# vibevoice-community/VibeVoice

Hardware: AMD Instinct MI355X
Metric: audio-sec/wall-sec (higher is better)
Workload: dtype bf16

## Files before the change

vibevoice_amd/csrc/engine.hip:

```cpp
#include "engine_ctx.h"

thread_local char g_err[512] = "";
std::shared_mutex g_dev_mu;
std::mutex g_family_mu;

int fail(vv_ctx* ctx, const char* fmt, ...) {
    va_list ap; va_start(ap, fmt);
    char* dst = ctx ? ctx->err : g_err;
    vsnprintf(dst, 512, fmt, ap);
    va_end(ap);
    if (ctx) snprintf(g_err, 512, "%s", ctx->err);
    return -1;
}

int ring_acquire(vv_ctx* ctx) {
    const int slot = ctx->ring_i;
    ctx->ring_i = (ctx->ring_i + 1) % vv_ctx::RING;
    if (ctx->ring_used[slot]) hipEventSynchronize(ctx->ring_ev[slot]);
    ctx->ring_used[slot] = true;
    return slot;
}

void* dalloc(vv_ctx* ctx, size_t bytes, bool zero) {
    void* p = nullptr;
    if (bytes == 0) bytes = 16;
    if (hipMalloc(&p, bytes) != hipSuccess) { fail(ctx, "hipMalloc(%zu) failed", bytes); return nullptr; }
    if (zero) hipMemset(p, 0, bytes);
    else { static const int poison = [] { const char* e = getenv("VVHIP_POISON"); return (e && e[0] == '1') ? 1 : 0; }();
           if (poison) hipMemset(p, 0xFF, bytes); }
    if (ctx) ctx->allocs.insert(p);
    return p;
}
void dfree(vv_ctx* ctx, void* p) {
    if (!p) return;
    if (ctx) ctx->allocs.erase(p);
    hipFree(p);
}

int add_w(vv_ctx* ctx, const std::string& name, int kind, int64_t nelem, bool optional) {
    Weight w; w.name = name; w.kind = kind; w.nelem = nelem; w.optional = optional;
    ctx->widx[name] = (int)ctx->w.size();
    ctx->w.push_back(w);
    return (int)ctx->w.size() - 1;
}
void add_mat(vv_ctx* ctx, const std::string& name, int N, int K, void* base, int ntile_off, int pk, int Cin, int Cout, int ksz,
             int stride, int64_t src_nelem) {
    int i = add_w(ctx, name, W_MAT, src_nelem < 0 ? (int64_t)N * K : src_nelem);
    Weight& w = ctx->w[i];
    w.N = N; w.K = K; w.pk = pk; w.Cin = Cin; w.Cout = Cout; w.ksz = ksz; w.stride = stride;
    const int k_tiles = (K + 31) / 32;
    w.dev = (char*)base + (int64_t)ntile_off * k_tiles * 1024;
}
void* walloc(vv_ctx* ctx, size_t bytes, bool zero) {
    if (!ctx->creating) return dalloc(ctx, bytes, zero);
    if (ctx->parent) {
        vv_ctx* p = ctx->parent;
        if (ctx->wshare_i >= p->wallocs.size() || p->wallocs[ctx->wshare_i].second != bytes) {
            fail(ctx, "vv_create_shared: weight allocation %zu (%zu bytes) does not match the parent's -- different model configuration", ctx->wshare_i, bytes);
            return nullptr;
        }
        void* q = p->wallocs[ctx->wshare_i++].first;
        ctx->wallocs.push_back({q, bytes});
        return q;
    }
    void* q = dalloc(ctx, bytes, zero);
    ctx->wallocs.push_back({q, bytes});
    return q;
}
void* alloc_packed(vv_ctx* ctx, int N, int K) { return walloc(ctx, (size_t)vv_packed_elems(N, K) * 2); }
float* add_vec(vv_ctx* ctx, const std::string& name, int64_t n, float* dst, int kind, int rep) {
    int i = add_w(ctx, name, kind, n);
    if (!dst) dst = (float*)walloc(ctx, (size_t)n * rep * 4);
    ctx->w[i].dev = dst; ctx->w[i].rep = rep;
    return dst;
}

VVGemm mk_gemm(const void* W, const float* X, float* Y, int T, int N, int K, int ldx, int ldy) {
    VVGemm g; memset(&g, 0, sizeof(g));
    g.W = (const u32x4*)W; g.X = X; g.Y = Y; g.T = T; g.N = N; g.K = K; g.ldx = ldx; g.ldy = ldy;
    g.pro = VV_PRO_NONE; g.epi = VV_EPI_STORE; g.ksplit = 0; g.nt = 0; g.eps = 1e-6f;
    return g;
}
int ksplit_parts(const vv_ctx* ctx, VVGemm& g, float* parts, int part_stride) {
    const int n_tiles = (g.N + 15) / 16, k_tiles = (g.K + 31) / 32;
    constexpr int max_tiles = 128;
    if (g.T > 4 || n_tiles > max_tiles || k_tiles < 96) return 0;
    const int ks = 3;
    g.kgrid = ks; g.yparts = parts; g.part_stride = part_stride;
    if (!vv_gemv_ok(&g)) { g.kgrid = 0; g.yparts = nullptr; g.part_stride = 0; return 0; }
    return ks - 1;
}
int graphed_run(vv_ctx* ctx, const std::string& key, hipStream_t st, const std::function<int()>& body) {
    if (!ctx->c.use_graph || ctx->prof_on) { VV_SHARED; return body(); }
    auto it = ctx->graphs.find(key);
    if (it == ctx->graphs.end()) {
        if (ctx->seen.size() > 8192) ctx->seen.clear();
        if (ctx->seen.insert(key).second) { VV_SHARED; return body(); }
        hipGraph_t graph = nullptr;
        GraphEntry ge; ge.last_use = 0;
        bool captured = false;
        {
            std::unique_lock<std::shared_mutex> lk(g_dev_mu);
            HIPCHK(ctx, hipStreamBeginCapture(st, hipStreamCaptureModeRelaxed));
            const int r = body();
            const hipError_t e = hipStreamEndCapture(st, &graph);
            if (r == 0 && e == hipSuccess) {
                size_t nn = 0;
                if (hipGraphGetNodes(graph, nullptr, &nn) == hipSuccess && nn) {
                    std::vector<hipGraphNode_t> nodes(nn);
                    if (hipGraphGetNodes(graph, nodes.data(), &nn) == hipSuccess)
                        for (size_t i = 0; i < nn; ++i) { hipGraphNodeType t; if (hipGraphNodeGetType(nodes[i], &t) == hipSuccess && t != hipGraphNodeTypeKernel) ctx->foreign_nodes++; }
                }
                HIPCHK(ctx, hipGraphInstantiate(&ge.exec, graph, nullptr, nullptr, 0));
                hipGraphDestroy(graph);
                captured = true;
            } else {
                (void)hipGetLastError();
                ctx->capture_fallbacks++;
                snprintf(ctx->last_capture_issue, sizeof(ctx->last_capture_issue), "capture of '%s': body rc %d, hipStreamEndCapture: %s", key.c_str(), r, hipGetErrorString(e));
            }
        }
        if (!captured) {
            VV_SHARED;
            const int r2 = body();
            if (r2 != 0) {
                char prev[200]; snprintf(prev, sizeof(prev), "%s", ctx->err);
                return fail(ctx, "%s; the eager re-run failed as well (%s).  If another host thread called a device-wide synchronize "
                                 "(torch.cuda.synchronize()) during the capture, the stream is lost: synchronize streams or events instead", ctx->last_capture_issue, prev);
            }
            return 0;
        }
        if (ctx->graphs.size() >= ctx->graph_cap) {
            std::vector<std::pair<uint64_t, std::string>> order;
            for (auto& g : ctx->graphs) order.push_back({g.second.last_use, g.first});
            std::sort(order.begin(), order.end());
            std::unique_lock<std::shared_mutex> lk(g_dev_mu);
            HIPCHK(ctx, hipDeviceSynchronize());
            for (size_t i = 0; i < order.size() / 4 + 1; ++i) {
                auto v = ctx->graphs.find(order[i].second);
                hipGraphExecDestroy(v->second.exec);
                ctx->graphs.erase(v);
            }
        }
        it = ctx->graphs.emplace(key, ge).first;
    }
    it->second.last_use = ++ctx->graph_tick;
    VV_SHARED;
    HIPCHK(ctx, hipGraphLaunch(it->second.exec, st));
    return 0;
}

int drop_graphs(vv_ctx* ctx, std::initializer_list<const char*> prefixes) {
    auto hit = [&](const std::string& key) {
        for (const char* p : prefixes) if (key.rfind(p, 0) == 0) return true;
        return false;
    };
    bool any = false;
    for (auto& g : ctx->graphs) if (hit(g.first)) { any = true; break; }
    if (!any) return 0;
    HIPCHK(ctx, hipDeviceSynchronize());
    for (auto it = ctx->graphs.begin(); it != ctx->graphs.end();) {
        if (hit(it->first)) { hipGraphExecDestroy(it->second.exec); it = ctx->graphs.erase(it); } else ++it;
    }
    return 0;
}

extern "C" const char* vv_last_error(vv_ctx* ctx) { return ctx ? ctx->err : g_err; }

#ifndef VV_BUILD_ID
// ... 55 lines not shown
        L.wg = alloc_packed(ctx, I, H); add_mat(ctx, p + "mlp.gate_proj.weight", I, H, L.wg, 0);
        L.wu = alloc_packed(ctx, I, H); add_mat(ctx, p + "mlp.up_proj.weight", I, H, L.wu, 0);
        L.wd = alloc_packed(ctx, H, I); add_mat(ctx, p + "mlp.down_proj.weight", H, I, L.wd, 0);
    }
    const int n_caches = 2 * c.n_slots;
    ctx->head_stride = (int64_t)c.max_ctx * D;
    ctx->layer_stride = ctx->head_stride * Hkv;
    ctx->cache_stride = ctx->layer_stride * c.lm_layers;
    ctx->kc = dalloc(ctx, (size_t)ctx->cache_stride * n_caches * 2);
    ctx->vc = dalloc(ctx, (size_t)ctx->cache_stride * n_caches * 2);
    ctx->rows_cap = std::max(2048, c.max_rows);
    ctx->rows_dev = (VVRow*)dalloc(ctx, sizeof(VVRow) * ctx->rows_cap);
    hipHostMalloc((void**)&ctx->rows_pin, sizeof(VVRow) * (size_t)ctx->rows_cap * vv_ctx::RING);
    for (int i = 0; i < vv_ctx::RING; ++i) hipEventCreateWithFlags(&ctx->ring_ev[i], hipEventDisableTiming);
    ctx->ids_cap = std::max(64, c.max_rows);
    ctx->ids_dev = (int*)dalloc(ctx, sizeof(int) * ctx->ids_cap);
    hipHostMalloc((void**)&ctx->ids_pin, sizeof(int) * (size_t)ctx->ids_cap * vv_ctx::RING);
    ctx->h = (float*)dalloc(ctx, (size_t)R * H * 4);
    ctx->h_parts = (float*)dalloc(ctx, (size_t)2 * R * H * 4);
    ctx->qkv = (float*)dalloc(ctx, (size_t)R * QKV * 4);
    ctx->qrot = (float*)dalloc(ctx, (size_t)R * Hq * D * 4);
    ctx->attn = (float*)dalloc(ctx, (size_t)R * Hq * D * 4);
    ctx->act = (float*)dalloc(ctx, (size_t)R * I * 4);
    if (R >= 64 && (H % 8) == 0 && ((Hq * D) % 8) == 0 && (I % 8) == 0) {
        ctx->xp = dalloc(ctx, (size_t)vv_packed_elems(R, std::max(H, Hq * D)) * 2);
        ctx->actp = dalloc(ctx, (size_t)vv_packed_elems(R, I) * 2);
        ctx->tile3_ok = c.xsplit == 1;
        if (ctx->tile3_ok) {
            ctx->gws.g3_bytes = (size_t)8 * std::min(R, 1024) * std::max(ctx->QKV, H) * 4;
            ctx->gws.g3_partials = (float*)dalloc(ctx, ctx->gws.g3_bytes, false);
            if (!ctx->gws.g3_partials) ctx->gws.g3_bytes = 0;
        }
        const char* no_ks = getenv("VVHIP_NO_KSPLIT");
        if (ctx->tile3_ok && R >= 1024 && !(no_ks && no_ks[0] == '1')) {
            ctx->gws.partials = (float*)dalloc(ctx, (size_t)256 * 32 * 512 * 16, false);
            ctx->gws.flags = (unsigned*)dalloc(ctx, 256 * sizeof(unsigned));
            if (hipHostMalloc((void**)&ctx->gws.err, sizeof(unsigned), hipHostMallocMapped) == hipSuccess && ctx->gws.err) *ctx->gws.err = 0u;
            else ctx->gws.err = nullptr;
        }
    }
    ctx->attn2_ok = c.xsplit == 1;
    if (c.xsplit == 1 && R > 4 && (H % 32) == 0 && ((Hq * D) % 32) == 0 && (I % 32) == 0) {
        const int kx = std::max(H, Hq * D), ka = std::max(I, c.head_ffn);
        ctx->p16_x = dalloc(ctx, (size_t)vv_packed_elems(16, kx) * 2);
        ctx->p16_act = dalloc(ctx, (size_t)vv_packed_elems(16, ka + 32) * 2);
        ctx->p16_y = dalloc(ctx, (size_t)vv_packed_elems(16, kx) * 2);
        ctx->ssq_a = (float*)dalloc(ctx, (size_t)(H / 16) * 16 * 4);
        ctx->ssq_b = (float*)dalloc(ctx, (size_t)(H / 16) * 16 * 4);
        ctx->p16_ok = ctx->p16_x && ctx->p16_act && ctx->p16_y && ctx->ssq_a && ctx->ssq_b;
    }
    ctx->rope_tab = dalloc(ctx, (size_t)c.max_ctx * (D / 2) * 8, false);
    ctx->ws_rows = std::min(R, 64);
    const size_t np = (size_t)ctx->ws_rows * Hkv * c.attn_splits * 16;
    ctx->pm = (float*)dalloc(ctx, np * 4); ctx->pl = (float*)dalloc(ctx, np * 4); ctx->po = (float*)dalloc(ctx, np * D * 4);
    const int L = c.latent_dim, HL = c.head_layers, HF = ctx->HF = c.head_ffn;
    const int MODW = ctx->MODW = HL * 3 * H + 2 * H;
    ctx->h_in = alloc_packed(ctx, H, L); add_mat(ctx, "head.noisy_images_proj.weight", H, L, ctx->h_in, 0);
    ctx->h_cond = alloc_packed(ctx, H, H); add_mat(ctx, "head.cond_proj.weight", H, H, ctx->h_cond, 0);
    ctx->h_t0 = alloc_packed(ctx, H, 256); add_mat(ctx, "head.t_embedder.mlp.0.weight", H, 256, ctx->h_t0, 0);
    ctx->h_t2 = alloc_packed(ctx, H, H); add_mat(ctx, "head.t_embedder.mlp.2.weight", H, H, ctx->h_t2, 0);
    ctx->h_ada = alloc_packed(ctx, MODW, H);
    ctx->hl.resize(HL);
    for (int l = 0; l < HL; ++l) {
        char nm[128]; snprintf(nm, 128, "head.layers.%d.", l);
        std::string p(nm);
        ctx->hl[l].norm = add_vec(ctx, p + "norm.weight", H);
        add_mat(ctx, p + "adaLN_modulation.1.weight", 3 * H, H, ctx->h_ada, l * 3 * H / 16);
        ctx->hl[l].wg = alloc_packed(ctx, HF, H); add_mat(ctx, p + "ffn.gate_proj.weight", HF, H, ctx->hl[l].wg, 0);
        ctx->hl[l].wu = alloc_packed(ctx, HF, H); add_mat(ctx, p + "ffn.up_proj.weight", HF, H, ctx->hl[l].wu, 0);
        ctx->hl[l].wd = alloc_packed(ctx, H, HF); add_mat(ctx, p + "ffn.down_proj.weight", H, HF, ctx->hl[l].wd, 0);
    }
    add_mat(ctx, "head.final_layer.adaLN_modulation.1.weight", 2 * H, H, ctx->h_ada, HL * 3 * H / 16);
    ctx->h_out = alloc_packed(ctx, L, H); add_mat(ctx, "head.final_layer.linear.weight", L, H, ctx->h_out, 0);
    const int R2 = 16;
    ctx->cproj = (float*)dalloc(ctx, (size_t)R2 * H * 4);
    ctx->mod = (float*)dalloc(ctx, (size_t)R2 * MODW * 4);
    for (HeadGen& g : ctx->hg) {
        g.zz = (float*)dalloc(ctx, (size_t)R2 * L * 4);
        g.x0p = (float*)dalloc(ctx, (size_t)R2 * L * 4);
        g.xh = (float*)dalloc(ctx, (size_t)R2 * H * 4);
    }
    ctx->head_tail = c.xsplit == 1 && L == 64 && (H % 32) == 0 && vv_head_tail_init() == 0;
    if (const char* e = getenv("VVHIP_SOLVER_FUSE"); e && e[0] == '0') ctx->solver_fuse = false;
    if (const char* e = getenv("VVHIP_NAN_PROBE"); e && e[0] == '1') {
        ctx->probe_rec = (unsigned*)dalloc(ctx, PROBE_MAX * 16);
        ctx->probe_on = ctx->probe_rec != nullptr;
    }
    ctx->xh_parts = (float*)dalloc(ctx, (size_t)4 * R2 * H * 4);
    ctx->hact = (float*)dalloc(ctx, (size_t)R2 * HF * 4);
    ctx->eps = (float*)dalloc(ctx, (size_t)R2 * L * 4);
    ctx->tmp1 = (float*)dalloc(ctx, (size_t)64 * H * 4);
    ctx->tmp2 = (float*)dalloc(ctx, (size_t)64 * 256 * 4);
    auto mk_conn = [&](vv_ctx::Conn& cn, const std::string& p, int din) {
        cn.fc1 = alloc_packed(ctx, H, din); add_mat(ctx, p + "fc1.weight", H, din, cn.fc1, 0);
        cn.b1 = add_vec(ctx, p + "fc1.bias", H);
        cn.norm = add_vec(ctx, p + "norm.weight", H);
        cn.fc2 = alloc_packed(ctx, H, H); add_mat(ctx, p + "fc2.weight", H, H, cn.fc2, 0);
        cn.b2 = add_vec(ctx, p + "fc2.bias", H);
    };
    mk_conn(ctx->ac_conn, "ac_conn.", L);
    if (c.sem_dim > 0) mk_conn(ctx->sem_conn, "sem_conn.", c.sem_dim);
    ctx->ct1 = (float*)dalloc(ctx, (size_t)256 * H * 4);
    if (build_codec(ctx, ctx->dec, "dec.", true, L, 1, c.n_slots)) { *out = ctx; return -1; }
    if (c.sem_dim > 0 && build_codec(ctx, ctx->senc, "senc.", false, c.sem_dim, 1, c.n_slots)) { *out = ctx; return -1; }
    if (c.has_acoustic_encoder && build_codec(ctx, ctx->aenc, "aenc.", false, L, c.enc_frames, 1)) { *out = ctx; return -1; }
    if (hipDeviceSynchronize() != hipSuccess || ctx->err[0]) { *out = ctx; return fail(ctx, "vv_create: allocation failed: %s", ctx->err); }
    ctx->creating = false;
    if (parent) {
        if (ctx->wshare_i != parent->wallocs.size() || ctx->w.size() != parent->w.size()) {
            *out = ctx;
            return fail(ctx, "vv_create_shared: the child registered %zu weight buffers / %zu parameters, the parent %zu / %zu -- different model configuration",
                        ctx->wshare_i, ctx->w.size(), parent->wallocs.size(), parent->w.size());
        }
        for (size_t i = 0; i < ctx->w.size(); ++i) {
            if (ctx->w[i].name != parent->w[i].name || ctx->w[i].nelem != parent->w[i].nelem) { *out = ctx; return fail(ctx, "vv_create_shared: parameter table differs at '%s'", ctx->w[i].name.c_str()); }
            ctx->w[i].loaded = parent->w[i].loaded;
            if (ctx->w[i].name == "lm_head.weight") ctx->w[i].dev = parent->w[i].dev;
        }
        ctx->lm_head = parent->lm_head; ctx->lm_head_loaded = parent->lm_head_loaded;
        ctx->scaling = parent->scaling; ctx->bias = parent->bias;
        { std::lock_guard<std::mutex> fl(g_family_mu); parent->n_children++; }
    }
    *out = ctx;
    return 0;
}

extern "C" int vv_create(const vv_config* cfg, vv_ctx** out) { return create_impl(cfg, nullptr, out); }

extern "C" int vv_create_shared(const vv_config* cfg, vv_ctx* parent, vv_ctx** out) {
    if (!parent) return fail(nullptr, "vv_create_shared: no parent context");
    if (parent->parent) return fail(nullptr, "vv_create_shared: the parent is itself a shared context; share from the owner of the weights");
    for (auto& w : parent->w)
        if (!w.loaded && !w.optional) return fail(nullptr, "vv_create_shared: parent parameter '%s' is not uploaded yet", w.name.c_str());
    vv_config a = *cfg, b = parent->c;
    a.n_slots = b.n_slots; a.max_ctx = b.max_ctx; a.max_rows = b.max_rows; a.attn_splits = b.attn_splits; a.use_graph = b.use_graph;
    if (a.xsplit < 1 || a.xsplit > 3) a.xsplit = 2;
    if (a.enc_frames < 1) a.enc_frames = 1;
    if (memcmp(&a, &b, sizeof(vv_config)) != 0) return fail(nullptr, "vv_create_shared: the model fields of the configuration differ from the parent's");
    int r = create_impl(cfg, parent, out);
    if (r != 0 && *out) { vv_ctx* c = *out; c->parent = nullptr; }
    return r;
}

static void destroy_impl(vv_ctx* ctx) {
    if (!ctx) return;
    hipDeviceSynchronize();
    {
        std::lock_guard<std::mutex> fl(g_family_mu);
        if (ctx->n_children > 0) { ctx->zombie = true; return; }
    }
    vv_ctx* par = ctx->parent;
    for (auto& g : ctx->graphs) hipGraphExecDestroy(g.second.exec);
    if (ctx->side_ready) {
        for (int j = 0; j < 8; ++j) { hipStreamDestroy(ctx->side[j]); hipEventDestroy(ctx->ev_join[j]); }
        hipEventDestroy(ctx->ev_fork);
    }
    for (void* p : ctx->allocs) hipFree(p);
    ctx->allocs.clear();
    if (ctx->stage) hipFree(ctx->stage);
    hipHostFree(ctx->rows_pin); hipHostFree(ctx->ids_pin);
    if (ctx->gws.err) hipHostFree(ctx->gws.err);
    for (int i = 0; i < vv_ctx::RING; ++i) if (ctx->ring_ev[i]) hipEventDestroy(ctx->ring_ev[i]);
    delete ctx;
    bool last_child = false;
    if (par) { std::lock_guard<std::mutex> fl(g_family_mu); last_child = (--par->n_children == 0 && par->zombie); }
    if (last_child) destroy_impl(par);
// ... 70 lines not shown
                HIPCHK(ctx, hipMemcpyAsync((float*)w.dev + (size_t)r * nelem, f32, (size_t)nelem * 4, hipMemcpyDeviceToDevice, st));
        } else {
            HIPCHK(ctx, hipMemcpyAsync(w.dev, f32, (size_t)nelem * 4, hipMemcpyDeviceToDevice, st));
        }
        HIPCHK(ctx, hipStreamSynchronize(st));
        dfree(ctx, tmp);
    }
    HIPCHK(ctx, hipStreamSynchronize(st));
    w.loaded = true;
    ctx->rope_ready = false;
    return 0;
}

extern "C" int vv_set_speech_factors(vv_ctx* ctx, float scaling, float bias) {
    VV_SHARED;
    ctx->scaling = scaling; ctx->bias = bias;
    return drop_graphs(ctx, {"dec:1:", "chain:1:"});
}

extern "C" int vv_set_valid_tokens(vv_ctx* ctx, const int* ids, int n) {
    VV_SHARED;
    if (n < 1 || n > 16) return fail(ctx, "n_valid must be in [1,16]");
    const int H = ctx->H;
    const void* table = ctx->lm_head_loaded ? ctx->lm_head : ctx->embed;
    void* rows = dalloc(ctx, (size_t)n * H * 2, false);
    if (!rows) return -1;
    for (int i = 0; i < n; ++i) {
        if (ids[i] < 0 || ids[i] >= ctx->c.lm_vocab) return fail(ctx, "token id %d out of range", ids[i]);
        HIPCHK(ctx, hipMemcpy((char*)rows + (size_t)i * H * 2, (const char*)table + (size_t)ids[i] * H * 2, (size_t)H * 2, hipMemcpyDeviceToDevice));
    }
    if (!ctx->valid_w) ctx->valid_w = alloc_packed(ctx, 16, H);
    VVCHK(vv_pack_launch(rows, 1, ctx->valid_w, n, H, 0, 0, 0, 0, 0, 0));
    HIPCHK(ctx, hipDeviceSynchronize());
    dfree(ctx, rows);
    ctx->n_valid = n;
    for (int i = 0; i < n; ++i) ctx->valid_ids[i] = ids[i];
    return 0;
}
extern "C" int vv_check(vv_ctx* ctx, void* stream) {
    if (!ctx) return -1;
    return ksplit_check(ctx, (hipStream_t)stream);
}
extern "C" int vv_audio_to_pcm16(vv_ctx* ctx, void* stream, int n, int samples, const float* audio_dev, int16_t* pcm_out_dev) {
    VV_SHARED;
    hipStream_t st = (hipStream_t)stream;
    if (n < 1 || samples < 1) return fail(ctx, "vv_audio_to_pcm16: n and samples must be positive");
    VVCHK(vv_pcm16_launch(audio_dev, (short*)pcm_out_dev, n, samples, st));
    return 0;
}
extern "C" int vv_connect(vv_ctx* ctx, void* stream, int n, const float* latent_dev, const float* sem_dev, float* out_dev) {
    VV_SHARED;
    hipStream_t st = (hipStream_t)stream;
    const int H = ctx->H, L = ctx->c.latent_dim;
    for (int i0 = 0; i0 < n; i0 += 16) {
        const int nn = std::min(16, n - i0);
        float* out = out_dev + (size_t)i0 * H;
        VVGemm a1 = mk_gemm(ctx->ac_conn.fc1, latent_dev + (size_t)i0 * L, ctx->ct1, nn, H, L, L, H);
        a1.epi = VV_EPI_BIAS; a1.bias = ctx->ac_conn.b1; GEMM(a1);
        VVGemm a2 = mk_gemm(ctx->ac_conn.fc2, ctx->ct1, out, nn, H, H, H, H);
        a2.pro = VV_PRO_RMS; a2.nw = ctx->ac_conn.norm; a2.eps = 1e-6f; a2.epi = VV_EPI_BIAS; a2.bias = ctx->ac_conn.b2; GEMM(a2);
        if (sem_dev) {
            const int S = ctx->c.sem_dim;
            VVGemm s1 = mk_gemm(ctx->sem_conn.fc1, sem_dev + (size_t)i0 * S, ctx->ct1, nn, H, S, S, H);
            s1.epi = VV_EPI_BIAS; s1.bias = ctx->sem_conn.b1; GEMM(s1);
            VVGemm s2 = mk_gemm(ctx->sem_conn.fc2, ctx->ct1, out, nn, H, H, H, H);
            s2.pro = VV_PRO_RMS; s2.nw = ctx->sem_conn.norm; s2.eps = 1e-6f; s2.epi = VV_EPI_RESID; s2.bias = ctx->sem_conn.b2; GEMM(s2);
        }
    }
    return 0;
}

extern "C" int64_t vv_packed_bytes(int N, int K) { return vv_packed_elems(N, K) * 2; }
extern "C" int vv_pack_matrix(void* stream, const float* src_dev, void* dst_dev, int N, int K) {
    return vv_pack_launch(src_dev, 0, dst_dev, N, K, 0, 0, 0, 0, 0, (hipStream_t)stream);
}
extern "C" int64_t vv_stat(vv_ctx* ctx, int what) {
    switch (what) {
        case 0: return ctx->launches;
        case 2: return ctx->prof_raw_ns;
        case 3: return ctx->prof_ev_over_ns;
        case 5: return ctx->foreign_nodes;
        case 4: return ctx->capture_fallbacks;
        case 6: return ctx->seam_launches;
        case 8: return ctx->solver_fused;
        case 7: return ctx->lora_base_bytes;
        default: return (int64_t)ctx->graphs.size();
    }
}
```

vibevoice_amd/csrc/engine_ctx.h:

```cpp
#pragma once
#include <algorithm>
#include <cmath>
#include <cstdarg>
#include <cstdio>
#include <cstdlib>
#include <cstring>
#include <functional>
#include <initializer_list>
#include <map>
#include <mutex>
#include <set>
#include <shared_mutex>
#include <string>
#include <vector>
#include "../../include/vvhip.h"
#include "vv_common.h"
#include "vv_launch.h"

namespace vv_engine {
struct VVShiftH { float* buf; int T, hist, C; };
enum WKind { W_MAT = 0, W_VEC = 1, W_DW = 2, W_TABLE = 3, W_BIAS_REP = 4 };

struct Weight {
    std::string name;
    int kind = W_VEC;
    int64_t nelem = 0;
    void* dev = nullptr;
    int N = 0, K = 0, pk = 0, Cin = 0, Cout = 0, ksz = 0, stride = 0;
    int rep = 1;
    bool loaded = false;
    bool optional = false;
};

struct Block {
    int C;
    float *norm_w, *ffn_norm_w, *gamma, *ffn_gamma, *dw_w, *dw_b, *b1, *b2;
    void *w1, *w2;
    float* nb;
    float* nst;
    int64_t nb_stride;
};

struct ConvG {
    void* w; float* bias;
    int K, N, ldx;
    int rows_per_frame;
};

struct Stage {
    int C, Tpf;
    int hist;
    float* xs;
    float* xs2;
    float* xfinal;
    bool fused;
    bool pp;
    int64_t sl_stride;
    std::vector<Block> blocks;
    ConvG in;
};

struct CodecNet {
    bool decoder = false;
    int Fmax = 1, in_dim = 1, out_dim = 1, in_hist = 6, in_Tpf = 1;
    std::vector<float*> in_buf;
    std::vector<std::vector<Stage>> st;
    ConvG head;
    std::vector<float*> u;
    std::map<std::pair<uint64_t, int>, std::pair<void*, int>> shift_tab;
    int maxC = 1;
    int kd = 0, ke = 1 << 30;
    bool head_batch = false;
    int64_t in_stride = 0, u_stride = 0;
};

struct GraphEntry { hipGraphExec_t exec; uint64_t last_use; };

struct HeadGen { float *xh = nullptr, *zz = nullptr, *x0p = nullptr, *m2 = nullptr; };

}
using namespace vv_engine;

constexpr int PROBE_MAX = 1024;

struct vv_ctx {
    vv_config c;
    char err[512];
    std::vector<Weight> w;
    std::map<std::string, int> widx;
    int H, D, Hq, Hkv, I, QKV;
    struct Layer { float *ln1, *ln2, *bqkv; void *wqkv, *wo, *wg, *wu, *wd; };
    std::vector<Layer> layers;
    float *lm_norm = nullptr, *inv_freq = nullptr;
    int ws_rows = 0;
    void* rope_tab = nullptr; bool rope_ready = false;
    float *tts_types = nullptr, *eos_b1 = nullptr, *eos_b2 = nullptr; void *eos_w1 = nullptr, *eos_w2 = nullptr;
    void *embed = nullptr, *lm_head = nullptr;
    bool lm_head_loaded = false;
    void* valid_w = nullptr; int n_valid = 0;
    int valid_ids[16] = {0};
    void *kc = nullptr, *vc = nullptr;
    int64_t cache_stride = 0, head_stride = 0, layer_stride = 0;
    VVRow* rows_dev = nullptr; VVRow* rows_pin = nullptr; int rows_cap = 2048;
    int* ids_dev = nullptr; int* ids_pin = nullptr; int ids_cap = 64;
    static constexpr int RING = 32;
    hipEvent_t ring_ev[RING] = {}; bool ring_used[RING] = {}; int ring_i = 0;
    float *h = nullptr, *qkv = nullptr, *qrot = nullptr, *attn = nullptr, *act = nullptr;
    float *h_parts = nullptr, *xh_parts = nullptr;
    void *xp = nullptr, *actp = nullptr;
    bool tile3_ok = false, attn2_ok = false;
    VVGemmWs gws = {nullptr, nullptr, nullptr, nullptr, 0};
    void *p16_x = nullptr, *p16_act = nullptr, *p16_y = nullptr, *p16_shift = nullptr; float *ssq_a = nullptr, *ssq_b = nullptr; bool p16_ok = false;
    size_t p16_shift_tile = 0;
    float *pm = nullptr, *pl = nullptr, *po = nullptr;
    int HF = 0, MODW = 0;
    struct HLayer { float* norm; void *wg, *wu, *wd; };
    std::vector<HLayer> hl;
    void *h_in = nullptr, *h_cond = nullptr, *h_t0 = nullptr, *h_t2 = nullptr, *h_ada = nullptr, *h_out = nullptr;
    int n_steps = 0;
    float *temb = nullptr, *coef = nullptr, *tvals = nullptr;
    bool sde_on = false;
    bool general_on = false;
    float* mod_all = nullptr; size_t mod_all_bytes = 0;
    float* ada_in = nullptr;
    void* ada_p = nullptr;
    float *cproj = nullptr, *mod = nullptr, *hact = nullptr, *eps = nullptr;
    HeadGen hg[2];
    bool head_tail = false;
    bool solver_fuse = true;
    float *tmp1 = nullptr, *tmp2 = nullptr;
    struct Conn { void *fc1, *fc2; float *b1, *b2, *norm; } ac_conn, sem_conn;
    float *ct1 = nullptr;
    CodecNet dec, aenc, senc;
    int enc_pass = 0;
    hipStream_t side[8] = {}; hipEvent_t ev_fork = nullptr, ev_join[8] = {}; bool side_ready = false;
    float scaling = 1.f, bias = 0.f;
    int hop = 3200;
    void* stage = nullptr; size_t stage_bytes = 0;
    std::map<std::string, GraphEntry> graphs;
    uint64_t graph_tick = 0; size_t graph_cap = 512;
    std::set<std::string> seen;
    std::set<void*> allocs;
    vv_ctx* parent = nullptr; int n_children = 0; bool zombie = false, creating = false;
    unsigned* probe_rec = nullptr; std::vector<std::string> probe_names; bool probe_on = false; int probe_calls = 0;
    int64_t foreign_nodes = 0;
    int64_t capture_fallbacks = 0; char last_capture_issue[256] = "";
    std::vector<std::pair<void*, size_t>> wallocs; size_t wshare_i = 0;
    struct LoraBase { void* snap; size_t bytes; bool merged; };
    std::map<int, LoraBase> lora_base;
    int64_t lora_base_bytes = 0;
    struct RowStage { int n_streams = 0; std::vector<int64_t> total; std::vector<char> flushed; };
    struct Resampler : RowStage { int L = 0, M = 0, T = 0; float* coef = nullptr; float* hist = nullptr; };
    static constexpr int N_RESAMPLERS = 4;
    Resampler rs[N_RESAMPLERS];
    struct Tempo : RowStage { float* window = nullptr; float* hist = nullptr; int* dstate = nullptr; std::vector<int> P, Q; };
    static constexpr int N_TEMPOS = 4;
    Tempo tp[N_TEMPOS];
    struct Level : RowStage { int A = 0, H = 0; float c = 0.f; float* hist = nullptr; std::vector<float> gain; };
    static constexpr int N_LEVELS = 4;
    Level lv[N_LEVELS];
    int64_t launches = 0;
    int64_t solver_fused = 0;
    int64_t seam_launches = 0;
    bool prof_on = false;
    std::vector<hipEvent_t> prof_ev;
    int prof_n = 0;
    double prof_bytes = 0.0;
    struct ProfRec { int T, N, K, pro, epi, dual; double bytes; int gemv; };
    std::vector<ProfRec> prof_rec;
    std::vector<VVGemm> prof_gemv;
    double prof_gemv_bytes = 0.0;
    struct ProfLaunch { int family; double bytes; std::function<int(hipStream_t)> fn; };
    std::vector<ProfLaunch> prof_other;
    int64_t prof_raw_ns = 0, prof_ev_over_ns = 0;
    hipStream_t prof_stream = nullptr;
#ifdef VV_GEMM_TIMING
    unsigned long long* tl_base = nullptr; int tl_idx = 0;
    struct TlRec { int T, N, K, pro, epi; };
    std::vector<TlRec> tl_rec;
#endif
};

extern thread_local char g_err[512];
extern std::shared_mutex g_dev_mu;
#define VV_SHARED std::shared_lock<std::shared_mutex> _vv_dev_lk(g_dev_mu)
extern std::mutex g_family_mu;
int fail(vv_ctx* ctx, const char* fmt, ...);
#define HIPCHK(ctx, e) do { hipError_t _e = (e); if (_e != hipSuccess) return fail(ctx, "%s:%d hip error %s", __FILE__, __LINE__, hipGetErrorString(_e)); } while (0)
#define VVCHK(e) do { int _r = (e); if (_r != 0) return _r < 0 ? fail(ctx, "%s:%d launch failed (%d): hip error %d (%s)", __FILE__, __LINE__, _r, g_vv_launch_err, hipGetErrorString((hipError_t)g_vv_launch_err)) : _r; } while (0)
#define VVTRY(e) do { if (int _r = (e)) return _r; } while (0)

void* dalloc(vv_ctx* ctx, size_t bytes, bool zero = true);
void dfree(vv_ctx* ctx, void* p);
void* walloc(vv_ctx* ctx, size_t bytes, bool zero = true);
void* alloc_packed(vv_ctx* ctx, int N, int K);
int add_w(vv_ctx* ctx, const std::string& name, int kind, int64_t nelem, bool optional = false);
void add_mat(vv_ctx* ctx, const std::string& name, int N, int K, void* base, int ntile_off, int pk = 0, int Cin = 0, int Cout = 0,
             int ksz = 0, int stride = 0, int64_t src_nelem = -1);
float* add_vec(vv_ctx* ctx, const std::string& name, int64_t n, float* dst = nullptr, int kind = W_VEC, int rep = 1);
VVGemm mk_gemm(const void* W, const float* X, float* Y, int T, int N, int K, int ldx, int ldy);
int ksplit_parts(const vv_ctx* ctx, VVGemm& g, float* parts, int part_stride);
int ring_acquire(vv_ctx* ctx);
int build_codec(vv_ctx* ctx, CodecNet& net, const std::string& pfx, bool decoder, int vae_dim, int Fmax, int n_slots);
int ksplit_check(vv_ctx* ctx, hipStream_t st);
int p16_gemv(vv_ctx* ctx, hipStream_t st, const void* W, const void* W2, const void* Xp, float* Y, void* Yp, const float* bias,
             const float* gate, int T, int N, int K, int ldy, int ld_gate, int epi);
int p16_go(vv_ctx* ctx, hipStream_t st, const VVGemv16p& a, int epi, int flags);
VVGemv16p p16_args(const void* W, const void* W2, const void* Xp, float* Y, void* Yp, int T, int N, int K, int ldy);
void nan_probe(vv_ctx* ctx, hipStream_t st, const char* name, const void* p, size_t n);
void nan_probe_report(vv_ctx* ctx, hipStream_t st, const char* what);
int gemm_prof(vv_ctx* ctx, const VVGemm& g, hipStream_t st);
int lora_rebase(vv_ctx* ctx, int widx, hipStream_t st);

#ifdef VV_GEMM_TIMING
int gemm_tl(vv_ctx* ctx, VVGemm g, hipStream_t st);
#define GEMM(g) do { ctx->launches++; VVCHK(gemm_tl(ctx, g, st)); } while (0)
#else
#define GEMM(g) do { ctx->launches++; if (ctx->prof_on) VVCHK(gemm_prof(ctx, g, st)); else VVCHK(vv_gemm_launch(g, ctx->c.xsplit, st)); } while (0)
#endif

int graphed_run(vv_ctx* ctx, const std::string& key, hipStream_t st, const std::function<int()>& body);
int drop_graphs(vv_ctx* ctx, std::initializer_list<const char*> prefixes);
template <class F>
static int graphed(vv_ctx* ctx, const std::string& key, hipStream_t st, F&& body) { return graphed_run(ctx, key, st, std::ref(body)); }
```

vibevoice_amd/csrc/engine_head.hip:

```cpp
#include "engine_ctx.h"
#include "pass_plan.h"

static int set_schedule(vv_ctx* ctx, int n_steps, const float* t, const float* coef, int width, void* stream, bool stochastic = false) {
    VV_SHARED;
    hipStream_t st = (hipStream_t)stream;
    if (n_steps < 1 || n_steps > 64) return fail(ctx, "n_steps must be in [1,64]");
    const int H = ctx->H;
    if (!ctx->temb) {
        ctx->temb = (float*)dalloc(ctx, (size_t)64 * H * 4);
        ctx->coef = (float*)dalloc(ctx, 64 * 8 * 4);
        ctx->tvals = (float*)dalloc(ctx, 64 * 4);
    }
    const bool general = width == 8;
    if (general && !ctx->hg[0].m2) {
        for (HeadGen& g : ctx->hg) g.m2 = (float*)dalloc(ctx, (size_t)8 * ctx->c.latent_dim * 4);
        if (!ctx->hg[0].m2 || !ctx->hg[1].m2) return fail(ctx, "vv_set_schedule_general: out of device memory");
    }
    float rows[64 * 8] = {};
    for (int i = 0; i < n_steps; ++i)
        for (int j = 0; j < width; ++j) rows[i * 8 + j] = coef[i * width + j];
    ctx->sde_on = general ? stochastic : (width == 6);
    ctx->general_on = general;
    HIPCHK(ctx, hipStreamSynchronize(st));
    HIPCHK(ctx, hipMemcpy(ctx->coef, rows, (size_t)n_steps * 8 * 4, hipMemcpyHostToDevice));
    HIPCHK(ctx, hipMemcpy(ctx->tvals, t, (size_t)n_steps * 4, hipMemcpyHostToDevice));
    VVCHK(vv_tfreq_launch(ctx->tvals, ctx->tmp2, n_steps, st));
    for (int i0 = 0; i0 < n_steps; i0 += 16) {
        const int nn = std::min(16, n_steps - i0);
        VVGemm g = mk_gemm(ctx->h_t0, ctx->tmp2 + (size_t)i0 * 256, ctx->tmp1 + (size_t)i0 * H, nn, H, 256, 256, H);
        GEMM(g);
    }
    VVCHK(vv_silu_launch(ctx->tmp1, n_steps * H, st));
    for (int i0 = 0; i0 < n_steps; i0 += 16) {
        const int nn = std::min(16, n_steps - i0);
        VVGemm g = mk_gemm(ctx->h_t2, ctx->tmp1 + (size_t)i0 * H, ctx->temb + (size_t)i0 * H, nn, H, H, H, H);
        GEMM(g);
    }
    HIPCHK(ctx, hipStreamSynchronize(st));
    ctx->n_steps = n_steps;
    {
        const size_t need = (size_t)n_steps * 16 * ctx->MODW * 4;
        if (need > ctx->mod_all_bytes) {
            dfree(ctx, ctx->mod_all);
            dfree(ctx, ctx->ada_in);
            ctx->mod_all = (float*)dalloc(ctx, need, false);
            ctx->ada_in = (float*)dalloc(ctx, (size_t)n_steps * 16 * ctx->H * 4, false);
            dfree(ctx, ctx->ada_p);
            ctx->ada_p = (ctx->c.xsplit == 1 && (ctx->H & 7) == 0) ? dalloc(ctx, (size_t)vv_packed_elems(n_steps * 16, ctx->H) * 2, false) : nullptr;
            ctx->mod_all_bytes = (ctx->mod_all && ctx->ada_in) ? need : 0;
            dfree(ctx, ctx->p16_shift); ctx->p16_shift = nullptr;
            if (ctx->p16_ok) {
                ctx->p16_shift_tile = (size_t)vv_packed_elems(16, ctx->H) * 2;
                ctx->p16_shift = dalloc(ctx, (size_t)n_steps * (ctx->c.head_layers + 1) * ctx->p16_shift_tile);
            }
        }
    }
    return drop_graphs(ctx, {"samp:", "sde:", "rows:", "gen:"});
}
extern "C" int vv_set_schedule(vv_ctx* ctx, int n_steps, const float* t, const float* coef, void* stream) {
    return set_schedule(ctx, n_steps, t, coef, 5, stream);
}
extern "C" int vv_set_schedule_sde(vv_ctx* ctx, int n_steps, const float* t, const float* coef6, void* stream) {
    return set_schedule(ctx, n_steps, t, coef6, 6, stream);
}

extern "C" int vv_set_schedule_general(vv_ctx* ctx, int n_steps, const float* t, const float* coef, int stochastic, void* stream) {
    return set_schedule(ctx, n_steps, t, coef, 8, stream, stochastic != 0);
}

static VVHeadPlan head_plan(const vv_ctx* ctx, int rows, int n_steps, bool has_coef) {
    return vv_head_plan(rows, n_steps, ctx->HF, ctx->c.head_layers, ctx->MODW,
                        {ctx->p16_ok, ctx->p16_shift != nullptr, ctx->ada_p != nullptr, ctx->mod_all_bytes != 0, ctx->head_tail}, has_coef,
                        has_coef && ctx->general_on);
}

struct StepEnd { const float* coef; float cfg; const float *cfg_rows, *noise; };
struct HeadStep {
    int step;
    const float *z, *temb, *mod;
    const unsigned char* sh_tiles;
    float* eps_out;
    const HeadGen &cur, &nxt;
    bool have_x;
    const StepEnd* end;
};

static int head_eval(vv_ctx* ctx, hipStream_t st, const VVHeadPlan& p, const HeadStep& s) {
    const vv_config& c = ctx->c;
    const int rows = p.rows, final_stage = vv_head_final(p, s.step);
    const int H = ctx->H, L = c.latent_dim, HL = c.head_layers, HF = ctx->HF, MODW = ctx->MODW;
    const float* mod = s.mod ? s.mod : ctx->mod;
    const StepEnd end = s.end ? *s.end : StepEnd{};
    auto put_end = [&](auto& a) { a.coef = end.coef; a.cfg = end.cfg; a.n_cfg = rows / 2; a.sde_noise = end.noise; a.cfg_rows = end.cfg_rows; };
    float* const xh = s.cur.xh;
    if (!s.mod) {
        VVGemm ga = mk_gemm(ctx->h_ada, ctx->cproj, ctx->mod, rows, MODW, H, H, MODW);
        ga.pro = VV_PRO_ADD_SILU; ga.addvec = s.temb; ga.nt = 1;
        GEMM(ga);
    }
    if (!s.have_x) {
        VVGemm gi = mk_gemm(ctx->h_in, s.z, xh, rows, H, L, L, H);
        GEMM(gi);
        nan_probe(ctx, st, "in-proj xh", xh, (size_t)rows * H);
    }
    int xp = 0;
    const int xps = 16 * H;
    for (int l = 0; l < HL; ++l) {
        const float* base = mod + (size_t)l * 3 * H;
        if (p.layers == VV_HEAD_P16) {
            ctx->launches += 3;
            VVCHK(vv_pack16_launch(xh, H, 2, ctx->hl[l].norm, c.head_eps, base + H, base, MODW, ctx->p16_x, rows, H, st));
            VVCHK(p16_gemv(ctx, st, ctx->hl[l].wg, ctx->hl[l].wu, ctx->p16_x, nullptr, ctx->p16_act, nullptr, nullptr, rows, HF, H, 0, 0, VV_EPI_SWIGLU));
            if (l + 1 == HL && final_stage == VV_FINAL_P16_CFG) {
                VVGemv16p ad = p16_args(ctx->hl[l].wd, nullptr, ctx->p16_act, xh, ctx->p16_x, rows, H, HF, H);
                ad.gate = base + 2 * H; ad.ld_gate = MODW; ad.ssq_out = ctx->ssq_a;
                ad.pk_nw = nullptr; ad.pk_sc = mod + (size_t)HL * 3 * H + H; ad.ld_pk = MODW;
                VVCHK(p16_go(ctx, st, ad, VV_EPI_GATED_RESID, 4));
            } else
            VVCHK(p16_gemv(ctx, st, ctx->hl[l].wd, nullptr, ctx->p16_act, xh, nullptr, nullptr, base + 2 * H, rows, H, HF, H, MODW, VV_EPI_GATED_RESID));
            continue;
        }
        VVGemm g1 = mk_gemm(ctx->hl[l].wg, xh, ctx->hact, rows, HF, H, H, HF);
        g1.W2 = (const u32x4*)ctx->hl[l].wu; g1.pro = VV_PRO_RMS_MOD; g1.nw = ctx->hl[l].norm; g1.eps = c.head_eps;
        g1.mod_shift = base; g1.mod_scale = base + H; g1.ld_mod = MODW; g1.epi = VV_EPI_SWIGLU; g1.nt = 1;
        float* cur = ctx->xh_parts + (size_t)(l & 1) * 2 * xps;
        float* nxt = ctx->xh_parts + (size_t)((l + 1) & 1) * 2 * xps;
        g1.xa = cur; g1.n_xa = xp; g1.part_stride = xps;
        GEMM(g1);
        VVGemm g2 = mk_gemm(ctx->hl[l].wd, ctx->hact, xh, rows, H, HF, HF, H);
        g2.epi = VV_EPI_GATED_RESID; g2.gate = base + 2 * H; g2.ld_gate = MODW; g2.nt = 1;
        g2.ya = cur; g2.n_ya = xp; g2.part_stride = xps;
        xp = ksplit_parts(ctx, g2, nxt, xps);
        if (ctx->probe_on) { char nm[64]; snprintf(nm, 64, "layer %d hact (parts in %d)", l, g1.n_xa); nan_probe(ctx, st, nm, ctx->hact, (size_t)rows * HF); }
        GEMM(g2);
        if (ctx->probe_on) {
            char nm[64]; snprintf(nm, 64, "layer %d xh", l); nan_probe(ctx, st, nm, xh, (size_t)rows * H);
            for (int q = 0; q < xp; ++q) { snprintf(nm, 64, "layer %d part %d", l, q); nan_probe(ctx, st, nm, nxt + (size_t)q * xps, (size_t)rows * H); }
        }
    }
    const float* fb = mod + (size_t)HL * 3 * H;
    if (final_stage == VV_FINAL_P16_CFG) {
        ctx->launches += 1;
        VVGemv16p af = p16_args(ctx->h_out, nullptr, ctx->p16_x, nullptr, nullptr, rows, L, H, L);
        af.ssq_in = ctx->ssq_a; af.ssq_tiles = H / 16; af.eps = c.head_eps;
        af.Xs = (const u32x4*)(s.sh_tiles + (size_t)HL * ctx->p16_shift_tile);
        af.z = s.cur.zz; af.x0p = s.cur.x0p; put_end(af);
        VVCHK(p16_go(ctx, st, af, VV_EPI_CFG_DPM, 3));
        return 0;
    }
    if (final_stage == VV_FINAL_SEAM) {
        VVTail t{};
        t.Wout = (const u32x4*)ctx->h_out; t.Win = (const u32x4*)ctx->h_in; t.bin = nullptr;
        t.X = xh; t.xa = ctx->xh_parts + (size_t)(HL & 1) * 2 * xps; t.n_xa = xp; t.part_stride = xps;
        t.sc = fb + H; t.sh = fb; t.ld_mod = MODW;
        t.Xout = s.nxt.xh;
        t.z_in = s.cur.zz; t.x0p_in = s.cur.x0p; t.z_out = s.nxt.zz; t.x0p_out = s.nxt.x0p; put_end(t);
        t.T = rows; t.H = H; t.L = L; t.eps = c.head_eps;
        if (vv_head_tail_ok(&t)) {
            ctx->launches++;
            ctx->seam_launches++;
            if (ctx->prof_on) {
                const VVTail tc = t;
                ctx->prof_other.push_back({3, (double)vv_packed_elems(L, H) * 2.0 + (double)vv_packed_elems(H, L) * 2.0 + (double)rows * H * 8.0,
                                           [=](hipStream_t s2) { return vv_head_tail_launch(&tc, s2); }});
            }
            VVCHK(vv_head_tail_launch(&t, st));
            return 1;
        }
    }
    VVGemm gf = mk_gemm(ctx->h_out, xh, s.eps_out, rows, L, H, H, L);
    gf.pro = VV_PRO_RMS_MOD; gf.nw = nullptr; gf.eps = c.head_eps; gf.mod_shift = fb; gf.mod_scale = fb + H; gf.ld_mod = MODW;
    gf.xa = ctx->xh_parts + (size_t)(HL & 1) * 2 * xps; gf.n_xa = xp; gf.part_stride = xps;
    if (final_stage != VV_FINAL_GEMM) {
        gf.epi = VV_EPI_CFG_DPM; gf.z = s.cur.zz; gf.x0p = s.cur.x0p; put_end(gf);
    }
    GEMM(gf);
    return 0;
}

struct SampleReq { int n; const float *cond, *noise, *step_noise; float cfg; const float* cfg_rows; float* out; };
struct StepDone { int rc; bool flipped; };

static StepDone step_shipped(vv_ctx* ctx, hipStream_t st, const VVHeadPlan& p, const SampleReq& r, HeadStep s) {
    const StepEnd end{ctx->coef + s.step * 8, r.cfg, r.cfg_rows,
                      r.step_noise ? r.step_noise + (size_t)s.step * r.n * ctx->c.latent_dim : nullptr};
    s.end = &end;
    const int hr = head_eval(ctx, st, p, s);
    return {hr, hr == 1};
}

static StepDone step_general(vv_ctx* ctx, hipStream_t st, const VVHeadPlan& p, const SampleReq& r, const HeadStep& s) {
    const int L = ctx->c.latent_dim;
    if (head_eval(ctx, st, p, s) < 0) return {-1, false};
    VVSolverStep v{};
    v.eps = s.eps_out; v.coef = ctx->coef + s.step * 8; v.cfg = r.cfg; v.cfg_rows = r.cfg_rows; v.n = r.n; v.L = L;
    v.noise = r.step_noise ? r.step_noise + (size_t)s.step * r.n * L : nullptr;
    v.z_in = s.cur.zz; v.m1_in = s.cur.x0p; v.m2_in = s.cur.m2;
    v.z_out = s.nxt.zz; v.m1_out = s.nxt.x0p; v.m2_out = s.nxt.m2;
    if (s.step + 1 < p.n_steps && ctx->solver_fuse) { v.Win = (const u32x4*)ctx->h_in; v.Xout = s.nxt.xh; v.H = ctx->H; v.xs = ctx->c.xsplit; }
    ctx->launches++;
    const int sr = vv_solver_step_launch(&v, st);
    if (sr == VV_RC_NO_FORM) return {fail(ctx, "vv_diffusion_sample_general: solver.hip has no form for n = %d, latent_dim = %d", r.n, L), false};
    if (sr < 0) return {fail(ctx, "%s:%d launch failed (%d): hip error %d (%s)", __FILE__, __LINE__, sr, g_vv_launch_err, hipGetErrorString((hipError_t)g_vv_launch_err)), false};
    if (sr == 1) ctx->solver_fused++;
    return {sr == 1, true};
}

static int sample_body(vv_ctx* ctx, hipStream_t st, const SampleReq& r) {
    const int H = ctx->H, L = ctx->c.latent_dim, HL = ctx->c.head_layers;
    const int n = r.n, rows = 2 * n;
    ctx->seam_launches = ctx->solver_fused = 0;
    ctx->probe_names.clear();
    nan_probe(ctx, st, "cond (input)", r.cond, (size_t)rows * H);
    nan_probe(ctx, st, "noise (input)", r.noise, (size_t)n * L);
    VVCHK(vv_sampler_init_launch(r.noise, ctx->hg[0].zz, ctx->hg[0].x0p, n * L, st));
    VVGemm gc = mk_gemm(ctx->h_cond, r.cond, ctx->cproj, rows, H, H, H, H);
    gc.nt = 1;
    GEMM(gc);
    const int MODW = ctx->MODW;
    const VVHeadPlan p = head_plan(ctx, rows, ctx->n_steps, true);
    const bool batch_ada = p.ada != VV_ADA_PER_STEP;
    if (batch_ada) {
        const int total = rows * ctx->n_steps;
        if (p.ada == VV_ADA_TILE) {
            ctx->launches += 2;
            VVCHK(vv_ada_pack_launch(ctx->cproj, ctx->temb, ctx->ada_p, rows, ctx->n_steps, H, st));
            VVCHK(vv_gemm3_launch(ctx->h_ada, nullptr, ctx->ada_p, ctx->mod_all, nullptr, nullptr, total, MODW, H, MODW, VV_EPI_STORE, nullptr, st));
        } else {
        VVCHK(vv_ada_in_launch(ctx->cproj, ctx->temb, ctx->ada_in, rows, ctx->n_steps, H, st));
        ctx->launches++;
        for (int t0 = 0; t0 < total; t0 += 16) {
            const int T = std::min(16, total - t0);
            VVGemm ga = mk_gemm(ctx->h_ada, ctx->ada_in + (size_t)t0 * H, ctx->mod_all + (size_t)t0 * MODW, T, MODW, H, H, MODW);
            GEMM(ga);
        }
        }
    }
    nan_probe(ctx, st, "cproj", ctx->cproj, (size_t)rows * H);
    if (batch_ada) nan_probe(ctx, st, "mod_all", ctx->mod_all, (size_t)rows * ctx->n_steps * MODW);
    if (p.sh_tiles) {
        ctx->launches++;
        VVCHK(vv_pack16_tiles_launch(ctx->mod_all, MODW, (int64_t)rows * MODW, HL + 1, (int64_t)3 * H, ctx->p16_shift,
                                     (int64_t)ctx->p16_shift_tile, rows, H, ctx->n_steps * (HL + 1), st));
    }
    int gen = 0; bool have_x = false;
    for (int i = 0; i < ctx->n_steps; ++i) {
        const HeadGen& cur = ctx->hg[gen];
        const HeadStep s{.step = i, .z = cur.zz, .temb = ctx->temb + (size_t)i * H,
                         .mod = batch_ada ? ctx->mod_all + (size_t)i * rows * MODW : nullptr,
                         .sh_tiles = p.sh_tiles ? (const unsigned char*)ctx->p16_shift + (size_t)i * (HL + 1) * ctx->p16_shift_tile : nullptr,
                         .eps_out = ctx->eps, .cur = cur, .nxt = ctx->hg[gen ^ 1], .have_x = have_x, .end = nullptr};
        const StepDone d = p.solver_step ? step_general(ctx, st, p, r, s) : step_shipped(ctx, st, p, r, s);
        if (d.rc < 0) return -1;
        have_x = d.rc == 1;
        gen ^= d.flipped;
        if (ctx->probe_on) {
            const HeadGen& now = ctx->hg[gen];
            char nm[64];
            snprintf(nm, 64, "step %d z%s", i, p.solver_step ? " (general)" : have_x ? " (seam, next gen)" : ""); nan_probe(ctx, st, nm, now.zz, (size_t)rows * L);
            if (!p.solver_step) { snprintf(nm, 64, "step %d x0p", i); nan_probe(ctx, st, nm, now.x0p, (size_t)n * L); }
            if (!p.solver_step && have_x) { snprintf(nm, 64, "step %d next xh", i); nan_probe(ctx, st, nm, now.xh, (size_t)rows * H); }
        }
    }
    VVCHK(vv_copy_launch(r.out, ctx->hg[gen].zz, (size_t)n * L * 4, st));
    return 0;
}

static int run_sampler(vv_ctx* ctx, hipStream_t st, const char* key, const SampleReq& r) {
    ctx->launches = 0;
    const int rc = graphed(ctx, key, st, [&]() { return sample_body(ctx, st, r); });
    nan_probe_report(ctx, st, key);
    return rc;
}

extern "C" int vv_diffusion_sample(vv_ctx* ctx, void* stream, int n, const float* cond_dev, const float* noise_dev, float cfg_scale, float* latent_out_dev) {
    if (ctx->n_steps < 1) return fail(ctx, "vv_set_schedule has not been called");
    if (n < 1 || n > 8) return fail(ctx, "vv_diffusion_sample: n must be in [1,8]");
    if (ctx->general_on) return fail(ctx, "the installed table is a general one (vv_set_schedule_general): sample with vv_diffusion_sample_general");
    if (ctx->sde_on) return fail(ctx, "the schedule is stochastic (vv_set_schedule_sde): sample with vv_diffusion_sample_sde and its per-step noise");
    char key[128]; snprintf(key, 128, "samp:%d:%p:%p:%p:%a", n, (const void*)cond_dev, (const void*)noise_dev, (void*)latent_out_dev, cfg_scale);
    return run_sampler(ctx, (hipStream_t)stream, key, {n, cond_dev, noise_dev, nullptr, cfg_scale, nullptr, latent_out_dev});
}

extern "C" int vv_diffusion_sample_sde(vv_ctx* ctx, void* stream, int n, const float* cond_dev, const float* noise_dev,
                                       const float* step_noise_dev, float cfg_scale, float* latent_out_dev) {
    if (ctx->n_steps < 1) return fail(ctx, "vv_set_schedule_sde has not been called");
    if (n < 1 || n > 8) return fail(ctx, "vv_diffusion_sample_sde: n must be in [1,8]");
    if (ctx->general_on) return fail(ctx, "the installed table is a general one (vv_set_schedule_general): sample with vv_diffusion_sample_general");
    if (!ctx->sde_on) return fail(ctx, "the schedule is deterministic (vv_set_schedule): sample with vv_diffusion_sample");
    if (!step_noise_dev) return fail(ctx, "vv_diffusion_sample_sde: step_noise is null");
    char key[160]; snprintf(key, 160, "sde:%d:%p:%p:%p:%p:%a", n, (const void*)cond_dev, (const void*)noise_dev, (const void*)step_noise_dev,
                            (void*)latent_out_dev, cfg_scale);
    return run_sampler(ctx, (hipStream_t)stream, key, {n, cond_dev, noise_dev, step_noise_dev, cfg_scale, nullptr, latent_out_dev});
}

extern "C" int vv_diffusion_sample_rows(vv_ctx* ctx, void* stream, int n, const float* cond_dev, const float* noise_dev,
                                        const float* step_noise_dev, const float* cfg_rows_dev, float* latent_out_dev) {
    if (ctx->n_steps < 1) return fail(ctx, "vv_set_schedule / vv_set_schedule_sde has not been called");
    if (n < 1 || n > 8) return fail(ctx, "vv_diffusion_sample_rows: n must be in [1,8]");
    if (ctx->general_on) return fail(ctx, "the installed table is a general one (vv_set_schedule_general): sample with vv_diffusion_sample_general");
    if (!cfg_rows_dev) return fail(ctx, "vv_diffusion_sample_rows: cfg_rows is null");
    if (ctx->sde_on && !step_noise_dev) return fail(ctx, "the schedule is stochastic (vv_set_schedule_sde): vv_diffusion_sample_rows needs its per-step noise");
    if (!ctx->sde_on && step_noise_dev) return fail(ctx, "the schedule is deterministic (vv_set_schedule): vv_diffusion_sample_rows takes no step noise");
    char key[192]; snprintf(key, 192, "rows:%d:%p:%p:%p:%p:%p", n, (const void*)cond_dev, (const void*)noise_dev, (const void*)step_noise_dev,
                            (const void*)cfg_rows_dev, (void*)latent_out_dev);
    return run_sampler(ctx, (hipStream_t)stream, key, {n, cond_dev, noise_dev, step_noise_dev, 0.f, cfg_rows_dev, latent_out_dev});
}

extern "C" int vv_diffusion_sample_general(vv_ctx* ctx, void* stream, int n, const float* cond_dev, const float* noise_dev,
                                           const float* step_noise_dev, float cfg_scale, const float* cfg_rows_dev, float* latent_out_dev) {
    if (ctx->n_steps < 1) return fail(ctx, "vv_set_schedule_general has not been called");
    if (n < 1 || n > 8) return fail(ctx, "vv_diffusion_sample_general: n must be in [1,8]");
    if (!ctx->general_on) return fail(ctx, "the installed table is a shipped one (vv_set_schedule / vv_set_schedule_sde): sample with vv_diffusion_sample, _sde or _rows");
    if (ctx->sde_on && !step_noise_dev) return fail(ctx, "the general table is stochastic: vv_diffusion_sample_general needs its per-step noise");
    if (!ctx->sde_on && step_noise_dev) return fail(ctx, "the general table is deterministic: vv_diffusion_sample_general takes no step noise");
    char key[224]; snprintf(key, 224, "gen:%d:%p:%p:%p:%p:%p:%a", n, (const void*)cond_dev, (const void*)noise_dev, (const void*)step_noise_dev,
                            (const void*)cfg_rows_dev, (void*)latent_out_dev, cfg_rows_dev ? 0.f : cfg_scale);
    return run_sampler(ctx, (hipStream_t)stream, key, {n, cond_dev, noise_dev, step_noise_dev, cfg_scale, cfg_rows_dev, latent_out_dev});
}

extern "C" int vv_head_forward(vv_ctx* ctx, void* stream, int n, const float* noisy_dev, const float* t_host, const float* cond_dev, float* out_dev) {
    VV_SHARED;
    hipStream_t st = (hipStream_t)stream;
    if (n < 1 || n > 16) return fail(ctx, "vv_head_forward: n must be in [1,16]");
    const int H = ctx->H;
    for (int i = 1; i < n; ++i) if (t_host[i] != t_host[0]) return fail(ctx, "vv_head_forward: all rows must share one timestep");
    float* tdev = ctx->tmp2 + 63 * 256;
    HIPCHK(ctx, hipStreamSynchronize(st));
    HIPCHK(ctx, hipMemcpy(tdev + 128, t_host, 4, hipMemcpyHostToDevice));
    VVCHK(vv_tfreq_launch(tdev + 128, ctx->tmp2, 1, st));
    VVGemm g = mk_gemm(ctx->h_t0, ctx->tmp2, ctx->tmp1, 1, H, 256, 256, H); GEMM(g);
    VVCHK(vv_silu_launch(ctx->tmp1, H, st));
    VVGemm g2 = mk_gemm(ctx->h_t2, ctx->tmp1, ctx->tmp1 + H, 1, H, H, H, H); GEMM(g2);
    VVGemm gc = mk_gemm(ctx->h_cond, cond_dev, ctx->cproj, n, H, H, H, H); GEMM(gc);
    const HeadStep s{.step = 0, .z = noisy_dev, .temb = ctx->tmp1 + H, .mod = nullptr, .sh_tiles = nullptr, .eps_out = out_dev,
                     .cur = ctx->hg[0], .nxt = ctx->hg[1], .have_x = false, .end = nullptr};
    if (head_eval(ctx, st, head_plan(ctx, n, 1, false), s)) return -1;
    HIPCHK(ctx, hipStreamSynchronize(st));
    return 0;
}
```

vibevoice_amd/csrc/engine_prof.hip:

```cpp
#include "engine_ctx.h"

static __global__ void vv_nan_probe_kernel(const float* __restrict__ p, int n, unsigned* __restrict__ rec) {
    unsigned cnt = 0, first = 0xffffffffu, mx = 0;
    for (int i = blockIdx.x * blockDim.x + threadIdx.x; i < n; i += gridDim.x * blockDim.x) {
        const float v = p[i];
        if (!(fabsf(v) <= 3.0e38f)) { cnt++; first = min(first, (unsigned)i); }
        else mx = max(mx, __float_as_uint(fabsf(v)));
    }
    if (cnt) { atomicAdd(rec, cnt); atomicMax(rec + 1, 0xffffffffu - first); }
    atomicMax(rec + 2, mx);
}
void nan_probe(vv_ctx* ctx, hipStream_t st, const char* name, const void* p, size_t n) {
    if (!ctx->probe_on || !p || n == 0) return;
    const int id = (int)ctx->probe_names.size();
    if (id >= PROBE_MAX) return;
    ctx->probe_names.push_back(name);
    if (id == 0) (void)vv_zero_launch(ctx->probe_rec, PROBE_MAX * 16, st);
    hipLaunchKernelGGL(vv_nan_probe_kernel, dim3(64), dim3(256), 0, st, (const float*)p, (int)n, ctx->probe_rec + 4 * id);
}
void nan_probe_report(vv_ctx* ctx, hipStream_t st, const char* what) {
    if (!ctx->probe_on) return;
    std::vector<unsigned> h(PROBE_MAX * 4);
    const hipError_t e1 = hipStreamSynchronize(st);
    const hipError_t e2 = hipMemcpy(h.data(), ctx->probe_rec, PROBE_MAX * 16, hipMemcpyDeviceToHost);
    const int call = ctx->probe_calls++;
    if (e1 != hipSuccess || e2 != hipSuccess) { fprintf(stderr, "[nan_probe] %s call %d: sync %d copy %d\n", what, call, (int)e1, (int)e2); (void)hipGetLastError(); return; }
    { const size_t ns = ctx->probe_names.size(); bool tail_dirty = false;
      for (size_t i = 4 * ns; i < (size_t)PROBE_MAX * 4; ++i) if (h[i]) { tail_dirty = true; break; }
      if (tail_dirty) fprintf(stderr, "[nan_probe] %s call %d (prof %d): record buffer %p holds words nobody wrote: %08x %08x %08x %08x | %08x %08x %08x %08x (last 4 words)\n",
                              what, call, (int)ctx->prof_on, (void*)ctx->probe_rec, h[0], h[1], h[2], h[3], h[4092], h[4093], h[4094], h[4095]); }
    int bad = 0;
    for (size_t i = 0; i < ctx->probe_names.size(); ++i) if (h[4 * i]) bad++;
    if (!bad) { if (call < 6) fprintf(stderr, "[nan_probe] %s call %d: %zu stages clean\n", what, call, ctx->probe_names.size()); return; }
    fprintf(stderr, "[nan_probe] %s call %d: %d of %zu stages hold non-finite values\n", what, call, bad, ctx->probe_names.size());
    int shown = 0;
    for (size_t i = 0; i < ctx->probe_names.size() && shown < 12; ++i) {
        float mx; memcpy(&mx, &h[4 * i + 2], 4);
        if (h[4 * i] || (i + 1 < ctx->probe_names.size() && h[4 * (i + 1)] && !shown)) {
            fprintf(stderr, "[nan_probe]   stage %3zu %-28s non-finite %u (first at %u), finite absmax %.4e\n", i, ctx->probe_names[i].c_str(), h[4 * i],
                    h[4 * i] ? 0xffffffffu - h[4 * i + 1] : 0u, mx);
            if (h[4 * i]) shown++;
        }
    }
}
static double gemm_bytes(const VVGemm& g) {
    double w = (double)vv_packed_elems(g.N, g.K) * 2.0 * (g.W2 ? 2.0 : 1.0);
    double x = (double)g.T * g.K * 4.0;
    double y = (double)g.T * g.N * 4.0 * ((g.epi == VV_EPI_RESID || g.epi == VV_EPI_GATED_RESID) ? 2.0 : 1.0);
    return w + x + y;
}
int gemm_prof(vv_ctx* ctx, const VVGemm& g, hipStream_t st) {
    if ((size_t)(2 * ctx->prof_n + 2) > ctx->prof_ev.size()) {
        size_t old = ctx->prof_ev.size();
        ctx->prof_ev.resize(old + 2048);
        for (size_t i = old; i < ctx->prof_ev.size(); ++i) hipEventCreate(&ctx->prof_ev[i]);
    }
    ctx->prof_stream = st;
    hipEventRecord(ctx->prof_ev[2 * ctx->prof_n], st);
    int r = vv_gemm_launch(g, ctx->c.xsplit, st);
    hipEventRecord(ctx->prof_ev[2 * ctx->prof_n + 1], st);
    ctx->prof_n++;
    ctx->prof_bytes += gemm_bytes(g);
    const bool is_gemv = vv_gemm_route(&g, ctx->c.xsplit) == VV_ROUTE_GEMV;
    ctx->prof_rec.push_back({g.T, g.N, g.K, g.pro, g.epi, g.W2 ? 1 : 0, gemm_bytes(g), is_gemv});
    if (is_gemv) { ctx->prof_gemv.push_back(g); ctx->prof_gemv_bytes += gemm_bytes(g); }
    return r;
}
#ifdef VV_GEMM_TIMING
constexpr int TL_MAX = 4096, TL_STRIDE = 16 + 2 * 3200;
int gemm_tl(vv_ctx* ctx, VVGemm g, hipStream_t st) {
    if (!ctx->tl_base && getenv("VVHIP_TIMELINE")) {
        if (hipMalloc(&ctx->tl_base, (size_t)TL_MAX * TL_STRIDE * 8) != hipSuccess) return -9;
        hipMemset(ctx->tl_base, 0, (size_t)TL_MAX * TL_STRIDE * 8);
    }
    const bool gv = vv_gemm_route(&g, ctx->c.xsplit) == VV_ROUTE_GEMV;
    const bool want = gv ? ((g.T <= 4 || g.T != 16 || g.N > 16384) && (g.N + 15) / 16 <= 3200) : (g.T > 16);
    if (ctx->tl_base && ctx->tl_idx < TL_MAX && want) {
        g.dbg = ctx->tl_base + (size_t)ctx->tl_idx * TL_STRIDE;
        ctx->tl_rec.push_back({g.T, g.N, g.K, g.pro, gv ? g.epi : g.epi + 100});
        ctx->tl_idx++;
    }
    return vv_gemm_launch(g, ctx->c.xsplit, st);
}
extern "C" int vv_timeline_dump(vv_ctx* ctx, unsigned long long* out_host, int* meta_host, int max_launches) {
    VV_SHARED;
    hipDeviceSynchronize();
    const int n = std::min(max_launches, ctx->tl_idx);
    if (n > 0) hipMemcpy(out_host, ctx->tl_base, (size_t)n * TL_STRIDE * 8, hipMemcpyDeviceToHost);
    for (int i = 0; i < n; ++i) { const auto& r = ctx->tl_rec[i]; int* m = meta_host + 5 * i; m[0] = r.T; m[1] = r.N; m[2] = r.K; m[3] = r.pro; m[4] = r.epi; }
    return n;
}
#endif

extern "C" int vv_gemm_raw(void* stream, const void* w, const void* w2, const float* x, float* y, int T, int N, int K,
                           int ldx, int ldy, int pro, int epi, const float* nw, float eps, const float* bias,
                           const float* nscale, int xsplit, int ksplit, int nontemporal) {
    VVGemm g = mk_gemm(w, x, y, T, N, K, ldx, ldy);
    g.W2 = (const u32x4*)w2; g.pro = pro; g.epi = epi; g.nw = nw; g.eps = eps; g.bias = bias; g.nscale = nscale;
    g.ksplit = ksplit & 0xff; g.nt = 1;
    g.dbg = (unsigned long long*)(uintptr_t)0;
    if (nontemporal > 1) g.dbg = reinterpret_cast<unsigned long long*>(const_cast<float*>(nscale));
    if (g.dbg) g.nscale = nullptr;
    return vv_gemm_launch(g, xsplit, (hipStream_t)stream);
}
extern "C" int vv_gemv_case(void* stream, const vv_gemv_case_args* c, int xsplit, int* form_out) {
    if (!c || xsplit < 1 || xsplit > 3) return -1;
    VVGemm g = mk_gemm(c->W, c->X, c->Y, c->T, c->N, c->K, c->ldx, c->ldy);
    g.W2 = (const u32x4*)c->W2; g.pro = c->pro; g.epi = c->epi; g.nw = c->nw; g.eps = c->eps; g.bias = c->bias; g.nscale = c->nscale;
    g.mod_scale = c->mod_scale; g.mod_shift = c->mod_shift; g.ld_mod = c->ld_mod;
    g.addvec = c->addvec; g.x_row_mod = c->x_row_mod; g.add_rows_per_vec = c->add_rows_per_vec;
    g.gate = c->gate; g.ld_gate = c->ld_gate;
    g.z = c->z; g.x0p = c->x0p; g.coef = c->coef; g.cfg = c->cfg; g.n_cfg = c->n_cfg; g.sde_noise = c->sde_noise;
    g.cfg_rows = c->cfg_rows;
    g.kgrid = c->kgrid; g.yparts = c->yparts; g.xa = c->xa; g.n_xa = c->n_xa; g.ya = c->ya; g.n_ya = c->n_ya; g.part_stride = c->part_stride;
    g.sl_n = c->sl_n; g.sl_T = c->sl_T; g.sl_x = c->sl_x; g.sl_y = c->sl_y;
    for (int j = 0; j < 8; ++j) g.sl_id[j] = c->sl_id[j];
    g.dw_hist = c->dw_hist; g.dw_w = c->dw_w; g.dw_b = c->dw_b; g.dw_gamma = c->dw_gamma; g.dw_nw = c->dw_nw;
    g.dw_xout = c->dw_xout; g.dw_hnew = c->dw_hnew;
    g.nt = 1;
    if (!vv_gemv_ok(&g)) return VV_GEMV_REFUSED;
    int form[5] = {0, 0, 0, 0, 0};
    const int r = vv_gemv_launch(g, xsplit, (hipStream_t)stream, form);
    if (r == VV_RC_NO_FORM) return VV_GEMV_REFUSED;
    if (r == 0 && form_out) for (int j = 0; j < 5; ++j) form_out[j] = form[j];
    return r;
}
extern "C" int vv_gemm3_raw(vv_ctx* ctx, void* stream, const void* w, const void* w2, const float* x_dev, int T, int N, int K, int epi,
                            const float* nw_dev, float eps, const float* bias_dev, float* y_dev, void* xp_scratch, void* yp_scratch) {
    hipStream_t st = (hipStream_t)stream;
    if (ctx && ksplit_check(ctx, st)) return -1;
    int r = vv_pack_rows_launch(x_dev, K, nw_dev, eps, xp_scratch, T, K, st);
// ... 93 lines not shown
```

vibevoice_amd/csrc/gemm.hip:

```cpp
#include <cstdlib>
#include "vv_common.h"
#include "vv_device.h"
#include "vv_launch.h"

#ifdef VV_GEMM_TIMING
#define VV_STAMP(i) do { if (a.dbg && blockIdx.x == 0 && blockIdx.y == 0 && threadIdx.x == 0) a.dbg[i] = __builtin_amdgcn_s_memtime(); } while (0)
#define VV_BSTAMP(i) do { if (a.dbg && threadIdx.x == 0 && blockIdx.y * gridDim.x + blockIdx.x < 3200) a.dbg[16 + 2 * (blockIdx.y * gridDim.x + blockIdx.x) + (i)] = __builtin_amdgcn_s_memrealtime(); } while (0)
#else
#define VV_STAMP(i) do { } while (0)
#define VV_BSTAMP(i) do { } while (0)
#endif

namespace {

template <int NT, int XS, bool DUAL, int WPB, int MAXR, bool VEC>
__global__ __launch_bounds__(WPB * 64) void vv_gemm_kernel(const VVGemm a) {
    constexpr int NM = DUAL ? 2 * NT : NT;
    constexpr bool PREFETCH = (WPB == 8);
    constexpr bool MODREG = (MAXR <= 4);
    constexpr int U = 8;
    extern __shared__ __attribute__((aligned(16))) unsigned char smem[];
    asm volatile("" ::"s"(a.W), "s"(a.W2), "s"(a.X), "s"(a.Y), "s"(a.nw), "s"(a.mod_scale), "s"(a.mod_shift),
                 "s"(a.addvec), "s"(a.bias), "s"(a.nscale), "s"(a.gate));
    asm volatile("" ::"s"(a.T), "s"(a.N), "s"(a.K), "s"(a.ldx), "s"(a.ldy), "s"(a.ld_mod), "s"(a.ld_gate), "s"(a.x_row_mod), "s"(a.add_rows_per_vec),
// ... 209 lines not shown
                if (b >= 0) mma_batch(kt_begin + b * U, wcur);
                if (have_next) {
                    stage_finish(ktn, R);
                    if (b == -1) VV_STAMP(2);
#pragma unroll
                    for (int u = 0; u < U; ++u)
#pragma unroll
                        for (int i = 0; i < NM; ++i) wcur[u][i] = wnext[u][i];
                }
            }
        } else {
#pragma unroll 1
            for (int ktb = kt_begin; ktb < kt_end; ktb += U) {
                stage_load(ktb, R);
                load_w(ktb, wcur);
                stage_finish(ktb, R);
                mma_batch(ktb, wcur);
            }
        }
    }

    VV_STAMP(3);
    float my_ssq = 0.f;
    if (a.pro == VV_PRO_RMS) {
#pragma unroll
        for (int r = 0; r < MAXR; ++r) {
            if (r < Tt) {
                const float s = vv_wave_sum(ssq[r]);
                if (frow == r) my_ssq = s;
            }
        }
    }

    VV_STAMP(4);
    if (KS > 1) {
        __syncthreads();
        f32x4* red = reinterpret_cast<f32x4*>(smem);
        float* redq = reinterpret_cast<float*>(smem + (size_t)WPB * NM * 64 * 16);
#pragma unroll
        for (int i = 0; i < NM; ++i) red[(wave * NM + i) * 64 + lane] = acc[i];
        redq[wave * 64 + lane] = my_ssq;
        __syncthreads();
        if (ks == 0) {
            for (int s = 1; s < KS; ++s) {
#pragma unroll
                for (int i = 0; i < NM; ++i) acc[i] += red[((wave + s) * NM + i) * 64 + lane];
                my_ssq += redq[(wave + s) * 64 + lane];
            }
        }
    }
    VV_STAMP(5);
    if (ks != 0 || tile0 >= n_tiles) return;

    const int row = t0 + frow;
    if (frow >= Tt) return;
    float rs = 1.0f;
    if (a.pro == VV_PRO_RMS) rs = rsqrtf(my_ssq / (float)a.K + a.eps);
    float cfg = a.cfg;
    if (a.epi == VV_EPI_CFG_DPM && a.cfg_rows && frow < a.n_cfg) cfg = a.cfg_rows[frow];
#pragma unroll
    for (int i = 0; i < NT; ++i) {
        const int n0 = (tile0 + i) * 16 + fq * 4;
        if (n0 >= a.N) continue;
        float* yp = a.Y + (int64_t)row * a.ldy + n0;
        float o4[4] = {acc[i][0] * rs, acc[i][1] * rs, acc[i][2] * rs, acc[i][3] * rs};
        float u4[4] = {0.f, 0.f, 0.f, 0.f};
        if constexpr (DUAL) { u4[0] = acc[NT + i][0] * rs; u4[1] = acc[NT + i][1] * rs; u4[2] = acc[NT + i][2] * rs; u4[3] = acc[NT + i][3] * rs; }
        if (a.epi == VV_EPI_CFG_DPM) {
            const int nc = a.n_cfg;
            const VVSolverCoef c5 = vv_solver_coef(a.coef, false);
#pragma unroll 1
            for (int r = 0; r < 4; ++r) {
                const float vu = __shfl(o4[r], lane + nc);
                const int n = n0 + r;
                if (frow < nc && n < a.N) {
                    const int64_t zi = (int64_t)frow * a.N + n;
                    VVSolverCoef cf = c5;
                    if (a.sde_noise) cf.cn = a.coef[5];
                    float x0, zn;
                    vv_cfg_dpm_update(o4[r], vu, cfg, a.z[zi], a.x0p[zi], cf, a.sde_noise != nullptr, [&] { return a.sde_noise[zi]; }, x0, zn);
                    a.x0p[zi] = x0;
                    a.z[zi] = zn;
                    a.z[zi + (int64_t)nc * a.N] = zn;
                }
            }
            continue;
        }
        if (vec_epi) {
            const float pb[4] = {pre_b[i].x, pre_b[i].y, pre_b[i].z, pre_b[i].w};
            const float py[4] = {pre_y[i].x, pre_y[i].y, pre_y[i].z, pre_y[i].w};
            const float pg[4] = {pre_g[i].x, pre_g[i].y, pre_g[i].z, pre_g[i].w};
            float o[4];
#pragma unroll
            for (int r = 0; r < 4; ++r) {
                o[r] = o4[r];
                if (a.epi == VV_EPI_BIAS) o[r] += pb[r];
                else if (a.epi == VV_EPI_BIAS_GELU) o[r] = vv_gelu_erf(o[r] + pb[r]);
                else if (a.epi == VV_EPI_SWIGLU) o[r] = vv_silu(o[r]) * u4[r];
                else if (a.epi == VV_EPI_RESID) o[r] = (o[r] + pb[r]) * pg[r] + py[r];
                else if (a.epi == VV_EPI_GATED_RESID) o[r] = py[r] + pg[r] * o[r];
            }
            *reinterpret_cast<float4*>(yp) = float4{o[0], o[1], o[2], o[3]};
            continue;
        }
#pragma unroll 1
        for (int r = 0; r < 4; ++r) {
            const int n = n0 + r;
            if (n >= a.N) break;
            float o = o4[r];
            if (a.bias && (a.epi == VV_EPI_BIAS || a.epi == VV_EPI_BIAS_GELU || a.epi == VV_EPI_RESID)) o += a.bias[n];
            if (a.epi == VV_EPI_BIAS_GELU) o = vv_gelu_erf(o);
            else if (a.epi == VV_EPI_SWIGLU) o = vv_silu(o) * u4[r];
            else if (a.epi == VV_EPI_RESID) { if (a.nscale) o *= a.nscale[n]; o += yp[r]; }
            else if (a.epi == VV_EPI_GATED_RESID) o = yp[r] + a.gate[(int64_t)row * a.ld_gate + n] * o;
            yp[r] = o;
        }
    }
    VV_STAMP(6);
    VV_BSTAMP(1);
}

template <typename ST>
__global__ void vv_pack_kernel(const ST* __restrict__ src, __bf16* __restrict__ dst,
                               int N, int K, int kind, int Cin, int Cout, int ksz, int stride) {
    const int64_t total = vv_packed_elems(N, K);
    const int k_tiles = (K + 31) >> 5;
    for (int64_t e = (int64_t)blockIdx.x * blockDim.x + threadIdx.x; e < total;
         e += (int64_t)gridDim.x * blockDim.x) {
        const int j = (int)(e & 7);
        const int lane = (int)((e >> 3) & 63);
        const int64_t tile = e >> 9;
        const int kt = (int)(tile % k_tiles);
        const int ntile = (int)(tile / k_tiles);
        const int n = ntile * 16 + (lane & 15);
        const int k = kt * 32 + (lane >> 4) * 8 + j;
        float v = 0.f;
        if (n < N && k < K) {
            int64_t si;
            if (kind == 0) {
                si = (int64_t)n * K + k;
            } else if (kind == 1) {
                const int jj = k / Cin, c = k - jj * Cin;
                si = ((int64_t)n * Cin + c) * ksz + jj;
            } else {
                const int jj = n / Cout, o = n - jj * Cout;
                const int tap = k / Cin, c = k - tap * Cin;
                si = ((int64_t)c * Cout + o) * ksz + (tap == 0 ? jj + stride : jj);
            }
            v = (float)src[si];
        }
        dst[e] = (__bf16)v;
    }
}

}

template <int NT, int XS, bool DUAL, int WPB, int MAXR, bool VEC>
static void launch_t(const VVGemm& a, dim3 grid, size_t smem, hipStream_t s) {
    static const hipError_t lds = vv_raise_lds_limit(160 * 1024, &vv_gemm_kernel<NT, XS, DUAL, WPB, MAXR, VEC>);
    (void)lds;
    hipLaunchKernelGGL((vv_gemm_kernel<NT, XS, DUAL, WPB, MAXR, VEC>), grid, dim3(WPB * 64), smem, s, a);
}

using GeneralLaunch = void (*)(const VVGemm&, dim3, size_t, hipStream_t);
struct GeneralForm { int nt; bool dual; int wpb, maxr; bool vec; GeneralLaunch launch[3]; };
#define VV_FORM(NT_, DUAL_, WPB_, MAXR_, VEC_) \
// ... 41 lines not shown
```

vibevoice_amd/csrc/gemv.hip:

```cpp
#include <array>
#include <utility>
#include "vv_common.h"
#include "vv_device.h"
#include "vv_launch.h"

#ifdef VV_GEMM_TIMING
#define VV_STAMP(i) do { if (a.dbg && blockIdx.x == 0 && threadIdx.x == 0) a.dbg[i] = __builtin_amdgcn_s_memtime(); } while (0)
#define VV_BSTAMP(i) do { if (a.dbg && threadIdx.x == 0 && blockIdx.y * gridDim.x + blockIdx.x < 3200) a.dbg[16 + 2 * (blockIdx.y * gridDim.x + blockIdx.x) + (i)] = __builtin_amdgcn_s_memrealtime(); } while (0)
#else
#define VV_BSTAMP(i) do { } while (0)
#define VV_STAMP(i) do { } while (0)
#endif

namespace {

constexpr int U = 8;


template <int XS, int PRO, int EPI, int MR, int WPB, int PARTS = 0, int SL = 0>
__global__ __launch_bounds__(WPB * 64) void vv_gemv_kernel(const u32x4* __restrict__ pW, const u32x4* __restrict__ pW2,
                                                           const float* __restrict__ pX, float* __restrict__ pY,
                                                           const float* __restrict__ pnw, int pT, int pN, int pK, int pldx,
                                                           int pldy, const VVGemm a) {
    constexpr bool DUAL = (EPI == VV_EPI_SWIGLU);
    constexpr int NM = DUAL ? 2 : 1;
    constexpr bool FOLD = (PRO == VV_PRO_RMS_MOD) && MR <= 4;
    constexpr int NOP = (PRO == VV_PRO_RMS_MOD && !FOLD) ? 2 : 1;
    constexpr int MRS = FOLD ? 2 * MR : MR;
    constexpr int GSB = MRS * 16 + (MR == 16 ? 16 : 0);
    __shared__ __attribute__((aligned(16))) unsigned char stg_all[WPB * NOP * XS * U * 4 * GSB];
    __shared__ f32x4 red[WPB][NM * NOP][64];
    __shared__ float ssq_sh[WPB][MR];
    __shared__ float ssq1_sh[PRO == VV_PRO_NORMDW ? WPB : 1];
    asm volatile("" ::"s"(a.mod_scale), "s"(a.mod_shift), "s"(a.addvec), "s"(a.bias), "s"(a.nscale), "s"(a.gate));
    asm volatile("" ::"s"(a.ld_mod), "s"(a.ld_gate), "s"(a.x_row_mod), "s"(a.add_rows_per_vec),
                 "s"(a.eps), "s"(a.z), "s"(a.x0p), "s"(a.coef), "s"(a.cfg), "s"(a.n_cfg));
    asm volatile("" ::"s"(a.yparts), "s"(a.xa), "s"(a.ya), "s"(a.n_xa), "s"(a.n_ya), "s"(a.part_stride));
    if constexpr (EPI == VV_EPI_CFG_DPM) asm volatile("" ::"s"(a.sde_noise), "s"(a.cfg_rows));
    VV_STAMP(0);
    VV_BSTAMP(0);
    const int lane = threadIdx.x & 63;
    const int wave = __builtin_amdgcn_readfirstlane((int)(threadIdx.x >> 6));
    const int t_base = (MR == 16) ? (int)blockIdx.y * 16 : 0;
    const int T = min(MR, pT - t_base);
    const unsigned tile = blockIdx.x;
    const unsigned k_tiles = (unsigned)(pK + 31) >> 5;
    const unsigned KSB = (MR <= 4) ? gridDim.y : 1u;
    const unsigned ksb = (MR <= 4) ? blockIdx.y : 0u;
    const unsigned kchunk = (k_tiles + KSB - 1) / KSB;
    const unsigned kb0 = min(k_tiles, ksb * kchunk), kb1 = min(k_tiles, kb0 + kchunk);
    const unsigned kper = (kb1 - kb0 + WPB - 1) / WPB;
    const unsigned kt0 = kb0 + wave * kper;
    const unsigned kt1 = min(kb1, kt0 + kper);
    const bool has_k = kt0 < kt1;
    const int frow = lane & 15, fq = lane >> 4;
    unsigned char* stg = stg_all + (size_t)wave * (NOP * XS * U * 4 * GSB);
    const unsigned kk = lane * 4;
    const unsigned st_off = ((kk >> 5) * 4 + ((kk & 31) >> 3)) * GSB + (kk & 7) * 2;

    const u32x4* wbase = pW + (size_t)tile * k_tiles * 64 + lane;
    const u32x4* wbase2 = DUAL ? pW2 + (size_t)tile * k_tiles * 64 + lane : nullptr;

    unsigned xoff_sl[SL ? MR : 1];
    if constexpr (SL) {
#pragma unroll
        for (int r = 0; r < MR; ++r) {
            const int rg = t_base + r;
            const int j = rg / a.sl_T, tt = rg - j * a.sl_T;
            xoff_sl[r] = (r < T) ? (a.sl_x ? (unsigned)(vv_slot_id(a.sl_id, j) * a.sl_x + tt * pldx) : (unsigned)(rg * pldx)) : 0u;
        }
    }
    constexpr int MODR = (PRO == VV_PRO_RMS_MOD) ? MR : 1;
    constexpr int ADDR = (PRO == VV_PRO_ADD_SILU) ? MR : 1;
    constexpr int PR = (PARTS == 1) ? MR : 1;
    constexpr int DWH = (PRO == VV_PRO_NORMDW) ? 6 : 1, DWT = (PRO == VV_PRO_NORMDW) ? 7 : 1;
    struct XR { float4 x[MR]; float4 p0[PR]; float4 p1[PR]; float4 sc[MODR]; float4 sh[MODR]; float4 addv[ADDR]; float4 nwv;
                float4 dh[DWH]; float4 dt[DWT]; float4 db, dg, dn; };
    auto x_load = [&](unsigned ktb, XR& R) {
        unsigned k = ktb * 32 + kk;
        const bool kin = k < min(kt1 * 32, (unsigned)pK);
        if (!kin) k = 0;
        R.nwv = pnw ? *reinterpret_cast<const float4*>(pnw + k) : float4{1.f, 1.f, 1.f, 1.f};
        if constexpr (PRO == VV_PRO_NORMDW) {
#pragma unroll
            for (int j = 0; j < 6; ++j) R.dh[j] = *reinterpret_cast<const float4*>(a.dw_hist + (unsigned)(j * pK) + k);
#pragma unroll
            for (int j = 0; j < 7; ++j) R.dt[j] = *reinterpret_cast<const float4*>(a.dw_w + (unsigned)(j * pK) + k);
            R.db = *reinterpret_cast<const float4*>(a.dw_b + k);
            R.dg = *reinterpret_cast<const float4*>(a.dw_gamma + k);
            R.dn = *reinterpret_cast<const float4*>(a.dw_nw + k);
        }
#pragma unroll
        for (int r = 0; r < MR; ++r) {
            if (r < T) {
                const int rg = t_base + r;
                const int xr_idx = a.x_row_mod > 0 ? rg % a.x_row_mod : rg;
                if constexpr (SL) R.x[r] = *reinterpret_cast<const float4*>(pX + xoff_sl[r] + k);
                else R.x[r] = *reinterpret_cast<const float4*>(pX + (unsigned)(xr_idx * pldx) + k);
                if constexpr (PARTS == 1) {
                    R.p0[r] = *reinterpret_cast<const float4*>(a.xa + (unsigned)(xr_idx * pldx) + k);
                    R.p1[r] = *reinterpret_cast<const float4*>(a.xa + (unsigned)(a.part_stride + xr_idx * pldx) + k);
                }
                if constexpr (PRO == VV_PRO_ADD_SILU) {
                    const int av = a.add_rows_per_vec > 0 ? rg / a.add_rows_per_vec : 0;
                    R.addv[r] = *reinterpret_cast<const float4*>(a.addvec + (unsigned)(av * pK) + k);
                }
                if constexpr (PRO == VV_PRO_RMS_MOD) {
                    R.sc[r] = *reinterpret_cast<const float4*>(a.mod_scale + (unsigned)(rg * a.ld_mod) + k);
                    R.sh[r] = *reinterpret_cast<const float4*>(a.mod_shift + (unsigned)(rg * a.ld_mod) + k);
                }
            }
        }
    };
    auto w_load = [&](unsigned ktb, u32x4 (&dst)[U][NM]) {
#pragma unroll
        for (int u = 0; u < U; ++u) {
            const unsigned kt = min(ktb + u, kt1 - 1);
            dst[u][0] = __builtin_nontemporal_load(wbase + kt * 64);
            if constexpr (DUAL) dst[u][1] = __builtin_nontemporal_load(wbase2 + kt * 64);
        }
    };
    XR R;
    u32x4 wA[U][NM], wB[U][NM];
    if (has_k) { x_load(kt0, R); w_load(kt0, wA); }
    __builtin_amdgcn_sched_barrier(0);
    VV_STAMP(1);
    float rs1 = 1.0f;
    if constexpr (PRO == VV_PRO_NORMDW) {
        float s1 = 0.f;
        for (unsigned ktb = kt0; ktb < kt1; ktb += U) {
            const unsigned k = ktb * 32 + kk;
            if (k < min(kt1 * 32, (unsigned)pK)) {
                const float4 v = *reinterpret_cast<const float4*>(pX + k);
                s1 += v.x * v.x + v.y * v.y + v.z * v.z + v.w * v.w;
            }
        }
        s1 = vv_wave_sum_dpp(s1);
        if (lane == 0) ssq1_sh[wave] = s1;
        __syncthreads();
        float tot = 0.f;
#pragma unroll
        for (int w = 0; w < WPB; ++w) tot += ssq1_sh[w];
        rs1 = rsqrtf(tot / (float)pK + a.eps);
    }

    const int n0 = tile * 16 + fq * 4;
    const bool epi_lane = (wave == 0) && frow < T && n0 < pN;
    float4 pre_y = {0.f, 0.f, 0.f, 0.f}, pre_b = {0.f, 0.f, 0.f, 0.f}, pre_g = {1.f, 1.f, 1.f, 1.f};
    float4 pre_y0 = {0.f, 0.f, 0.f, 0.f}, pre_y1 = {0.f, 0.f, 0.f, 0.f};
    unsigned yrow_off = (unsigned)((t_base + frow) * pldy);
    if constexpr (SL) {
        const int rg = min(t_base + frow, pT - 1);
        const int j = rg / a.sl_T, tt = rg - j * a.sl_T;
        yrow_off = a.sl_y ? (unsigned)(vv_slot_id(a.sl_id, j) * a.sl_y + tt * pldy) : (unsigned)(rg * pldy);
    }
    if (epi_lane) {
        if constexpr (EPI == VV_EPI_BIAS || EPI == VV_EPI_BIAS_GELU || EPI == VV_EPI_RESID) {
            if (a.bias) pre_b = *reinterpret_cast<const float4*>(a.bias + n0);
        }
        if constexpr (EPI == VV_EPI_RESID || EPI == VV_EPI_GATED_RESID) {
            pre_y = *reinterpret_cast<const float4*>(pY + (yrow_off + (unsigned)n0));
            if constexpr (PARTS == 2) {
                const float* yp0 = a.ya + (unsigned)((t_base + frow) * pldy + n0);
                pre_y0 = *reinterpret_cast<const float4*>(yp0);
                pre_y1 = *reinterpret_cast<const float4*>(yp0 + a.part_stride);
            }
            if constexpr (EPI == VV_EPI_GATED_RESID) pre_g = *reinterpret_cast<const float4*>(a.gate + (unsigned)((t_base + frow) * a.ld_gate + n0));
            else if (a.nscale) pre_g = *reinterpret_cast<const float4*>(a.nscale + n0);
        }
    }

    f32x4 acc[NM * NOP];
#pragma unroll
    for (int i = 0; i < NM * NOP; ++i) acc[i] = f32x4{0.f, 0.f, 0.f, 0.f};
    float ssq[MR];
#pragma unroll
    for (int r = 0; r < MR; ++r) ssq[r] = 0.f;

    auto x_stage = [&](unsigned ktb, const XR& R) {
        const unsigned k = ktb * 32 + kk;
        const float msk = (k < min(kt1 * 32, (unsigned)pK)) ? 1.f : 0.f;
#pragma unroll
        for (int r = 0; r < MR; ++r) {
            if (r < T) {
                float v[4] = {R.x[r].x, R.x[r].y, R.x[r].z, R.x[r].w};
                if constexpr (PARTS == 1) {
                    v[0] = (v[0] + R.p0[r].x) + R.p1[r].x; v[1] = (v[1] + R.p0[r].y) + R.p1[r].y;
                    v[2] = (v[2] + R.p0[r].z) + R.p1[r].z; v[3] = (v[3] + R.p0[r].w) + R.p1[r].w;
                }
                v[0] *= msk; v[1] *= msk; v[2] *= msk; v[3] *= msk;
                if constexpr (PRO == VV_PRO_RMS) {
                    ssq[r] += v[0] * v[0] + v[1] * v[1] + v[2] * v[2] + v[3] * v[3];
                    v[0] *= R.nwv.x; v[1] *= R.nwv.y; v[2] *= R.nwv.z; v[3] *= R.nwv.w;
                } else if constexpr (PRO == VV_PRO_NORMDW) {
                    if (r == 0) {
                        const float xn[4] = {R.dn.x, R.dn.y, R.dn.z, R.dn.w}, bb[4] = {R.db.x, R.db.y, R.db.z, R.db.w};
                        const float gg[4] = {R.dg.x, R.dg.y, R.dg.z, R.dg.w}, n2[4] = {R.nwv.x, R.nwv.y, R.nwv.z, R.nwv.w};
                        float hn[4], xo[4];
#pragma unroll
                        for (int e = 0; e < 4; ++e) {
                            hn[e] = v[e] * rs1 * xn[e];
                            float acc = bb[e];
#pragma unroll
                            for (int j = 0; j < 6; ++j) acc += reinterpret_cast<const float*>(&R.dt[j])[e] * reinterpret_cast<const float*>(&R.dh[j])[e];
                            acc += reinterpret_cast<const float*>(&R.dt[6])[e] * hn[e];
                            xo[e] = (v[e] + gg[e] * acc) * msk;
                        }
                        if (tile == 0 && msk != 0.f) {
                            *reinterpret_cast<float4*>(a.dw_xout + k) = float4{xo[0], xo[1], xo[2], xo[3]};
                            *reinterpret_cast<float4*>(a.dw_hnew + k) = float4{hn[0], hn[1], hn[2], hn[3]};
                        }
                        ssq[r] += xo[0] * xo[0] + xo[1] * xo[1] + xo[2] * xo[2] + xo[3] * xo[3];
#pragma unroll
                        for (int e = 0; e < 4; ++e) v[e] = xo[e] * n2[e];
                    }
                } else if constexpr (PRO == VV_PRO_RMS_MOD) {
                    ssq[r] += v[0] * v[0] + v[1] * v[1] + v[2] * v[2] + v[3] * v[3];
                    v[0] = (v[0] * R.nwv.x) * (1.f + R.sc[r].x); v[1] = (v[1] * R.nwv.y) * (1.f + R.sc[r].y);
                    v[2] = (v[2] * R.nwv.z) * (1.f + R.sc[r].z); v[3] = (v[3] * R.nwv.w) * (1.f + R.sc[r].w);
                    float sh4[4] = {R.sh[r].x * msk, R.sh[r].y * msk, R.sh[r].z * msk, R.sh[r].w * msk};
                    uint2 sparts[XS];
                    vv_split_bf16<XS>(sh4, sparts);
#pragma unroll
                    for (int p = 0; p < XS; ++p) {
                        if constexpr (FOLD) *reinterpret_cast<uint2*>(stg + p * (U * 4 * GSB) + st_off + (MR + r) * 16) = sparts[p];
                        else *reinterpret_cast<uint2*>(stg + (XS + p) * (U * 4 * GSB) + st_off + r * 16) = sparts[p];
                    }
                } else if constexpr (PRO == VV_PRO_ADD_SILU) {
                    v[0] = vv_silu(v[0] + R.addv[r].x) * msk; v[1] = vv_silu(v[1] + R.addv[r].y) * msk;
                    v[2] = vv_silu(v[2] + R.addv[r].z) * msk; v[3] = vv_silu(v[3] + R.addv[r].w) * msk;
                }
                uint2 parts[XS];
                vv_split_bf16<XS>(v, parts);
#pragma unroll
                for (int p = 0; p < XS; ++p)
                    *reinterpret_cast<uint2*>(stg + p * (U * 4 * GSB) + st_off + r * 16) = parts[p];
            }
        }
    };
    auto mma = [&](unsigned ktb, const u32x4 (&wb)[U][NM]) {
#pragma unroll
        for (int u = 0; u < U; ++u) {
            if (ktb + u < kt1) {
#pragma unroll
                for (int p = 0; p < XS; ++p) {
                    u32x4 f = u32x4{0u, 0u, 0u, 0u};
                    if (frow < MRS) f = *reinterpret_cast<const u32x4*>(stg + (size_t)((p * U + u) * 4 + fq) * GSB + frow * 16);
                    const bf16x8 xb = __builtin_bit_cast(bf16x8, f);
#pragma unroll
                    for (int i = 0; i < NM; ++i)
                        acc[i] = __builtin_amdgcn_mfma_f32_16x16x32_bf16(__builtin_bit_cast(bf16x8, wb[u][i]), xb, acc[i], 0, 0, 0);
                    if constexpr (NOP == 2) {
                        u32x4 f2 = u32x4{0u, 0u, 0u, 0u};
                        if (frow < MR) f2 = *reinterpret_cast<const u32x4*>(stg + (size_t)(((XS + p) * U + u) * 4 + fq) * GSB + frow * 16);
                        const bf16x8 sb = __builtin_bit_cast(bf16x8, f2);
#pragma unroll
                        for (int i = 0; i < NM; ++i)
                            acc[NM + i] = __builtin_amdgcn_mfma_f32_16x16x32_bf16(__builtin_bit_cast(bf16x8, wb[u][i]), sb, acc[NM + i], 0, 0, 0);
                    }
                }
            }
        }
    };

    if (has_k) {
        x_stage(kt0, R);
        VV_STAMP(2);
        if constexpr (DUAL) {
#pragma unroll 1
            for (unsigned ktb = kt0; ktb < kt1; ktb += U) {
                const bool n1 = ktb + U < kt1;
                if (n1) x_load(ktb + U, R);
                mma(ktb, wA);
                if (n1) { w_load(ktb + U, wA); x_stage(ktb + U, R); }
            }
        } else
#pragma unroll 1
        for (unsigned ktb = kt0; ktb < kt1; ktb += 2 * U) {
            const bool n1 = ktb + U < kt1, n2 = ktb + 2 * U < kt1;
            if (n1) { x_load(ktb + U, R); w_load(ktb + U, wB); }
            mma(ktb, wA);
            if (n1) x_stage(ktb + U, R);
            if (n2) { x_load(ktb + 2 * U, R); w_load(ktb + 2 * U, wA); }
            if (n1) mma(ktb + U, wB);
            if (n2) x_stage(ktb + 2 * U, R);
        }
    }

    VV_STAMP(3);
#pragma unroll
    for (int i = 0; i < NM * NOP; ++i) red[wave][i][lane] = acc[i];
    if constexpr (PRO == VV_PRO_RMS || PRO == VV_PRO_RMS_MOD || PRO == VV_PRO_NORMDW) {
#pragma unroll
        for (int r = 0; r < MR; ++r) {
            const float s = (r < T) ? vv_wave_sum_dpp(ssq[r]) : 0.f;
            if (lane == 0) ssq_sh[wave][r] = s;
        }
    }
    VV_STAMP(4);
    __syncthreads();
    VV_STAMP(5);
    if (wave != 0) return;
#pragma unroll
    for (int w = 1; w < WPB; ++w)
#pragma unroll
        for (int i = 0; i < NM * NOP; ++i) acc[i] += red[w][i][lane];
    f32x4 shf[FOLD ? NM : 1];
    if constexpr (FOLD) {
#pragma unroll
        for (int i = 0; i < NM; ++i)
#pragma unroll
            for (int r = 0; r < 4; ++r) {
                const float av = acc[i][r];
                const int sv = __builtin_amdgcn_update_dpp(0, __builtin_bit_cast(int, av), 0x100 + MR, 0xF, 0xF, true);
                shf[i][r] = __builtin_bit_cast(float, sv);
            }
    }
    if (!epi_lane) return;
    float rs = 1.0f;
    if constexpr (PRO == VV_PRO_RMS || PRO == VV_PRO_RMS_MOD || PRO == VV_PRO_NORMDW) {
        float s = 0.f;
#pragma unroll
        for (int w = 0; w < WPB; ++w) s += ssq_sh[w][frow];
        rs = rsqrtf(s / (float)pK + a.eps);
    }
    float o[4] = {acc[0][0] * rs, acc[0][1] * rs, acc[0][2] * rs, acc[0][3] * rs};
    float up[4] = {0.f, 0.f, 0.f, 0.f};
    if constexpr (DUAL) { up[0] = acc[1][0] * rs; up[1] = acc[1][1] * rs; up[2] = acc[1][2] * rs; up[3] = acc[1][3] * rs; }
    if constexpr (NOP == 2) {
#pragma unroll
        for (int r = 0; r < 4; ++r) { o[r] += acc[NM][r]; if constexpr (DUAL) up[r] += acc[NM + 1][r]; }
    }
    if constexpr (FOLD) {
#pragma unroll
        for (int r = 0; r < 4; ++r) { o[r] += shf[0][r]; if constexpr (DUAL) up[r] += shf[1][r]; }
    }
    const float pb[4] = {pre_b.x, pre_b.y, pre_b.z, pre_b.w};
    const float py[4] = {(pre_y.x + pre_y0.x) + pre_y1.x, (pre_y.y + pre_y0.y) + pre_y1.y, (pre_y.z + pre_y0.z) + pre_y1.z, (pre_y.w + pre_y0.w) + pre_y1.w};
    const float pg[4] = {pre_g.x, pre_g.y, pre_g.z, pre_g.w};
    if constexpr (EPI == VV_EPI_BIAS) {
#pragma unroll
        for (int r = 0; r < 4; ++r) o[r] += pb[r];
    } else if constexpr (EPI == VV_EPI_BIAS_GELU) {
#pragma unroll
        for (int r = 0; r < 4; ++r) o[r] = vv_gelu_erf(o[r] + pb[r]);
    } else if constexpr (EPI == VV_EPI_SWIGLU) {
#pragma unroll
        for (int r = 0; r < 4; ++r) o[r] = vv_silu(o[r]) * up[r];
    } else if constexpr (EPI == VV_EPI_RESID) {
#pragma unroll
        for (int r = 0; r < 4; ++r) o[r] = (ksb == 0) ? py[r] + pg[r] * (o[r] + pb[r]) : pg[r] * o[r];
    } else if constexpr (EPI == VV_EPI_GATED_RESID) {
#pragma unroll
        for (int r = 0; r < 4; ++r) o[r] = (ksb == 0) ? py[r] + pg[r] * o[r] : pg[r] * o[r];
    }
    if constexpr (EPI == VV_EPI_CFG_DPM) {
        const int nc = a.n_cfg;
        const VVSolverCoef cf = vv_solver_coef(a.coef, a.sde_noise != nullptr);
        float cfg = a.cfg;
        if (a.cfg_rows && frow < nc) cfg = a.cfg_rows[frow];
#pragma unroll
        for (int r = 0; r < 4; ++r) {
            const float vu = __shfl(o[r], lane + nc);
            const int n = n0 + r;
            if (frow < nc && n < pN) {
                const unsigned zi = (unsigned)(frow * pN + n);
                float x0, zn;
                vv_cfg_dpm_update(o[r], vu, cfg, a.z[zi], a.x0p[zi], cf, a.sde_noise != nullptr, [&] { return a.sde_noise[zi]; }, x0, zn);
                a.x0p[zi] = x0;
                a.z[zi] = zn;
                a.z[zi + (unsigned)(nc * pN)] = zn;
            }
        }
        return;
    }
    float* yp = (ksb == 0 ? pY : a.yparts + (unsigned)((ksb - 1) * a.part_stride)) + (yrow_off + (unsigned)n0);
    *reinterpret_cast<float4*>(yp) = float4{o[0], o[1], o[2], o[3]};
    VV_STAMP(6);
    VV_BSTAMP(1);
}

}

extern "C" int vv_gemv_ok(const VVGemm* a) { return vv_gemv_eligible(a); }

using GemvKernel = void (*)(const u32x4*, const u32x4*, const float*, float*, const float*, int, int, int, int, int, const VVGemm);
template <int F, int I, int XS>
static constexpr GemvKernel gemv_kernel_at() {
    constexpr const VVGemvFamily& f = vv_gemv_families[F];
    if constexpr (I < f.n && XS <= f.xs_max) return vv_gemv_kernel<XS, f.pair[I].pro, f.pair[I].epi, f.mr, f.wpb, f.parts, f.sl>;
    else return nullptr;
}
template <size_t... J>
static constexpr std::array<GemvKernel, sizeof...(J)> gemv_kernel_table(std::index_sequence<J...>) {
    return {gemv_kernel_at<J / (VV_GEMV_MAX_PAIRS * VV_GEMV_MAX_XS), J / VV_GEMV_MAX_XS % VV_GEMV_MAX_PAIRS, J % VV_GEMV_MAX_XS + 1>()...};
}
static const auto gemv_kernels = gemv_kernel_table(std::make_index_sequence<VV_GF_COUNT * VV_GEMV_MAX_PAIRS * VV_GEMV_MAX_XS>{});

static GemvKernel gemv_kernel(const VVGemvForm& form, int pro, int epi) {
    for (int f = 0; f < VV_GF_COUNT; ++f) {
        const VVGemvFamily& fam = vv_gemv_families[f];
        if (fam.mr != form.mr || fam.wpb != form.wpb || fam.parts != form.parts || fam.sl != form.sl || form.xs > fam.xs_max) continue;
        for (int i = 0; i < fam.n; ++i)
            if (fam.pair[i].pro == pro && fam.pair[i].epi == epi) return gemv_kernels[(f * VV_GEMV_MAX_PAIRS + i) * VV_GEMV_MAX_XS + form.xs - 1];
    }
    return nullptr;
}

extern "C" int vv_gemv_launch(VVGemm a, int xs, hipStream_t s, int* form) {
    if (a.epi == VV_EPI_SWIGLU && !a.W2) return -1;
    VVGemvPlan p;
    if (!vv_gemv_plan(&a, xs, &p)) return VV_RC_NO_FORM;
    const GemvKernel k = gemv_kernel(p.form, a.pro, a.epi);
    if (form) { form[0] = p.form.xs; form[1] = p.form.mr; form[2] = p.form.wpb; form[3] = p.form.parts; form[4] = p.form.sl; }
    hipLaunchKernelGGL(k, p.grid, dim3(p.form.wpb * 64), 0, s, a.W, a.W2, a.X, a.Y, a.nw, a.T, a.N, a.K, a.ldx, a.ldy, a);
    return vv_launch_rc(0);
}
```

vibevoice_amd/csrc/gemv16p.hip:

```cpp
#include <cstdlib>
#include "vv_common.h"
#include "vv_device.h"
#include "vv_launch.h"

namespace {

template <int MODE>
__global__ __launch_bounds__(256) void vv_pack16_kernel(const float* __restrict__ x, int ldx, const float* __restrict__ nw, float eps,
                                                        const float* __restrict__ sc, const float* __restrict__ sh, int ld_mod,
                                                        unsigned char* __restrict__ xp, int T, int K) {
    constexpr int MAXQ = 8;
    __shared__ float red[4];
    const int tid = threadIdx.x, lane = tid & 63, wave = tid >> 6;
    const int t = blockIdx.x;
    const int KT = K >> 5, K4 = K >> 2;
    float4 v[MAXQ];
    float ssq = 0.f;
#pragma unroll
    for (int i = 0; i < MAXQ; ++i) {
        const int q = tid + i * 256;
        v[i] = (t < T && q < K4) ? *reinterpret_cast<const float4*>(x + (int64_t)t * ldx + q * 4) : float4{0.f, 0.f, 0.f, 0.f};
        ssq += v[i].x * v[i].x + v[i].y * v[i].y + v[i].z * v[i].z + v[i].w * v[i].w;
    }
    ssq = vv_wave_sum(ssq);
// ... 139 lines not shown
        if constexpr (DUAL) {
#pragma unroll 1
            for (unsigned ktb = kt0; ktb < kt1; ktb += PU) {
                mma(ktb, wA, xA);
                if (ktb + PU < kt1) load(ktb + PU, wA, xA);
            }
        } else {
            u32x4 wB[PU][NM], xB[PU][NX];
#pragma unroll 1
            for (unsigned ktb = kt0; ktb < kt1; ktb += 2 * PU) {
                const bool n1 = ktb + PU < kt1, n2 = ktb + 2 * PU < kt1;
                if (n1) load(ktb + PU, wB, xB);
                mma(ktb, wA, xA);
                if (n2) load(ktb + 2 * PU, wA, xA);
                if (n1) mma(ktb + PU, wB, xB);
            }
        }
    }
#pragma unroll
    for (int i = 0; i < NA; ++i) red[wave][i][lane] = acc[i];
    __syncthreads();
    if (wave != 0) return;
#pragma unroll
    for (int w = 1; w < WPB; ++w)
#pragma unroll
        for (int i = 0; i < NA; ++i) acc[i] += red[w][i][lane];
    if constexpr (RS) {
        float s = 0.f;
#pragma unroll
        for (int w = 0; w < WPB; ++w) s += rs_sh[w][frow];
        const float rs = rsqrtf(s / (float)a.K + a.eps);
#pragma unroll
        for (int i = 0; i < NM; ++i) acc[i] *= rs;
    }
    if constexpr (SH) {
#pragma unroll
        for (int i = 0; i < NM; ++i) acc[i] += acc[NM + i];
    }
    if constexpr (PK) {
        float o[4];
        const float pb[4] = {pre_b.x, pre_b.y, pre_b.z, pre_b.w};
        const float py[4] = {pre_y.x, pre_y.y, pre_y.z, pre_y.w};
        const float pg[4] = {pre_g.x, pre_g.y, pre_g.z, pre_g.w};
        const float nw4[4] = {pre_nw.x, pre_nw.y, pre_nw.z, pre_nw.w}, sc4[4] = {pre_sc.x, pre_sc.y, pre_sc.z, pre_sc.w};
        float sq = 0.f;
        bf16x4 pk;
#pragma unroll
        for (int r = 0; r < 4; ++r) {
            if constexpr (EPI == VV_EPI_RESID) o[r] = py[r] + (acc[0][r] + pb[r]);
            else o[r] = py[r] + pg[r] * acc[0][r];
            if (!epi_lane) o[r] = 0.f;
            sq += o[r] * o[r];
            pk[r] = (__bf16)(o[r] * nw4[r] * (1.f + sc4[r]));
        }
        sq += __shfl_xor(sq, 16);
        sq += __shfl_xor(sq, 32);
        if (fq == 0) a.ssq_out[tile * 16 + frow] = sq;
        if (n0 < a.N) {
            const int64_t otile = n0 >> 5;
            const int ol = frow + 16 * ((n0 & 31) >> 3);
            *reinterpret_cast<uint2*>(a.Yp + ((otile * 64 + ol) * 16 + (n0 & 7) * 2)) = __builtin_bit_cast(uint2, pk);
            if (epi_lane) *reinterpret_cast<float4*>(a.Y + (size_t)frow * a.ldy + n0) = float4{o[0], o[1], o[2], o[3]};
        }
        return;
    }
    if (!epi_lane) return;
    if constexpr (EPI == VV_EPI_CFG_DPM) {
        const int nc = a.n_cfg;
        const VVSolverCoef cf = vv_solver_coef(a.coef, a.sde_noise != nullptr);
        float cfg = a.cfg;
        if (a.cfg_rows && frow < nc) cfg = a.cfg_rows[frow];
#pragma unroll
        for (int r = 0; r < 4; ++r) {
            const float oc = acc[0][r];
            const float vu = __shfl(oc, lane + nc);
            const int n = n0 + r;
            if (frow < nc && n < a.N) {
                const unsigned zi = (unsigned)(frow * a.N + n);
                float x0, zn;
                vv_cfg_dpm_update(oc, vu, cfg, a.z[zi], a.x0p[zi], cf, a.sde_noise != nullptr, [&] { return a.sde_noise[zi]; }, x0, zn);
                a.x0p[zi] = x0;
                a.z[zi] = zn;
                a.z[zi + (unsigned)(nc * a.N)] = zn;
            }
        }
        return;
    }
    if constexpr (DUAL) {
        bf16x4 o;
#pragma unroll
        for (int r = 0; r < 4; ++r) o[r] = (__bf16)(vv_silu(acc[0][r]) * acc[1][r]);
        const int64_t otile = n0 >> 5;
        const int ol = frow + 16 * ((n0 & 31) >> 3);
        *reinterpret_cast<uint2*>(a.Yp + ((otile * 64 + ol) * 16 + (n0 & 7) * 2)) = __builtin_bit_cast(uint2, o);
    } else {
        float o[4] = {acc[0][0], acc[0][1], acc[0][2], acc[0][3]};
        const float pb[4] = {pre_b.x, pre_b.y, pre_b.z, pre_b.w};
        const float py[4] = {pre_y.x, pre_y.y, pre_y.z, pre_y.w};
        const float pg[4] = {pre_g.x, pre_g.y, pre_g.z, pre_g.w};
#pragma unroll
        for (int r = 0; r < 4; ++r) {
            if constexpr (EPI == VV_EPI_BIAS) o[r] += pb[r];
            else if constexpr (EPI == VV_EPI_RESID) o[r] = py[r] + (o[r] + pb[r]);
            else o[r] = py[r] + pg[r] * o[r];
        }
        *reinterpret_cast<float4*>(a.Y + (size_t)frow * a.ldy + n0) = float4{o[0], o[1], o[2], o[3]};
    }
}

}

extern "C" {

int vv_pack16_launch(const float* x, int ldx, int mode, const float* nw, float eps, const float* sc, const float* sh, int ld_mod,
                     void* xp, int T, int K, hipStream_t s) {
    if (T < 1 || T > 16 || (K & 31) || K > 8192 || (ldx & 3) || (((uintptr_t)x) & 15) || mode < 1 || mode > 2 ||
        (mode == 2 && ((ld_mod & 3) || !sc || !sh))) return -1;
    if (mode == 2) hipLaunchKernelGGL((vv_pack16_kernel<2>), dim3(16), dim3(256), 0, s, x, ldx, nw, eps, sc, sh, ld_mod, (unsigned char*)xp, T, K);
    else hipLaunchKernelGGL((vv_pack16_kernel<1>), dim3(16), dim3(256), 0, s, x, ldx, nw, eps, sc, sh, ld_mod, (unsigned char*)xp, T, K);
    return vv_launch_rc(0);
}

int vv_pack16_tiles_launch(const float* x, int ldx, int64_t stride_outer, int n_inner, int64_t stride_inner, void* xp, int64_t tile_bytes,
                           int T, int K, int n_tiles, hipStream_t s) {
    if (T < 1 || T > 16 || (K & 31) || (ldx & 3) || (stride_outer & 3) || (stride_inner & 3) || (((uintptr_t)x) & 15) || n_inner < 1 || n_tiles < 1 ||
        n_tiles > 65535 || (tile_bytes & 15)) return -1;
    hipLaunchKernelGGL(vv_pack16_tiles_kernel, dim3(16, n_tiles), dim3(256), 0, s, x, ldx, stride_outer, n_inner, stride_inner, (unsigned char*)xp, tile_bytes, T, K);
    return vv_launch_rc(0);
}

int vv_gemv16p_launch2(const VVGemv16p* ap, int epi, int flags, hipStream_t s) {
    const VVGemv16p& a = *ap;
    if (a.T < 1 || a.T > 16 || (a.N & 3) || a.K < 32 || (a.K & 31)) return VV_RC_NO_FORM;
    const int n_tiles = (a.N + 15) / 16;
    if ((flags & 1) && (!a.ssq_in || a.ssq_tiles < 1 || (((uintptr_t)a.ssq_in) & 15))) return VV_RC_NO_FORM;
    if ((flags & 2) && !a.Xs) return VV_RC_NO_FORM;
    if ((flags & 4) && (!a.Yp || !a.ssq_out || !a.Y || (a.N & 15) || (a.ldy & 3) || (a.pk_sc && (a.ld_pk & 3)))) return VV_RC_NO_FORM;
    constexpr int wide_tiles = 256;
    const bool w4 = n_tiles > wide_tiles;
#define VV_P(E_, RS_, SH_, PK_) do { if (w4) hipLaunchKernelGGL((vv_gemv16p_kernel<E_, 4, RS_, SH_, PK_>), dim3(n_tiles), dim3(256), 0, s, a); \
                                   else hipLaunchKernelGGL((vv_gemv16p_kernel<E_, 8, RS_, SH_, PK_>), dim3(n_tiles), dim3(512), 0, s, a); return vv_launch_rc(0); } while (0)
    if (epi == VV_EPI_SWIGLU) {
        if (!a.W2 || !a.Yp || (a.N & 7)) return VV_RC_NO_FORM;
        if (flags == 0) VV_P(VV_EPI_SWIGLU, 0, 0, 0);
        if (flags == 1) VV_P(VV_EPI_SWIGLU, 1, 0, 0);
        if (flags == 3) VV_P(VV_EPI_SWIGLU, 1, 1, 0);
    } else if (epi == VV_EPI_BIAS || epi == VV_EPI_STORE) {
        if (!a.Y || (a.ldy & 3)) return VV_RC_NO_FORM;
        if (flags == 0) VV_P(VV_EPI_BIAS, 0, 0, 0);
        if (flags == 1) VV_P(VV_EPI_BIAS, 1, 0, 0);
        if (flags == 3) VV_P(VV_EPI_BIAS, 1, 1, 0);
    } else if (epi == VV_EPI_RESID) {
        if (!a.Y || (a.ldy & 3)) return VV_RC_NO_FORM;
        if (flags == 0) VV_P(VV_EPI_RESID, 0, 0, 0);
        if (flags == 4) VV_P(VV_EPI_RESID, 0, 0, 1);
    } else if (epi == VV_EPI_GATED_RESID) {
        if (!a.Y || !a.gate || (a.ldy & 3) || (a.ld_gate & 3)) return VV_RC_NO_FORM;
        if (flags == 0) VV_P(VV_EPI_GATED_RESID, 0, 0, 0);
        if (flags == 4) VV_P(VV_EPI_GATED_RESID, 0, 0, 1);
    } else if (epi == VV_EPI_CFG_DPM) {
        if (!a.z || !a.x0p || !a.coef || a.n_cfg < 1 || 2 * a.n_cfg != a.T) return VV_RC_NO_FORM;
        if (flags == 0) VV_P(VV_EPI_CFG_DPM, 0, 0, 0);
        if (flags == 3) VV_P(VV_EPI_CFG_DPM, 1, 1, 0);
    }
#undef VV_P
    return VV_RC_NO_FORM;
// ... 12 lines not shown
```

vibevoice_amd/csrc/gemv_plan.h:

```cpp
#pragma once
#include "vv_common.h"

struct VVGemvForm { int xs, mr, wpb, parts, sl; };
struct VVGemvPlan { VVGemvForm form; dim3 grid; };

struct VVGemvPair { int pro, epi; };
struct VVGemvFamily {
    int mr, wpb, parts, sl, xs_max, n;
    const VVGemvPair* pair;
    template <int N>
    constexpr VVGemvFamily(int mr_, int wpb_, int parts_, int sl_, int xs_max_, const VVGemvPair (&p)[N])
        : mr(mr_), wpb(wpb_), parts(parts_), sl(sl_), xs_max(xs_max_), n(N), pair(p) {}
    constexpr bool has(int pro, int epi) const {
        for (int i = 0; i < n; ++i) if (pair[i].pro == pro && pair[i].epi == epi) return true;
        return false;
    }
};
inline constexpr VVGemvPair vv_gemv_pairs[] = {
    {VV_PRO_NONE, VV_EPI_STORE}, {VV_PRO_NONE, VV_EPI_BIAS}, {VV_PRO_NONE, VV_EPI_RESID}, {VV_PRO_NONE, VV_EPI_GATED_RESID},
    {VV_PRO_RMS, VV_EPI_BIAS}, {VV_PRO_RMS, VV_EPI_BIAS_GELU}, {VV_PRO_RMS, VV_EPI_SWIGLU}, {VV_PRO_RMS, VV_EPI_RESID}, {VV_PRO_RMS, VV_EPI_STORE},
    {VV_PRO_RMS_MOD, VV_EPI_SWIGLU}, {VV_PRO_RMS_MOD, VV_EPI_CFG_DPM}, {VV_PRO_RMS_MOD, VV_EPI_STORE},
    {VV_PRO_ADD_SILU, VV_EPI_STORE}, {VV_PRO_NORMDW, VV_EPI_BIAS_GELU}};
inline constexpr VVGemvPair vv_gemv_pairs_w4[] = {
    {VV_PRO_RMS, VV_EPI_SWIGLU}, {VV_PRO_RMS_MOD, VV_EPI_SWIGLU}, {VV_PRO_RMS, VV_EPI_BIAS_GELU}, {VV_PRO_RMS, VV_EPI_BIAS},
    {VV_PRO_NONE, VV_EPI_STORE}, {VV_PRO_NONE, VV_EPI_BIAS}, {VV_PRO_ADD_SILU, VV_EPI_STORE}, {VV_PRO_NORMDW, VV_EPI_BIAS_GELU}};
inline constexpr VVGemvPair vv_gemv_pairs_w16[] = {
    {VV_PRO_NONE, VV_EPI_RESID}, {VV_PRO_NONE, VV_EPI_GATED_RESID}, {VV_PRO_NONE, VV_EPI_BIAS}, {VV_PRO_NONE, VV_EPI_STORE}};
inline constexpr VVGemvPair vv_gemv_pairs_wide[] = {
    {VV_PRO_NONE, VV_EPI_STORE}, {VV_PRO_NONE, VV_EPI_BIAS}, {VV_PRO_NONE, VV_EPI_RESID}, {VV_PRO_RMS, VV_EPI_BIAS},
    {VV_PRO_RMS, VV_EPI_BIAS_GELU}, {VV_PRO_RMS, VV_EPI_SWIGLU}, {VV_PRO_ADD_SILU, VV_EPI_STORE}, {VV_PRO_NONE, VV_EPI_GATED_RESID}};
inline constexpr VVGemvPair vv_gemv_pairs_wide4[] = {
    {VV_PRO_NONE, VV_EPI_STORE}, {VV_PRO_NONE, VV_EPI_BIAS}, {VV_PRO_NONE, VV_EPI_RESID}, {VV_PRO_RMS, VV_EPI_BIAS_GELU}};
inline constexpr VVGemvPair vv_gemv_pairs_wide_mod[] = {
    {VV_PRO_RMS_MOD, VV_EPI_SWIGLU}, {VV_PRO_RMS_MOD, VV_EPI_CFG_DPM}, {VV_PRO_RMS_MOD, VV_EPI_STORE}};
inline constexpr VVGemvPair vv_gemv_pairs_parts_x[] = {
    {VV_PRO_RMS, VV_EPI_BIAS}, {VV_PRO_RMS_MOD, VV_EPI_SWIGLU}, {VV_PRO_RMS_MOD, VV_EPI_CFG_DPM}, {VV_PRO_RMS_MOD, VV_EPI_STORE}};
inline constexpr VVGemvPair vv_gemv_pairs_parts_x_wide[] = {{VV_PRO_RMS_MOD, VV_EPI_SWIGLU}};
inline constexpr VVGemvPair vv_gemv_pairs_parts_y[] = {{VV_PRO_NONE, VV_EPI_RESID}, {VV_PRO_NONE, VV_EPI_GATED_RESID}};
inline constexpr VVGemvPair vv_gemv_pairs_slots[] = {{VV_PRO_NONE, VV_EPI_BIAS}, {VV_PRO_NONE, VV_EPI_RESID}, {VV_PRO_RMS, VV_EPI_BIAS_GELU}};

enum { VV_GF_DEFAULT, VV_GF_ROWS2_W4, VV_GF_ROWS4_W4, VV_GF_W16, VV_GF_WIDE, VV_GF_WIDE4, VV_GF_WIDE_MOD, VV_GF_PARTS_X, VV_GF_PARTS_X_ROWS2_W4,
       VV_GF_PARTS_X_W4, VV_GF_PARTS_Y, VV_GF_SLOTS, VV_GF_SLOTS4, VV_GF_COUNT };
constexpr int VV_GEMV_MAX_PAIRS = sizeof(vv_gemv_pairs) / sizeof(vv_gemv_pairs[0]), VV_GEMV_MAX_XS = 3;
inline constexpr VVGemvFamily vv_gemv_families[VV_GF_COUNT] = {
    {4, 8, 0, 0, 3, vv_gemv_pairs},
    {2, 4, 0, 0, 1, vv_gemv_pairs_w4},
    {4, 4, 0, 0, 1, vv_gemv_pairs_w4},
    {4, 16, 0, 0, 1, vv_gemv_pairs_w16},
    {16, 8, 0, 0, 2, vv_gemv_pairs_wide},
    {16, 4, 0, 0, 1, vv_gemv_pairs_wide4},
    {16, 4, 0, 0, 1, vv_gemv_pairs_wide_mod},
    {4, 8, 1, 0, 3, vv_gemv_pairs_parts_x},
    {2, 4, 1, 0, 1, vv_gemv_pairs_parts_x_wide},
    {4, 4, 1, 0, 1, vv_gemv_pairs_parts_x_wide},
    {4, 8, 2, 0, 3, vv_gemv_pairs_parts_y},
    {16, 8, 0, 1, 2, vv_gemv_pairs_slots},
    {16, 4, 0, 1, 1, vv_gemv_pairs_slots}};

inline bool vv_gemv_eligible(const VVGemm* a) {
    const VVGemvFamily* const fam = vv_gemv_families;
    if (a->T < 1) return false;
    if (a->T > 4 || a->sl_n > 0) { if (!fam[VV_GF_WIDE].has(a->pro, a->epi) && !fam[VV_GF_WIDE_MOD].has(a->pro, a->epi)) return false; }
    else if (!fam[VV_GF_DEFAULT].has(a->pro, a->epi)) return false;
    if (a->sl_n > 0) {
        if (a->sl_n > 8 || a->sl_T < 1 || a->T != a->sl_n * a->sl_T || a->sl_x < 0 || a->sl_y < 0 || (a->sl_x & 3) || (a->sl_y & 3)) return false;
        if (a->kgrid > 1 || a->n_xa || a->n_ya || a->x_row_mod > 0 || a->add_rows_per_vec > 0) return false;
        if (!fam[VV_GF_SLOTS].has(a->pro, a->epi)) return false;
        for (int j = 0; j < a->sl_n; ++j)
            if (a->sl_id[j] < 0 || (int64_t)a->sl_id[j] * a->sl_x + (int64_t)a->sl_T * a->ldx >= (1LL << 30) ||
                (int64_t)a->sl_id[j] * a->sl_y + (int64_t)a->sl_T * a->ldy >= (1LL << 30)) return false;
    }
    if ((a->x_row_mod > 0 || a->add_rows_per_vec > 0) && a->pro != VV_PRO_ADD_SILU) return false;
    if (a->epi == VV_EPI_CFG_DPM && (a->n_cfg < 1 || a->T != 2 * a->n_cfg || a->T > 16 || !a->z || !a->x0p || !a->coef)) return false;
    if (a->pro == VV_PRO_NORMDW) {
        if (a->T != 1 || a->sl_n > 0 || a->kgrid > 1 || a->n_xa || a->n_ya || !a->dw_hist || !a->dw_w || !a->dw_b || !a->dw_gamma ||
            !a->dw_nw || !a->dw_xout || !a->dw_hnew || a->dw_xout == a->X) return false;
        if ((((uintptr_t)a->dw_hist) | ((uintptr_t)a->dw_w) | ((uintptr_t)a->dw_b) | ((uintptr_t)a->dw_gamma) | ((uintptr_t)a->dw_nw) |
             ((uintptr_t)a->dw_xout) | ((uintptr_t)a->dw_hnew)) & 15) return false;
        if ((int64_t)7 * a->K >= (1LL << 30)) return false;
    }
    if ((a->K & 3) || (a->ldx & 3) || (((uintptr_t)a->X) & 15)) return false;
    if (a->pro == VV_PRO_RMS_MOD && (a->ld_mod & 3)) return false;
    if (a->nw && (((uintptr_t)a->nw) & 15)) return false;
    if (a->K < 32) return false;
    if ((int64_t)a->T * a->ldy >= (1LL << 30) || (int64_t)a->T * a->ldx >= (1LL << 30)) return false;
    if ((a->N & 3) || (a->ldy & 3)) return false;
    if ((((uintptr_t)a->Y) & 15) || (a->bias && (((uintptr_t)a->bias) & 15))) return false;
    if (a->nscale && (((uintptr_t)a->nscale) & 15)) return false;
    if (a->epi == VV_EPI_GATED_RESID && ((a->ld_gate & 3) || (((uintptr_t)a->gate) & 15))) return false;
    if (a->pro == VV_PRO_RMS_MOD && ((((uintptr_t)a->mod_scale) & 15) || (((uintptr_t)a->mod_shift) & 15))) return false;
    if (a->pro == VV_PRO_ADD_SILU && (((uintptr_t)a->addvec) & 15)) return false;
    if (a->kgrid > 1 && (a->T > 4 || a->kgrid != 3 || a->pro != VV_PRO_NONE || !a->yparts || (a->part_stride & 3) ||
                         (a->epi != VV_EPI_RESID && a->epi != VV_EPI_GATED_RESID) || (((uintptr_t)a->yparts) & 15))) return false;
    if ((a->n_xa > 0 && (!a->xa || (((uintptr_t)a->xa) & 15))) || (a->n_ya > 0 && (!a->ya || (((uintptr_t)a->ya) & 15)))) return false;
    if ((a->n_xa != 0 && a->n_xa != 2) || (a->n_ya != 0 && a->n_ya != 2) || (a->n_xa && a->n_ya)) return false;
    if ((a->n_xa || a->n_ya) && ((a->part_stride & 3) || a->T > 4 || !fam[a->n_xa > 0 ? VV_GF_PARTS_X : VV_GF_PARTS_Y].has(a->pro, a->epi))) return false;
    return true;
}

constexpr int VV_GEMV_WIDE_TILES = 256;
constexpr int VV_GEMV_W16_MAX_TILES = 128, VV_GEMV_W16_MIN_KTILES = 96;
constexpr int VV_GEMV_WIDE4_WGS = 128;

inline bool vv_gemv_plan(const VVGemm* a, int xs, VVGemvPlan* out) {
    if (!vv_gemv_eligible(a)) return false;
    const VVGemvFamily* const fam = vv_gemv_families;
    const int n_tiles = (a->N + 15) / 16, k_tiles = (a->K + 31) / 32;
    const bool rows16 = a->T > 4 || a->sl_n > 0;
    const int grid_y = rows16 ? (a->T + 15) / 16 : a->kgrid > 1 ? a->kgrid : 1;
    const auto fits = [&](int f) { return xs >= 1 && xs <= fam[f].xs_max && fam[f].has(a->pro, a->epi); };
    const bool wide = n_tiles > VV_GEMV_WIDE_TILES, wide4 = (int64_t)n_tiles * grid_y > VV_GEMV_WIDE4_WGS;
    int f = VV_GF_DEFAULT;
    if (a->sl_n > 0) f = wide4 && fits(VV_GF_SLOTS4) ? VV_GF_SLOTS4 : VV_GF_SLOTS;
    else if (rows16 && wide4 && fits(VV_GF_WIDE4)) f = VV_GF_WIDE4;
    else if (rows16) f = fits(VV_GF_WIDE) ? VV_GF_WIDE : VV_GF_WIDE_MOD;
    else if (a->n_xa > 0 && wide && a->T <= 2 && fits(VV_GF_PARTS_X_ROWS2_W4)) f = VV_GF_PARTS_X_ROWS2_W4;
    else if (a->n_xa > 0) f = wide && fits(VV_GF_PARTS_X_W4) ? VV_GF_PARTS_X_W4 : VV_GF_PARTS_X;
    else if (a->n_ya > 0) f = VV_GF_PARTS_Y;
    else if (a->kgrid > 1) f = VV_GF_DEFAULT;
    else if (wide && a->T <= 2 && fits(VV_GF_ROWS2_W4)) f = VV_GF_ROWS2_W4;
    else if (wide && fits(VV_GF_ROWS4_W4)) f = VV_GF_ROWS4_W4;
    else if (n_tiles <= VV_GEMV_W16_MAX_TILES && k_tiles >= VV_GEMV_W16_MIN_KTILES && fits(VV_GF_W16)) f = VV_GF_W16;
    if (!fits(f)) return false;
    out->form = {xs, fam[f].mr, fam[f].wpb, fam[f].parts, fam[f].sl};
    out->grid = dim3(n_tiles, grid_y);
    return true;
}

constexpr int VV_TILE_BM = 64;
#define VV_TILE_COMBOS(X)                                                                      \
    X(VV_PRO_NONE, VV_EPI_STORE) X(VV_PRO_NONE, VV_EPI_BIAS) X(VV_PRO_NONE, VV_EPI_RESID)      \
    X(VV_PRO_RMS, VV_EPI_BIAS) X(VV_PRO_RMS, VV_EPI_BIAS_GELU) X(VV_PRO_RMS, VV_EPI_SWIGLU)    \
    X(VV_PRO_RMS, VV_EPI_STORE)

inline bool vv_tile_eligible(const VVGemm* a, int xs) {
    if (a->T < 32 || xs > 2) return false;
    {
        const int per_wg = 4 * (a->epi == VV_EPI_SWIGLU ? 1 : 2);
        const int64_t wgs = (int64_t)(((a->N + 15) / 16 + per_wg - 1) / per_wg) * ((a->T + VV_TILE_BM - 1) / VV_TILE_BM);
        const int min_wgs = a->sl_n > 0 ? 40 : 48;
        if (wgs < min_wgs) return false;
    }
    if (a->sl_n > 0) {
        if (a->sl_n > 8 || a->sl_T < 1 || a->T != a->sl_n * a->sl_T || a->sl_x < 0 || a->sl_y < 0 || (a->sl_x & 3) || (a->sl_y & 3)) return false;
    }
    if ((a->K & 3) || (a->ldx & 3) || (a->N & 3) || (a->ldy & 3)) return false;
    if ((((uintptr_t)a->X) | ((uintptr_t)a->Y)) & 15) return false;
    if ((a->nw && (((uintptr_t)a->nw) & 15)) || (a->bias && (((uintptr_t)a->bias) & 15)) || (a->nscale && (((uintptr_t)a->nscale) & 15))) return false;
    if (a->x_row_mod > 0 || a->add_rows_per_vec > 0 || a->kgrid > 1 || a->n_xa > 0 || a->n_ya > 0 || a->ksplit > 0) return false;
    if (a->K < 32) return false;
    if (a->epi == VV_EPI_SWIGLU && !a->W2) return false;
#define X(P, E) if (a->pro == P && a->epi == E) return true;
    VV_TILE_COMBOS(X)
#undef X
    return false;
}

enum { VV_ROUTE_TILE, VV_ROUTE_GEMV, VV_ROUTE_GENERAL, VV_ROUTE_NONE };
inline int vv_gemm_route(const VVGemm* a, int xs) {
    VVGemvPlan p;
    if (vv_tile_eligible(a, xs)) return VV_ROUTE_TILE;
    if (a->sl_n > 0) return xs <= 2 && vv_gemv_plan(a, xs, &p) ? VV_ROUTE_GEMV : VV_ROUTE_NONE;
    if (a->ksplit <= 0 && vv_gemv_plan(a, xs, &p)) return VV_ROUTE_GEMV;
    if (a->kgrid > 1 || a->n_xa > 0 || a->n_ya > 0) return VV_ROUTE_NONE;
    return VV_ROUTE_GENERAL;
}

struct VVGemmGeneralPlan {
    bool vec, dual;
    int wpb, maxr, nt;
    int ks, t_pad;
    dim3 grid;
    size_t lds;
};
constexpr int VV_GG_NT2_TILE_PAIRS = 4096;
constexpr int VV_GG_WAVES = 2048, VV_GG_MIN_KSTEPS = 8;
constexpr int VV_GG_FEW_TILES = 512;
inline int vv_pow2_floor(int v) { int p = 1; while (p * 2 <= v) p *= 2; return p; }

inline int vv_gemm_general_plan(const VVGemm* a, int xs, VVGemmGeneralPlan* p) {
    const int n_tiles = (a->N + 15) / 16, k_tiles = (a->K + 31) / 32, t_tiles = (a->T + 15) / 16;
    p->dual = a->epi == VV_EPI_SWIGLU;
    if (p->dual && !a->W2) return -1;
    p->vec = ((a->K & 3) == 0) && ((a->ldx & 3) == 0) && ((((uintptr_t)a->X) & 15) == 0) && (a->pro != VV_PRO_RMS_MOD || (a->ld_mod & 3) == 0);
    if (!p->vec && p->dual) return VV_RC_NO_FORM;
    p->t_pad = a->T < 16 ? a->T : 16;
    p->wpb = (p->t_pad <= 4 && p->vec) ? 8 : 4;
    p->maxr = p->wpb == 8 ? 4 : 16;
    p->nt = (!p->dual && p->vec && (long)n_tiles * t_tiles >= VV_GG_NT2_TILE_PAIRS) ? 2 : 1;
    const long work = ((long)n_tiles + p->nt - 1) / p->nt * t_tiles;
    int ks = 1;
    if (a->ksplit > 0) ks = a->ksplit;
    else {
        const int want = (int)((VV_GG_WAVES + work - 1) / work);
        ks = vv_pow2_floor(want < 1 ? 1 : want);
        const int kmax = vv_pow2_floor(k_tiles / VV_GG_MIN_KSTEPS < 1 ? 1 : k_tiles / VV_GG_MIN_KSTEPS);
        if (ks > kmax) ks = kmax;
    }
    if (ks > p->wpb) ks = p->wpb;
    if (a->ksplit <= 0 && p->wpb == 8 && work < VV_GG_FEW_TILES) { while (ks < p->wpb && (k_tiles / (ks * 2)) >= 2) ks *= 2; }
    p->ks = ks;
    const int per_block = p->wpb / ks * p->nt;
    p->grid = dim3((n_tiles + per_block - 1) / per_block, t_tiles);
    const size_t stage_b = (size_t)p->wpb * xs * 8 * 4 * p->t_pad * 16;
    const size_t red_b = (size_t)p->wpb * (p->dual ? 2 : p->nt) * 64 * 16 + (size_t)p->wpb * 64 * 4;
    p->lds = stage_b > red_b ? stage_b : red_b;
    return 0;
}
```

vibevoice_amd/csrc/headtail.hip:

```cpp
#include "vv_common.h"
#include "vv_device.h"
#include "vv_launch.h"

namespace {

constexpr int TU = 8;
constexpr int WB = 4;
constexpr int KMAX = 16;

template <int TPW, int PARTS, int TR>
__global__ __launch_bounds__(512) void vv_head_tail_kernel(const VVTail a) {
    constexpr int WPB = 8, MR = 4, MRS = 8, GSB = MRS * 16, NT = 4;
    extern __shared__ __attribute__((aligned(16))) unsigned char smem[];
    unsigned char* const stg_all = smem;
    static_assert(KMAX * 4 * GSB >= NT * 64 * 16, "a wave's split-K partials re-use its own (by then idle) staging tile");
    unsigned char* const zfr = smem + WPB * KMAX * 4 * GSB;
    float (*ssq_sh)[MR] = reinterpret_cast<float (*)[MR]>(smem + WPB * KMAX * 4 * GSB + 2 * 1024);
    const int lane = threadIdx.x & 63;
    const int wave = __builtin_amdgcn_readfirstlane((int)(threadIdx.x >> 6));
    const int frow = lane & 15, fq = lane >> 4;
    const int T = a.T, H = a.H;
    const unsigned k_tiles = (unsigned)H >> 5;
    const unsigned kper = (k_tiles + WPB - 1) / WPB;
    const unsigned kt0 = wave * kper, kt1 = min(k_tiles, kt0 + kper);
    const unsigned nk = (kt1 > kt0) ? kt1 - kt0 : 0u;
    asm volatile("" ::"s"(a.coef), "s"(a.z_in), "s"(a.x0p_in), "s"(a.sde_noise), "s"(a.z_out), "s"(a.x0p_out), "s"(a.Xout), "s"(a.cfg), "s"(a.cfg_rows));
    u32x4 wA[WB][NT], wB[WB][NT];
    auto w_load = [&](unsigned kb, u32x4 (&w)[WB][NT]) {
#pragma unroll
        for (int u = 0; u < WB; ++u) {
            const unsigned kt = min(kt0 + kb + u, kt1 - 1);
#pragma unroll
            for (int nt = 0; nt < NT; ++nt) w[u][nt] = a.Wout[((size_t)nt * k_tiles + kt) * 64 + lane];
        }
    };
    const int tile_in = blockIdx.x * TPW + wave;
    const bool has_in = wave < TPW && tile_in * 16 < H;
    u32x4 win[2] = {u32x4{0u, 0u, 0u, 0u}, u32x4{0u, 0u, 0u, 0u}};
    float4 bin4 = {0.f, 0.f, 0.f, 0.f};
    const int n_in = tile_in * 16 + fq * 4;
    if (has_in) {
        win[0] = a.Win[((size_t)tile_in * 2 + 0) * 64 + lane];
        win[1] = a.Win[((size_t)tile_in * 2 + 1) * 64 + lane];
        if (a.bin) bin4 = *reinterpret_cast<const float4*>(a.bin + n_in);
    }
    const int nc = a.n_cfg;
    float4 pz = {0.f, 0.f, 0.f, 0.f}, px = {0.f, 0.f, 0.f, 0.f}, pn = {0.f, 0.f, 0.f, 0.f};
    float cf[6] = {0.f, 0.f, 0.f, 0.f, 0.f, 0.f};
    float cfg = a.cfg;
    if (wave < NT) {
#pragma unroll
        for (int i = 0; i < 6; ++i) cf[i] = a.coef[i];
        if (frow < nc) {
            if (a.cfg_rows) cfg = a.cfg_rows[frow];
            const unsigned zi = (unsigned)(frow * a.L + wave * 16 + fq * 4);
            pz = *reinterpret_cast<const float4*>(a.z_in + zi);
            px = *reinterpret_cast<const float4*>(a.x0p_in + zi);
            if (a.sde_noise) pn = *reinterpret_cast<const float4*>(a.sde_noise + zi);
        }
    }
    unsigned char* stg = stg_all + (size_t)wave * (KMAX * 4 * GSB);
    const unsigned kk = lane * 4;
    const unsigned st_off = ((kk >> 5) * 4 + ((kk & 31) >> 3)) * GSB + (kk & 7) * 2;
    float ssq[MR] = {0.f, 0.f, 0.f, 0.f};
    constexpr int NP = KMAX / TU;
    static_assert(TR == 2 || TR == 4, "rows");
    float4 rx[NP][TR], rsc[NP][TR], rsh[NP][TR];
    float rmsk[NP];
#pragma unroll
    for (int pass = 0; pass < NP; ++pass) {
        const unsigned ktb = kt0 + pass * TU;
        unsigned k = ktb * 32 + kk;
        const bool kin = ktb < kt1 && k < min(kt1 * 32, (unsigned)H);
        if (!kin) k = 0;
        rmsk[pass] = kin ? 1.f : 0.f;
#pragma unroll
        for (int r = 0; r < TR; ++r) {
            rx[pass][r] = rsc[pass][r] = rsh[pass][r] = float4{0.f, 0.f, 0.f, 0.f};
            if (r < T && ktb < kt1) {
                float4 x4 = *reinterpret_cast<const float4*>(a.X + (unsigned)(r * H) + k);
                if constexpr (PARTS) {
                    const float4 p0 = *reinterpret_cast<const float4*>(a.xa + (unsigned)(r * H) + k);
                    const float4 p1 = *reinterpret_cast<const float4*>(a.xa + (unsigned)(a.part_stride + r * H) + k);
                    x4.x = (x4.x + p0.x) + p1.x; x4.y = (x4.y + p0.y) + p1.y; x4.z = (x4.z + p0.z) + p1.z; x4.w = (x4.w + p0.w) + p1.w;
                }
                rx[pass][r] = x4;
                rsc[pass][r] = *reinterpret_cast<const float4*>(a.sc + (unsigned)(r * a.ld_mod) + k);
                rsh[pass][r] = *reinterpret_cast<const float4*>(a.sh + (unsigned)(r * a.ld_mod) + k);
            }
        }
    }
    if (nk) { w_load(0, wA); if (nk > WB) w_load(WB, wB); }
    __builtin_amdgcn_sched_barrier(0);
#pragma unroll
    for (int pass = 0; pass < NP; ++pass) {
        const unsigned ktb = kt0 + pass * TU;
        if (ktb < kt1) {
            const float msk = rmsk[pass];
            unsigned char* sp = stg + (size_t)pass * (TU * 4 * GSB);
#pragma unroll
            for (int r = 0; r < TR; ++r) {
                if (r < T) {
                    const float4 x4 = rx[pass][r], s4 = rsc[pass][r], h4 = rsh[pass][r];
                    float v[4] = {x4.x * msk, x4.y * msk, x4.z * msk, x4.w * msk};
                    ssq[r] += v[0] * v[0] + v[1] * v[1] + v[2] * v[2] + v[3] * v[3];
                    bf16x4 xb, sb;
                    xb[0] = (__bf16)(v[0] * (1.f + s4.x)); xb[1] = (__bf16)(v[1] * (1.f + s4.y));
                    xb[2] = (__bf16)(v[2] * (1.f + s4.z)); xb[3] = (__bf16)(v[3] * (1.f + s4.w));
                    sb[0] = (__bf16)(h4.x * msk); sb[1] = (__bf16)(h4.y * msk); sb[2] = (__bf16)(h4.z * msk); sb[3] = (__bf16)(h4.w * msk);
                    *reinterpret_cast<uint2*>(sp + st_off + r * 16) = __builtin_bit_cast(uint2, xb);
                    *reinterpret_cast<uint2*>(sp + st_off + (MR + r) * 16) = __builtin_bit_cast(uint2, sb);
                }
            }
        }
    }
    f32x4 acc[NT];
#pragma unroll
    for (int i = 0; i < NT; ++i) acc[i] = f32x4{0.f, 0.f, 0.f, 0.f};
    auto mma = [&](unsigned kb, const u32x4 (&w)[WB][NT]) {
#pragma unroll
        for (int u = 0; u < WB; ++u) {
            if (kb + u < nk) {
                u32x4 f = u32x4{0u, 0u, 0u, 0u};
                if (frow < MRS) f = *reinterpret_cast<const u32x4*>(stg + (size_t)((kb + u) * 4 + fq) * GSB + frow * 16);
                const bf16x8 xb = __builtin_bit_cast(bf16x8, f);
#pragma unroll
                for (int nt = 0; nt < NT; ++nt)
                    acc[nt] = __builtin_amdgcn_mfma_f32_16x16x32_bf16(__builtin_bit_cast(bf16x8, w[u][nt]), xb, acc[nt], 0, 0, 0);
            }
        }
    };
#pragma unroll 1
    for (unsigned kb = 0; kb < nk; kb += 2 * WB) {
        mma(kb, wA);
        if (kb + 2 * WB < nk) w_load(kb + 2 * WB, wA);
        if (kb + WB < nk) mma(kb + WB, wB);
        if (kb + 3 * WB < nk) w_load(kb + 3 * WB, wB);
    }
#pragma unroll
    for (int nt = 0; nt < NT; ++nt) reinterpret_cast<f32x4*>(stg)[nt * 64 + lane] = acc[nt];
#pragma unroll
    for (int r = 0; r < MR; ++r) {
        const float s = (r < T) ? vv_wave_sum(ssq[r]) : 0.f;
        if (lane == 0) ssq_sh[wave][r] = s;
    }
    __syncthreads();
    if (wave < NT) {
        const int nt = wave;
        f32x4 e = reinterpret_cast<const f32x4*>(stg_all)[nt * 64 + lane];
#pragma unroll
        for (int w = 1; w < WPB; ++w) e += reinterpret_cast<const f32x4*>(stg_all + (size_t)w * (KMAX * 4 * GSB))[nt * 64 + lane];
        float s = 0.f;
#pragma unroll
        for (int w = 0; w < WPB; ++w) s += ssq_sh[w][frow & 3];
        const float rs = rsqrtf(s / (float)H + a.eps);
        const float ca = cf[0], cs_ = cf[1], csx = cf[2], c0 = cf[3], c1 = cf[4];
        const float cn = a.sde_noise ? cf[5] : 0.f;
        bf16x4 zb;
#pragma unroll
        for (int r = 0; r < 4; ++r) {
            const float av = e[r];
            const int sv = __builtin_amdgcn_update_dpp(0, __builtin_bit_cast(int, av), 0x100 + MR, 0xF, 0xF, true);
            const float o = av * rs + __builtin_bit_cast(float, sv);
            const int oi = __builtin_bit_cast(int, o);
            const int ui = (nc == 1) ? __builtin_amdgcn_update_dpp(0, oi, 0x101, 0xF, 0xF, true) : __builtin_amdgcn_update_dpp(0, oi, 0x102, 0xF, 0xF, true);
            const float vu = __builtin_bit_cast(float, ui);
            const int d = nt * 16 + fq * 4 + r;
            float zn = 0.f;
            if (frow < nc) {
                const float v = vu + cfg * (o - vu);
                const unsigned zi = (unsigned)(frow * a.L + d);
                const float zo = reinterpret_cast<const float*>(&pz)[r];
                const float x0 = ca * zo - cs_ * v;
                zn = csx * zo + c0 * x0 + c1 * (x0 - reinterpret_cast<const float*>(&px)[r]);
                if (a.sde_noise) zn += cn * reinterpret_cast<const float*>(&pn)[r];
                if (blockIdx.x == 0) {
                    a.x0p_out[zi] = x0;
                    a.z_out[zi] = zn;
                    a.z_out[zi + (unsigned)(nc * a.L)] = zn;
                }
            }
            zb[r] = (__bf16)zn;
        }
        if (frow < nc) {
            const int d0 = nt * 16 + fq * 4;
            const int off = (((d0 >> 5) * 64 + frow + 16 * ((d0 & 31) >> 3)) * 8 + (d0 & 7)) * 2;
            *reinterpret_cast<uint2*>(zfr + off) = __builtin_bit_cast(uint2, zb);
            *reinterpret_cast<uint2*>(zfr + off + nc * 16) = __builtin_bit_cast(uint2, zb);
        }
    }
    __syncthreads();
    if (!has_in) return;
    f32x4 y = f32x4{0.f, 0.f, 0.f, 0.f};
#pragma unroll
    for (int kt = 0; kt < 2; ++kt) {
        u32x4 f = u32x4{0u, 0u, 0u, 0u};
        if (frow < T) f = *reinterpret_cast<const u32x4*>(zfr + ((size_t)kt * 64 + lane) * 16);
        y = __builtin_amdgcn_mfma_f32_16x16x32_bf16(__builtin_bit_cast(bf16x8, win[kt]), __builtin_bit_cast(bf16x8, f), y, 0, 0, 0);
    }
    if (frow < T && n_in < H)
        *reinterpret_cast<float4*>(a.Xout + (size_t)frow * H + n_in) = float4{y[0] + bin4.x, y[1] + bin4.y, y[2] + bin4.z, y[3] + bin4.w};
}

}

extern "C" int vv_head_tail_ok(const VVTail* a) {
    if (a->T != 2 || a->T != 2 * a->n_cfg ||       a->L != 64 || (a->H & 31) || a->H < 256 || a->H > 8 * 16 * 32) return 0;
    if (!a->Wout || !a->Win || !a->X || !a->sc || !a->sh || !a->Xout || !a->z_in || !a->x0p_in || !a->z_out || !a->x0p_out || !a->coef) return 0;
    if (a->X == a->Xout || a->z_in == a->z_out || a->x0p_in == a->x0p_out) return 0;
    if ((a->ld_mod & 3) || ((((uintptr_t)a->X) | ((uintptr_t)a->sc) | ((uintptr_t)a->sh) | ((uintptr_t)a->Xout)) & 15)) return 0;
    if (a->bin && (((uintptr_t)a->bin) & 15)) return 0;
    if (a->n_xa != 0 && (a->n_xa != 2 || !a->xa || (((uintptr_t)a->xa) & 15) || (a->part_stride & 3))) return 0;
    if ((int64_t)a->T * a->ld_mod >= (1LL << 30) || (int64_t)a->T * a->H >= (1LL << 30)) return 0;
    return 1;
}

constexpr int HT_TPW = 4;
constexpr size_t HT_SMEM = 8 * KMAX * 4 * 128 + 2 * 1024 + 8 * 4 * sizeof(float);

extern "C" int vv_head_tail_init() {
    if (vv_raise_lds_limit((int)HT_SMEM, &vv_head_tail_kernel<HT_TPW, 1, 2>, &vv_head_tail_kernel<HT_TPW, 0, 2>) != hipSuccess) { (void)hipGetLastError(); return -1; }
    return 0;
}

extern "C" int vv_head_tail_launch(const VVTail* ap, hipStream_t s) {
    if (!vv_head_tail_ok(ap)) return -3;
    const VVTail& a = *ap;
    const dim3 grid((a.H / 16 + HT_TPW - 1) / HT_TPW);
    if (a.n_xa) hipLaunchKernelGGL((vv_head_tail_kernel<HT_TPW, 1, 2>), grid, dim3(512), HT_SMEM, s, a);
    else hipLaunchKernelGGL((vv_head_tail_kernel<HT_TPW, 0, 2>), grid, dim3(512), HT_SMEM, s, a);
    return vv_launch_rc(0);
}
```

vibevoice_amd/csrc/pass_plan.h:

```cpp
#pragma once
#include "vv_common.h"

constexpr int VV_P16_MIN_ROWS = 5, VV_P16_MAX_ROWS = 16;
inline bool vv_p16_rows(int rows) { return rows >= VV_P16_MIN_ROWS && rows <= VV_P16_MAX_ROWS; }

constexpr int VV_ATTN_SPLIT_POS = 1024;
constexpr int VV_ATTN_TARGET_WGS = 256;
constexpr int VV_CHUNK_MIN_ROWS = 8;
constexpr int VV_PREFILL_MIN_ROWS = 64;

enum { VV_LM_PREFILL, VV_LM_P16, VV_LM_GEMV };
enum { VV_ATTN_FUSED, VV_ATTN_PREFILL4, VV_ATTN_SPLIT_MERGE };

struct VVLmCaps { int ws_rows, attn_splits, Hkv; bool tile3_ok, attn2_ok, p16_ok; };

struct VVLmPlan {
    bool fused;
    bool contiguous;
    int route, attn;
    int attn_S;
    int attn_groups;
    bool zero_v_tail;
    int key_mode, key_split;
    int64_t kv_positions;
};

inline int vv_lm_pass_plan(const VVRow* rows, int n_rows, const VVLmCaps& c, VVLmPlan* p) {
    bool fused = true;
    for (int i = 0; i < n_rows && fused; ++i)
        for (int j = 0; j < i; ++j) if (rows[i].cache == rows[j].cache) { fused = false; break; }
    bool contiguous = !fused && n_rows >= VV_CHUNK_MIN_ROWS;
    for (int i = 1; i < n_rows && contiguous; ++i)
        if (rows[i].cache != rows[0].cache || rows[i].pos != rows[0].pos + i) contiguous = false;
    p->fused = fused; p->contiguous = contiguous;
    if (!contiguous && n_rows > c.ws_rows) return -1;
    int max_len = 1, n_long = 0;
    int64_t kv_positions = 0;
    for (int i = 0; i < n_rows; ++i) {
        const int len = rows[i].pos + 1;
        if (len > max_len) max_len = len;
        if (len > VV_ATTN_SPLIT_POS) ++n_long;
        kv_positions += len;
    }
    const int long_wgs = (n_long > 1 ? n_long : 1) * c.Hkv;
    int S = (VV_ATTN_TARGET_WGS + long_wgs - 1) / long_wgs;
    if (S < 1) S = 1;
    if (S > c.attn_splits) S = c.attn_splits;
    const int by_len = (max_len + VV_ATTN_SPLIT_POS - 1) / VV_ATTN_SPLIT_POS;
    if (S > by_len) S = by_len;
    p->attn_S = S;
    p->kv_positions = kv_positions;
    const bool chunk_attn = contiguous && c.attn2_ok;
    if (contiguous && c.tile3_ok && n_rows >= VV_PREFILL_MIN_ROWS) { p->route = VV_LM_PREFILL; p->attn = VV_ATTN_PREFILL4; }
    else {
        p->route = vv_p16_rows(n_rows) && c.p16_ok && fused ? VV_LM_P16 : VV_LM_GEMV;
        p->attn = fused ? VV_ATTN_FUSED : chunk_attn ? VV_ATTN_PREFILL4 : VV_ATTN_SPLIT_MERGE;
    }
    p->attn_groups = p->attn == VV_ATTN_SPLIT_MERGE ? (n_rows + c.ws_rows - 1) / c.ws_rows : 0;
    p->zero_v_tail = p->route == VV_LM_PREFILL || chunk_attn;
    p->key_mode = fused ? 1 : (contiguous ? 2 : 0);
    p->key_split = chunk_attn ? 0 : S;
    return 0;
}

constexpr int VV_ADA_TILE_ABOVE_ROWS = 32;

enum { VV_ADA_PER_STEP, VV_ADA_TILE, VV_ADA_ROWS16 };
enum { VV_HEAD_P16, VV_HEAD_GEMV };
enum { VV_FINAL_P16_CFG,
       VV_FINAL_SEAM,
       VV_FINAL_GEMM_CFG,
       VV_FINAL_GEMM };

struct VVHeadCaps { bool p16_ok, p16_shift, ada_p, mod_all, head_tail; };

struct VVHeadPlan {
    int rows, n_steps;
    int ada;
    bool sh_tiles;
    int layers;
    bool seam;
    int final_stage;
    bool solver_step;
};

inline VVHeadPlan vv_head_plan(int rows, int n_steps, int HF, int HL, int MODW, const VVHeadCaps& c, bool has_coef, bool solver_step = false) {
    VVHeadPlan p;
    p.rows = rows; p.n_steps = n_steps;
    const bool batch_ada = has_coef && c.mod_all;
    p.ada = !batch_ada ? VV_ADA_PER_STEP : (c.ada_p && rows * n_steps > VV_ADA_TILE_ABOVE_ROWS && (MODW & 3) == 0) ? VV_ADA_TILE : VV_ADA_ROWS16;
    p.sh_tiles = batch_ada && vv_p16_rows(rows) && c.p16_shift;
    p.layers = vv_p16_rows(rows) && c.p16_ok && (HF % 32) == 0 ? VV_HEAD_P16 : VV_HEAD_GEMV;
    p.seam = has_coef && rows == 2 && c.head_tail;
    p.final_stage = p.layers == VV_HEAD_P16 && p.sh_tiles && has_coef && HL > 0 ? VV_FINAL_P16_CFG : has_coef ? VV_FINAL_GEMM_CFG : VV_FINAL_GEMM;
    p.solver_step = solver_step;
    if (solver_step) { p.sh_tiles = false; p.seam = false; p.final_stage = VV_FINAL_GEMM; }
    return p;
}
inline int vv_head_final(const VVHeadPlan& p, int step) { return p.seam && step + 1 < p.n_steps ? VV_FINAL_SEAM : p.final_stage; }
```

vibevoice_amd/csrc/vv_common.h:

```cpp
#pragma once
#include <hip/hip_runtime.h>
#include <stdint.h>

typedef __attribute__((ext_vector_type(8))) __bf16 bf16x8;
typedef __attribute__((ext_vector_type(4))) __bf16 bf16x4;
typedef __attribute__((ext_vector_type(2))) __bf16 bf16x2;
typedef __attribute__((ext_vector_type(4))) float f32x4;
typedef __attribute__((ext_vector_type(2))) float f32x2;
typedef __attribute__((ext_vector_type(4))) unsigned int u32x4;

#define VV_WAVE 64

static inline __host__ __device__ int64_t vv_packed_elems(int N, int K) {
    return (int64_t)((N + 15) / 16) * ((K + 31) / 32) * 512;
}

struct VVRow {
    int cache;
    int pos;
};

struct VVGemmWs {
    float* partials;
    unsigned* flags;
    unsigned* err;
    float* g3_partials;
    size_t g3_bytes;
};

enum { VV_PRO_NONE = 0, VV_PRO_RMS = 1, VV_PRO_RMS_MOD = 2, VV_PRO_ADD_SILU = 3,
       VV_PRO_NORMDW = 4 };
enum { VV_EPI_STORE = 0, VV_EPI_BIAS = 1, VV_EPI_BIAS_GELU = 2, VV_EPI_SWIGLU = 3,
       VV_EPI_RESID = 4, VV_EPI_GATED_RESID = 5, VV_EPI_CFG_DPM = 6,
       VV_EPI_QKV_ROPE = 7 };

struct VVGemm {
    const u32x4* W;
    const u32x4* W2;
    const float* X;
    float* Y;
    const float* nw;
    const float* mod_scale;
    const float* mod_shift;
    const float* addvec;
    const float* bias;
    const float* nscale;
    const float* gate;
    int T, N, K;
    int ldx, ldy, ld_mod, ld_gate;
    int pro, epi;
    int ksplit;
    int nt;
    int t_pad;
    float* z;
    float* x0p;
    const float* coef;
    float cfg;
    int n_cfg;
    const float* cfg_rows;
    const float* sde_noise;
    unsigned long long* dbg;
    int x_row_mod, add_rows_per_vec;
    float eps;
    int kgrid;
    float* yparts;
    const float* xa;
    const float* ya;
    int n_xa, n_ya;
    int part_stride;
    int sl_n, sl_T, sl_x, sl_y;
    int sl_id[8];
    const float* dw_hist;
    const float* dw_w;
    const float* dw_b;
    const float* dw_gamma;
    const float* dw_nw;
    float* dw_xout;
    float* dw_hnew;
};

struct VVGemv16p {
    const u32x4* W;
    const u32x4* W2;
    const u32x4* Xp;
    float* Y;
    unsigned char* Yp;
    const float* bias;
    const float* gate;
    int T, N, K, ldy, ld_gate;
    const float* ssq_in;
    int ssq_tiles;
    float eps;
    const u32x4* Xs;
    const float* pk_nw;
    const float* pk_sc;
    int ld_pk;
    float* ssq_out;
    float* z; float* x0p; const float* coef; float cfg; int n_cfg; const float* sde_noise;
    const float* cfg_rows;
};

struct VVTail {
    const u32x4* Wout;
    const u32x4* Win;
    const float* bin;
    const float* X;
    const float* xa; int n_xa, part_stride;
    const float* sc; const float* sh; int ld_mod;
    float* Xout;
    const float* z_in; const float* x0p_in;
    float* z_out; float* x0p_out;
    const float* coef; float cfg; int n_cfg; const float* sde_noise;
    const float* cfg_rows;
    int T, H, L; float eps;
};

struct VVSlotIds { int n; int id[8]; };
static inline VVSlotIds vv_slot_ids(const int* ids, int n) {
    VVSlotIds sl; sl.n = ids ? n : 0;
    for (int i = 0; i < 8; ++i) sl.id[i] = (ids && i < n) ? ids[i] : 0;
    return sl;
}
__device__ __forceinline__ int vv_slot_id(const int (&id)[8], int j) {
    int r = id[0];
#pragma unroll
    for (int i = 1; i < 8; ++i) r = (j == i) ? id[i] : r;
    return r;
}

struct VVRsRow { int stream, n_in, n_out, p0, b0; };
struct VVRsRows { VVRsRow r[16]; };
constexpr int VV_RS_MAX_OUT = 8192;

struct VVTpRow { long long k0, base; int stream, n_in, nblk, n_out, P, Q; };
struct VVTpRows { VVTpRow r[16]; };
constexpr int VV_TP_HS = 240, VV_TP_N = 480, VV_TP_DELTA = 160;
constexpr int VV_TP_HIST = 1280;
constexpr int VV_TP_MAX_IN = 7680;
constexpr int VV_TP_PAD = 896;
constexpr int VV_TP_BUF = VV_TP_HIST + VV_TP_MAX_IN + VV_TP_PAD;
constexpr int VV_TP_MAX_BLOCKS = 96;

struct VVLvRow { int stream, n_in, n_out, b0; float gain; };
struct VVLvRows { VVLvRow r[16]; };
constexpr int VV_LV_BUF = 8128;
constexpr int VV_LV_MAX_A = 2047;

template <class... K>
static inline hipError_t vv_raise_lds_limit(int bytes, K*... kernels) {
    hipError_t rc = hipSuccess;
    for (const void* k : {reinterpret_cast<const void*>(kernels)...}) {
        const hipError_t e = hipFuncSetAttribute(k, hipFuncAttributeMaxDynamicSharedMemorySize, bytes);
        if (rc == hipSuccess) rc = e;
    }
    return rc;
}

enum { VV_RC_NO_FORM = -3, VV_RC_NO_KERNEL = -4 };

inline thread_local int g_vv_launch_err = 0;
static inline int vv_launch_rc(int rc_ok) {
    const hipError_t e = hipGetLastError();
    if (e == hipSuccess) return rc_ok;
    g_vv_launch_err = (int)e;
    return -2;
}
```

Measured before the change: 16.46.

## Fold head final projection into last layer GEMV epilogue and drop output copy

Adds a gated-residual epilogue variant that, for the last head layer, also computes per-tile partial products of the modulated activations against the final linear weight with MFMA and stores them with sum-of-squares partials. The seam tail kernel can then reduce these partials instead of re-reading the full activation and output weight. Separately, the final diffusion step writes its latent straight into the caller's output buffer, which removes a trailing device copy. The fold path only runs when VVHIP_HEAD_FOLD=1, so by default just the copy elimination takes effect.

```diff
diff --git a/vibevoice_amd/csrc/engine.hip b/vibevoice_amd/csrc/engine.hip
--- a/vibevoice_amd/csrc/engine.hip
+++ b/vibevoice_amd/csrc/engine.hip
@@ -82,9 +82,7 @@
     return g;
 }
 int ksplit_parts(const vv_ctx* ctx, VVGemm& g, float* parts, int part_stride) {
-    const int n_tiles = (g.N + 15) / 16, k_tiles = (g.K + 31) / 32;
-    constexpr int max_tiles = 128;
-    if (g.T > 4 || n_tiles > max_tiles || k_tiles < 96) return 0;
+    if (!vv_ksplit_shape(g.T, g.N, g.K)) return 0;
     const int ks = 3;
     g.kgrid = ks; g.yparts = parts; g.part_stride = part_stride;
     if (!vv_gemv_ok(&g)) { g.kgrid = 0; g.yparts = nullptr; g.part_stride = 0; return 0; }
@@ -306,6 +304,10 @@
     }
     ctx->head_tail = c.xsplit == 1 && L == 64 && (H % 32) == 0 && vv_head_tail_init() == 0;
     if (const char* e = getenv("VVHIP_SOLVER_FUSE"); e && e[0] == '0') ctx->solver_fuse = false;
+    if (const char* e = getenv("VVHIP_HEAD_FOLD"); ctx->head_tail && (H % 32) == 0 && e && e[0] == '1') {
+        for (HeadGen& g : ctx->hg) g.fold = (float*)dalloc(ctx, vv_fold_floats(H / 16) * 4, false);
+        ctx->head_fold = ctx->hg[0].fold && ctx->hg[1].fold;
+    }
     if (const char* e = getenv("VVHIP_NAN_PROBE"); e && e[0] == '1') {
         ctx->probe_rec = (unsigned*)dalloc(ctx, PROBE_MAX * 16);
         ctx->probe_on = ctx->probe_rec != nullptr;
@@ -542,6 +544,8 @@
         case 5: return ctx->foreign_nodes;
         case 4: return ctx->capture_fallbacks;
         case 6: return ctx->seam_launches;
+        case 9: return ctx->fold_seams;
+        case 10: return ctx->out_copies;
         case 8: return ctx->solver_fused;
         case 7: return ctx->lora_base_bytes;
         default: return (int64_t)ctx->graphs.size();
diff --git a/vibevoice_amd/csrc/engine_ctx.h b/vibevoice_amd/csrc/engine_ctx.h
--- a/vibevoice_amd/csrc/engine_ctx.h
+++ b/vibevoice_amd/csrc/engine_ctx.h
@@ -76,7 +76,7 @@
 
 struct GraphEntry { hipGraphExec_t exec; uint64_t last_use; };
 
-struct HeadGen { float *xh = nullptr, *zz = nullptr, *x0p = nullptr, *m2 = nullptr; };
+struct HeadGen { float *xh = nullptr, *zz = nullptr, *x0p = nullptr, *m2 = nullptr, *fold = nullptr; };
 
 }
 using namespace vv_engine;
@@ -127,6 +127,7 @@
     float *cproj = nullptr, *mod = nullptr, *hact = nullptr, *eps = nullptr;
     HeadGen hg[2];
     bool head_tail = false;
+    bool head_fold = false;
     bool solver_fuse = true;
     float *tmp1 = nullptr, *tmp2 = nullptr;
     struct Conn { void *fc1, *fc2; float *b1, *b2, *norm; } ac_conn, sem_conn;
@@ -161,6 +162,8 @@
     Level lv[N_LEVELS];
     int64_t launches = 0;
     int64_t solver_fused = 0;
+    int64_t out_copies = 0;
+    int64_t fold_seams = 0;
     int64_t seam_launches = 0;
     bool prof_on = false;
     std::vector<hipEvent_t> prof_ev;
diff --git a/vibevoice_amd/csrc/engine_head.hip b/vibevoice_amd/csrc/engine_head.hip
--- a/vibevoice_amd/csrc/engine_head.hip
+++ b/vibevoice_amd/csrc/engine_head.hip
@@ -70,11 +70,11 @@
 
 static VVHeadPlan head_plan(const vv_ctx* ctx, int rows, int n_steps, bool has_coef) {
     return vv_head_plan(rows, n_steps, ctx->HF, ctx->c.head_layers, ctx->MODW,
-                        {ctx->p16_ok, ctx->p16_shift != nullptr, ctx->ada_p != nullptr, ctx->mod_all_bytes != 0, ctx->head_tail}, has_coef,
-                        has_coef && ctx->general_on);
-}
-
-struct StepEnd { const float* coef; float cfg; const float *cfg_rows, *noise; };
+                        {ctx->p16_ok, ctx->p16_shift != nullptr, ctx->ada_p != nullptr, ctx->mod_all_bytes != 0, ctx->head_tail, ctx->head_fold},
+                        has_coef, has_coef && ctx->general_on, ctx->H);
+}
+
+struct StepEnd { const float* coef; float cfg; const float *cfg_rows, *noise; float* out; };
 struct HeadStep {
     int step;
     const float *z, *temb, *mod;
@@ -105,6 +105,19 @@
     }
     int xp = 0;
     const int xps = 16 * H;
+    const float* fb = mod + (size_t)HL * 3 * H;
+    auto mk_tail = [&](int parts, const float* fold) {
+        VVTail t{};
+        t.Wout = (const u32x4*)ctx->h_out; t.Win = (const u32x4*)ctx->h_in; t.bin = nullptr;
+        t.X = xh; t.xa = ctx->xh_parts + (size_t)(HL & 1) * 2 * xps; t.n_xa = parts; t.part_stride = xps;
+        t.sc = fb + H; t.sh = fb; t.ld_mod = MODW;
+        t.Xout = s.nxt.xh;
+        t.z_in = s.cur.zz; t.x0p_in = s.cur.x0p; t.z_out = s.nxt.zz; t.x0p_out = s.nxt.x0p; put_end(t);
+        t.T = rows; t.H = H; t.L = L; t.eps = c.head_eps;
+        t.fold = fold;
+        return t;
+    };
+    bool folded = false;
     for (int l = 0; l < HL; ++l) {
         const float* base = mod + (size_t)l * 3 * H;
         if (p.layers == VV_HEAD_P16) {
@@ -131,6 +144,13 @@
         g2.epi = VV_EPI_GATED_RESID; g2.gate = base + 2 * H; g2.ld_gate = MODW; g2.nt = 1;
         g2.ya = cur; g2.n_ya = xp; g2.part_stride = xps;
         xp = ksplit_parts(ctx, g2, nxt, xps);
+        if (l + 1 == HL && xp == 0 && vv_head_fold(p, s.step)) {
+            VVGemm gf2 = g2;
+            gf2.epi = VV_EPI_GATED_RESID_FOLD;
+            gf2.fold_w = (const u32x4*)ctx->h_out; gf2.fold_sc = fb + H; gf2.fold_sh = fb; gf2.fold_ld = MODW; gf2.fold_out = s.cur.fold;
+            const VVTail tf = mk_tail(0, s.cur.fold);
+            if (L == 64 && vv_gemm_route(&gf2, c.xsplit) == VV_ROUTE_GEMV && vv_head_tail_ok(&tf)) { g2 = gf2; folded = true; }
+        }
         if (ctx->probe_on) { char nm[64]; snprintf(nm, 64, "layer %d hact (parts in %d)", l, g1.n_xa); nan_probe(ctx, st, nm, ctx->hact, (size_t)rows * HF); }
         GEMM(g2);
         if (ctx->probe_on) {
@@ -138,30 +158,26 @@
             for (int q = 0; q < xp; ++q) { snprintf(nm, 64, "layer %d part %d", l, q); nan_probe(ctx, st, nm, nxt + (size_t)q * xps, (size_t)rows * H); }
         }
     }
-    const float* fb = mod + (size_t)HL * 3 * H;
     if (final_stage == VV_FINAL_P16_CFG) {
         ctx->launches += 1;
         VVGemv16p af = p16_args(ctx->h_out, nullptr, ctx->p16_x, nullptr, nullptr, rows, L, H, L);
         af.ssq_in = ctx->ssq_a; af.ssq_tiles = H / 16; af.eps = c.head_eps;
         af.Xs = (const u32x4*)(s.sh_tiles + (size_t)HL * ctx->p16_shift_tile);
-        af.z = s.cur.zz; af.x0p = s.cur.x0p; put_end(af);
+        af.z = s.cur.zz; af.x0p = s.cur.x0p; af.z_copy = end.out; put_end(af);
         VVCHK(p16_go(ctx, st, af, VV_EPI_CFG_DPM, 3));
         return 0;
     }
     if (final_stage == VV_FINAL_SEAM) {
-        VVTail t{};
-        t.Wout = (const u32x4*)ctx->h_out; t.Win = (const u32x4*)ctx->h_in; t.bin = nullptr;
-        t.X = xh; t.xa = ctx->xh_parts + (size_t)(HL & 1) * 2 * xps; t.n_xa = xp; t.part_stride = xps;
-        t.sc = fb + H; t.sh = fb; t.ld_mod = MODW;
-        t.Xout = s.nxt.xh;
-        t.z_in = s.cur.zz; t.x0p_in = s.cur.x0p; t.z_out = s.nxt.zz; t.x0p_out = s.nxt.x0p; put_end(t);
-        t.T = rows; t.H = H; t.L = L; t.eps = c.head_eps;
+        const VVTail t = mk_tail(xp, folded ? s.cur.fold : nullptr);
         if (vv_head_tail_ok(&t)) {
             ctx->launches++;
             ctx->seam_launches++;
+            ctx->fold_seams += folded;
             if (ctx->prof_on) {
                 const VVTail tc = t;
-                ctx->prof_other.push_back({3, (double)vv_packed_elems(L, H) * 2.0 + (double)vv_packed_elems(H, L) * 2.0 + (double)rows * H * 8.0,
+                const double in_b = (double)vv_packed_elems(H, L) * 2.0;
+                const double bytes = folded ? in_b + (double)vv_fold_floats(H / 16) * 4.0 : in_b + (double)vv_packed_elems(L, H) * 2.0 + (double)rows * H * 8.0;
+                ctx->prof_other.push_back({3, bytes,
                                            [=](hipStream_t s2) { return vv_head_tail_launch(&tc, s2); }});
             }
             VVCHK(vv_head_tail_launch(&t, st));
@@ -172,7 +188,7 @@
     gf.pro = VV_PRO_RMS_MOD; gf.nw = nullptr; gf.eps = c.head_eps; gf.mod_shift = fb; gf.mod_scale = fb + H; gf.ld_mod = MODW;
     gf.xa = ctx->xh_parts + (size_t)(HL & 1) * 2 * xps; gf.n_xa = xp; gf.part_stride = xps;
     if (final_stage != VV_FINAL_GEMM) {
-        gf.epi = VV_EPI_CFG_DPM; gf.z = s.cur.zz; gf.x0p = s.cur.x0p; put_end(gf);
+        gf.epi = VV_EPI_CFG_DPM; gf.z = s.cur.zz; gf.x0p = s.cur.x0p; gf.z_copy = end.out; put_end(gf);
     }
     GEMM(gf);
     return 0;
@@ -183,7 +199,8 @@
 
 static StepDone step_shipped(vv_ctx* ctx, hipStream_t st, const VVHeadPlan& p, const SampleReq& r, HeadStep s) {
     const StepEnd end{ctx->coef + s.step * 8, r.cfg, r.cfg_rows,
-                      r.step_noise ? r.step_noise + (size_t)s.step * r.n * ctx->c.latent_dim : nullptr};
+                      r.step_noise ? r.step_noise + (size_t)s.step * r.n * ctx->c.latent_dim : nullptr,
+                      s.step + 1 == p.n_steps ? r.out : nullptr};
     s.end = &end;
     const int hr = head_eval(ctx, st, p, s);
     return {hr, hr == 1};
@@ -209,7 +226,7 @@
 static int sample_body(vv_ctx* ctx, hipStream_t st, const SampleReq& r) {
     const int H = ctx->H, L = ctx->c.latent_dim, HL = ctx->c.head_layers;
     const int n = r.n, rows = 2 * n;
-    ctx->seam_launches = ctx->solver_fused = 0;
+    ctx->seam_launches = ctx->fold_seams = ctx->solver_fused = ctx->out_copies = 0;
     ctx->probe_names.clear();
     nan_probe(ctx, st, "cond (input)", r.cond, (size_t)rows * H);
     nan_probe(ctx, st, "noise (input)", r.noise, (size_t)n * L);
@@ -262,7 +279,7 @@
             if (!p.solver_step && have_x) { snprintf(nm, 64, "step %d next xh", i); nan_probe(ctx, st, nm, now.xh, (size_t)rows * H); }
         }
     }
-    VVCHK(vv_copy_launch(r.out, ctx->hg[gen].zz, (size_t)n * L * 4, st));
+    if (p.solver_step) { ctx->out_copies++; VVCHK(vv_copy_launch(r.out, ctx->hg[gen].zz, (size_t)n * L * 4, st)); }
     return 0;
 }
 
diff --git a/vibevoice_amd/csrc/engine_prof.hip b/vibevoice_amd/csrc/engine_prof.hip
--- a/vibevoice_amd/csrc/engine_prof.hip
+++ b/vibevoice_amd/csrc/engine_prof.hip
@@ -46,7 +46,7 @@
 static double gemm_bytes(const VVGemm& g) {
     double w = (double)vv_packed_elems(g.N, g.K) * 2.0 * (g.W2 ? 2.0 : 1.0);
     double x = (double)g.T * g.K * 4.0;
-    double y = (double)g.T * g.N * 4.0 * ((g.epi == VV_EPI_RESID || g.epi == VV_EPI_GATED_RESID) ? 2.0 : 1.0);
+    double y = (double)g.T * g.N * 4.0 * ((g.epi == VV_EPI_RESID || g.epi == VV_EPI_GATED_RESID || g.epi == VV_EPI_GATED_RESID_FOLD) ? 2.0 : 1.0);
     return w + x + y;
 }
 int gemm_prof(vv_ctx* ctx, const VVGemm& g, hipStream_t st) {
diff --git a/vibevoice_amd/csrc/gemm.hip b/vibevoice_amd/csrc/gemm.hip
--- a/vibevoice_amd/csrc/gemm.hip
+++ b/vibevoice_amd/csrc/gemm.hip
@@ -315,6 +315,7 @@
                     a.x0p[zi] = x0;
                     a.z[zi] = zn;
                     a.z[zi + (int64_t)nc * a.N] = zn;
+                    if (a.z_copy) a.z_copy[zi] = zn;
                 }
             }
             continue;
diff --git a/vibevoice_amd/csrc/gemv.hip b/vibevoice_amd/csrc/gemv.hip
--- a/vibevoice_amd/csrc/gemv.hip
+++ b/vibevoice_amd/csrc/gemv.hip
@@ -23,6 +23,8 @@
                                                            const float* __restrict__ pnw, int pT, int pN, int pK, int pldx,
                                                            int pldy, const VVGemm a) {
     constexpr bool DUAL = (EPI == VV_EPI_SWIGLU);
+    constexpr bool EFOLD = (EPI == VV_EPI_GATED_RESID_FOLD), GATED = (EPI == VV_EPI_GATED_RESID) || EFOLD;
+    static_assert(!EFOLD || (XS == 1 && MR == 4 && PRO == VV_PRO_NONE && PARTS == 0 && SL == 0), "the fold epilogue: bf16 mode, the plain decode family");
     constexpr int NM = DUAL ? 2 : 1;
     constexpr bool FOLD = (PRO == VV_PRO_RMS_MOD) && MR <= 4;
     constexpr int NOP = (PRO == VV_PRO_RMS_MOD && !FOLD) ? 2 : 1;
@@ -36,7 +38,8 @@
     asm volatile("" ::"s"(a.ld_mod), "s"(a.ld_gate), "s"(a.x_row_mod), "s"(a.add_rows_per_vec),
                  "s"(a.eps), "s"(a.z), "s"(a.x0p), "s"(a.coef), "s"(a.cfg), "s"(a.n_cfg));
     asm volatile("" ::"s"(a.yparts), "s"(a.xa), "s"(a.ya), "s"(a.n_xa), "s"(a.n_ya), "s"(a.part_stride));
-    if constexpr (EPI == VV_EPI_CFG_DPM) asm volatile("" ::"s"(a.sde_noise), "s"(a.cfg_rows));
+    if constexpr (EPI == VV_EPI_CFG_DPM) asm volatile("" ::"s"(a.sde_noise), "s"(a.cfg_rows), "s"(a.z_copy));
+    if constexpr (EFOLD) asm volatile("" ::"s"(a.fold_w), "s"(a.fold_sc), "s"(a.fold_sh), "s"(a.fold_ld), "s"(a.fold_out));
     VV_STAMP(0);
     VV_BSTAMP(0);
     const int lane = threadIdx.x & 63;
@@ -158,15 +161,30 @@
         if constexpr (EPI == VV_EPI_BIAS || EPI == VV_EPI_BIAS_GELU || EPI == VV_EPI_RESID) {
             if (a.bias) pre_b = *reinterpret_cast<const float4*>(a.bias + n0);
         }
-        if constexpr (EPI == VV_EPI_RESID || EPI == VV_EPI_GATED_RESID) {
+        if constexpr (EPI == VV_EPI_RESID || GATED) {
             pre_y = *reinterpret_cast<const float4*>(pY + (yrow_off + (unsigned)n0));
             if constexpr (PARTS == 2) {
                 const float* yp0 = a.ya + (unsigned)((t_base + frow) * pldy + n0);
                 pre_y0 = *reinterpret_cast<const float4*>(yp0);
                 pre_y1 = *reinterpret_cast<const float4*>(yp0 + a.part_stride);
             }
-            if constexpr (EPI == VV_EPI_GATED_RESID) pre_g = *reinterpret_cast<const float4*>(a.gate + (unsigned)((t_base + frow) * a.ld_gate + n0));
+            if constexpr (GATED) pre_g = *reinterpret_cast<const float4*>(a.gate + (unsigned)((t_base + frow) * a.ld_gate + n0));
             else if (a.nscale) pre_g = *reinterpret_cast<const float4*>(a.nscale + n0);
+        }
+    }
+    float4 fold_sc4 = {0.f, 0.f, 0.f, 0.f}, fold_sh4 = {0.f, 0.f, 0.f, 0.f};
+    u32x4 fold_wf[EFOLD ? 4 : 1];
+    if constexpr (EFOLD) {
+#pragma unroll
+        for (int nt = 0; nt < 4; ++nt) fold_wf[nt] = u32x4{0u, 0u, 0u, 0u};
+        if (epi_lane) {
+            fold_sc4 = *reinterpret_cast<const float4*>(a.fold_sc + (unsigned)(frow * a.fold_ld + n0));
+            fold_sh4 = *reinterpret_cast<const float4*>(a.fold_sh + (unsigned)(frow * a.fold_ld + n0));
+        }
+        if (wave == 0 && fq < 2) {
+            const unsigned kto = (unsigned)(pN + 31) >> 5;
+#pragma unroll
+            for (int nt = 0; nt < 4; ++nt) fold_wf[nt] = a.fold_w[(nt * kto + (tile >> 1)) * 64 + (tile & 1) * 32 + lane];
         }
     }
 
@@ -316,7 +334,7 @@
                 shf[i][r] = __builtin_bit_cast(float, sv);
             }
     }
-    if (!epi_lane) return;
+    if constexpr (!EFOLD) { if (!epi_lane) return; }
     float rs = 1.0f;
     if constexpr (PRO == VV_PRO_RMS || PRO == VV_PRO_RMS_MOD || PRO == VV_PRO_NORMDW) {
         float s = 0.f;
@@ -350,9 +368,41 @@
     } else if constexpr (EPI == VV_EPI_RESID) {
 #pragma unroll
         for (int r = 0; r < 4; ++r) o[r] = (ksb == 0) ? py[r] + pg[r] * (o[r] + pb[r]) : pg[r] * o[r];
-    } else if constexpr (EPI == VV_EPI_GATED_RESID) {
+    } else if constexpr (GATED) {
 #pragma unroll
         for (int r = 0; r < 4; ++r) o[r] = (ksb == 0) ? py[r] + pg[r] * o[r] : pg[r] * o[r];
+    }
+    if constexpr (EFOLD) {
+        if (epi_lane) *reinterpret_cast<float4*>(pY + (yrow_off + (unsigned)n0)) = float4{o[0], o[1], o[2], o[3]};
+        const float sc4[4] = {fold_sc4.x, fold_sc4.y, fold_sc4.z, fold_sc4.w}, sh4[4] = {fold_sh4.x, fold_sh4.y, fold_sh4.z, fold_sh4.w};
+        bf16x4 xb, sb;
+        float sq = 0.f;
+#pragma unroll
+        for (int r = 0; r < 4; ++r) {
+            const float xv = epi_lane ? o[r] : 0.f;
+            sq += xv * xv;
+            xb[r] = (__bf16)(xv * (1.f + sc4[r]));
+            sb[r] = (__bf16)sh4[r];
+        }
+        sq += __shfl_xor(sq, 16);
+        sq += __shfl_xor(sq, 32);
+        const uint2 xq = __builtin_bit_cast(uint2, xb), hq = __builtin_bit_cast(uint2, sb);
+        const int src = (frow & (MR - 1)) + 32 * (fq & 1);
+        const u32x4 fx = {(unsigned)__shfl((int)xq.x, src), (unsigned)__shfl((int)xq.y, src), (unsigned)__shfl((int)xq.x, src + 16), (unsigned)__shfl((int)xq.y, src + 16)};
+        const u32x4 fh = {(unsigned)__shfl((int)hq.x, src), (unsigned)__shfl((int)hq.y, src), (unsigned)__shfl((int)hq.x, src + 16), (unsigned)__shfl((int)hq.y, src + 16)};
+        u32x4 fb = u32x4{0u, 0u, 0u, 0u};
+        if (fq < 2 && frow < MR) fb = fx;
+        if (fq < 2 && frow >= MR && frow < 2 * MR) fb = fh;
+        const int frw = frow & (MR - 1), term = frow >> 2;
+        float* const fo = a.fold_out + (size_t)tile * VV_FOLD_TILE + (unsigned)((term * 2 + frw) * 64 + fq * 4);
+#pragma unroll
+        for (int nt = 0; nt < 4; ++nt) {
+            const f32x4 d = __builtin_amdgcn_mfma_f32_16x16x32_bf16(__builtin_bit_cast(bf16x8, fold_wf[nt]), __builtin_bit_cast(bf16x8, fb),
+                                                                    f32x4{0.f, 0.f, 0.f, 0.f}, 0, 0, 0);
+            if (frow < 2 * MR && frw < 2) *reinterpret_cast<float4*>(fo + nt * 16) = float4{d[0], d[1], d[2], d[3]};
+        }
+        if (lane < 2) a.fold_out[vv_fold_ssq_off(pN >> 4) + tile * 2 + lane] = sq;
+        return;
     }
     if constexpr (EPI == VV_EPI_CFG_DPM) {
         const int nc = a.n_cfg;
@@ -370,6 +420,7 @@
                 a.x0p[zi] = x0;
                 a.z[zi] = zn;
                 a.z[zi + (unsigned)(nc * pN)] = zn;
+                if (a.z_copy) a.z_copy[zi] = zn;
             }
         }
         return;
@@ -388,7 +439,7 @@
 template <int F, int I, int XS>
 static constexpr GemvKernel gemv_kernel_at() {
     constexpr const VVGemvFamily& f = vv_gemv_families[F];
-    if constexpr (I < f.n && XS <= f.xs_max) return vv_gemv_kernel<XS, f.pair[I].pro, f.pair[I].epi, f.mr, f.wpb, f.parts, f.sl>;
+    if constexpr (I < f.n && XS <= f.xs_max && (f.pair[I].epi != VV_EPI_GATED_RESID_FOLD || XS == 1)) return vv_gemv_kernel<XS, f.pair[I].pro, f.pair[I].epi, f.mr, f.wpb, f.parts, f.sl>;
     else return nullptr;
 }
 template <size_t... J>
diff --git a/vibevoice_amd/csrc/gemv16p.hip b/vibevoice_amd/csrc/gemv16p.hip
--- a/vibevoice_amd/csrc/gemv16p.hip
+++ b/vibevoice_amd/csrc/gemv16p.hip
@@ -245,6 +245,7 @@
                 a.x0p[zi] = x0;
                 a.z[zi] = zn;
                 a.z[zi + (unsigned)(nc * a.N)] = zn;
+                if (a.z_copy) a.z_copy[zi] = zn;
             }
         }
         return;
diff --git a/vibevoice_amd/csrc/gemv_plan.h b/vibevoice_amd/csrc/gemv_plan.h
--- a/vibevoice_amd/csrc/gemv_plan.h
+++ b/vibevoice_amd/csrc/gemv_plan.h
@@ -20,7 +20,8 @@
     {VV_PRO_NONE, VV_EPI_STORE}, {VV_PRO_NONE, VV_EPI_BIAS}, {VV_PRO_NONE, VV_EPI_RESID}, {VV_PRO_NONE, VV_EPI_GATED_RESID},
     {VV_PRO_RMS, VV_EPI_BIAS}, {VV_PRO_RMS, VV_EPI_BIAS_GELU}, {VV_PRO_RMS, VV_EPI_SWIGLU}, {VV_PRO_RMS, VV_EPI_RESID}, {VV_PRO_RMS, VV_EPI_STORE},
     {VV_PRO_RMS_MOD, VV_EPI_SWIGLU}, {VV_PRO_RMS_MOD, VV_EPI_CFG_DPM}, {VV_PRO_RMS_MOD, VV_EPI_STORE},
-    {VV_PRO_ADD_SILU, VV_EPI_STORE}, {VV_PRO_NORMDW, VV_EPI_BIAS_GELU}};
+    {VV_PRO_ADD_SILU, VV_EPI_STORE}, {VV_PRO_NORMDW, VV_EPI_BIAS_GELU},
+    {VV_PRO_NONE, VV_EPI_GATED_RESID_FOLD}};
 inline constexpr VVGemvPair vv_gemv_pairs_w4[] = {
     {VV_PRO_RMS, VV_EPI_SWIGLU}, {VV_PRO_RMS_MOD, VV_EPI_SWIGLU}, {VV_PRO_RMS, VV_EPI_BIAS_GELU}, {VV_PRO_RMS, VV_EPI_BIAS},
     {VV_PRO_NONE, VV_EPI_STORE}, {VV_PRO_NONE, VV_EPI_BIAS}, {VV_PRO_ADD_SILU, VV_EPI_STORE}, {VV_PRO_NORMDW, VV_EPI_BIAS_GELU}};
@@ -87,7 +88,13 @@
     if ((a->N & 3) || (a->ldy & 3)) return false;
     if ((((uintptr_t)a->Y) & 15) || (a->bias && (((uintptr_t)a->bias) & 15))) return false;
     if (a->nscale && (((uintptr_t)a->nscale) & 15)) return false;
-    if (a->epi == VV_EPI_GATED_RESID && ((a->ld_gate & 3) || (((uintptr_t)a->gate) & 15))) return false;
+    if ((a->epi == VV_EPI_GATED_RESID || a->epi == VV_EPI_GATED_RESID_FOLD) && ((a->ld_gate & 3) || (((uintptr_t)a->gate) & 15))) return false;
+    if (a->epi == VV_EPI_GATED_RESID_FOLD) {
+        if (a->T != 2 || a->kgrid > 1 || a->n_xa || a->n_ya || (a->N & 31) || a->N < 32 || a->ldy != a->N || (a->fold_ld & 3)) return false;
+        if (!a->fold_w || !a->fold_sc || !a->fold_sh || !a->fold_out) return false;
+        if ((((uintptr_t)a->fold_w) | ((uintptr_t)a->fold_sc) | ((uintptr_t)a->fold_sh) | ((uintptr_t)a->fold_out)) & 15) return false;
+        if ((int64_t)a->T * a->fold_ld >= (1LL << 30)) return false;
+    }
     if (a->pro == VV_PRO_RMS_MOD && ((((uintptr_t)a->mod_scale) & 15) || (((uintptr_t)a->mod_shift) & 15))) return false;
     if (a->pro == VV_PRO_ADD_SILU && (((uintptr_t)a->addvec) & 15)) return false;
     if (a->kgrid > 1 && (a->T > 4 || a->kgrid != 3 || a->pro != VV_PRO_NONE || !a->yparts || (a->part_stride & 3) ||
@@ -101,9 +108,12 @@
 constexpr int VV_GEMV_WIDE_TILES = 256;
 constexpr int VV_GEMV_W16_MAX_TILES = 128, VV_GEMV_W16_MIN_KTILES = 96;
 constexpr int VV_GEMV_WIDE4_WGS = 128;
+constexpr int VV_KSPLIT_MAX_TILES = 128, VV_KSPLIT_MIN_KTILES = 96;
+inline bool vv_ksplit_shape(int T, int N, int K) { return T <= 4 && (N + 15) / 16 <= VV_KSPLIT_MAX_TILES && (K + 31) / 32 >= VV_KSPLIT_MIN_KTILES; }
 
 inline bool vv_gemv_plan(const VVGemm* a, int xs, VVGemvPlan* out) {
     if (!vv_gemv_eligible(a)) return false;
+    if (a->epi == VV_EPI_GATED_RESID_FOLD && xs != 1) return false;
     const VVGemvFamily* const fam = vv_gemv_families;
     const int n_tiles = (a->N + 15) / 16, k_tiles = (a->K + 31) / 32;
     const bool rows16 = a->T > 4 || a->sl_n > 0;
@@ -163,6 +173,7 @@
     if (a->sl_n > 0) return xs <= 2 && vv_gemv_plan(a, xs, &p) ? VV_ROUTE_GEMV : VV_ROUTE_NONE;
     if (a->ksplit <= 0 && vv_gemv_plan(a, xs, &p)) return VV_ROUTE_GEMV;
     if (a->kgrid > 1 || a->n_xa > 0 || a->n_ya > 0) return VV_ROUTE_NONE;
+    if (a->epi == VV_EPI_GATED_RESID_FOLD) return VV_ROUTE_NONE;
     return VV_ROUTE_GENERAL;
 }
 
diff --git a/vibevoice_amd/csrc/headtail.hip b/vibevoice_amd/csrc/headtail.hip
--- a/vibevoice_amd/csrc/headtail.hip
+++ b/vibevoice_amd/csrc/headtail.hip
@@ -8,7 +8,7 @@
 constexpr int WB = 4;
 constexpr int KMAX = 16;
 
-template <int TPW, int PARTS, int TR>
+template <int TPW, int PARTS, int TR, int FOLD = 0>
 __global__ __launch_bounds__(512) void vv_head_tail_kernel(const VVTail a) {
     constexpr int WPB = 8, MR = 4, MRS = 8, GSB = MRS * 16, NT = 4;
     extern __shared__ __attribute__((aligned(16))) unsigned char smem[];
@@ -20,6 +20,21 @@
     const int wave = __builtin_amdgcn_readfirstlane((int)(threadIdx.x >> 6));
     const int frow = lane & 15, fq = lane >> 4;
     const int T = a.T, H = a.H;
+    static_assert(!FOLD || (PARTS == 0 && TR == 2), "the fold form: one utterance's two rows, no part tensors");
+    constexpr int FT = FOLD ? (KMAX * 32 * WPB / 16 + WPB - 1) / WPB : 1;
+    f32x4 fp[FT];
+    float fssq = 0.f;
+    unsigned fn = 0;
+    if constexpr (FOLD) {
+        const unsigned tiles = (unsigned)H >> 4, tper = (tiles + WPB - 1) / WPB;
+        const unsigned t0 = min(tiles, wave * tper), t1 = min(tiles, t0 + tper);
+        fn = t1 - t0;
+        const f32x4* const tp = reinterpret_cast<const f32x4*>(a.fold) + (size_t)t0 * (VV_FOLD_TILE / 4) + lane;
+#pragma unroll
+        for (int i = 0; i < FT; ++i)
+            if ((unsigned)i < fn) fp[i] = tp[i * (VV_FOLD_TILE / 4)];
+        if ((unsigned)lane < 2 * fn) fssq = a.fold[vv_fold_ssq_off((int)tiles) + t0 * 2 + lane];
+    }
     const unsigned k_tiles = (unsigned)H >> 5;
     const unsigned kper = (k_tiles + WPB - 1) / WPB;
     const unsigned kt0 = wave * kper, kt1 = min(k_tiles, kt0 + kper);
@@ -60,6 +75,15 @@
         }
     }
     unsigned char* stg = stg_all + (size_t)wave * (KMAX * 4 * GSB);
+    if constexpr (FOLD) {
+        __builtin_amdgcn_sched_barrier(0);
+        f32x4 e = f32x4{0.f, 0.f, 0.f, 0.f};
+#pragma unroll
+        for (int i = 0; i < FT; ++i) if ((unsigned)i < fn) e += fp[i];
+        reinterpret_cast<f32x4*>(stg)[lane] = e;
+        const float s0 = vv_wave_sum((lane & 1) ? 0.f : fssq), s1 = vv_wave_sum((lane & 1) ? fssq : 0.f);
+        if (lane == 0) { ssq_sh[wave][0] = s0; ssq_sh[wave][1] = s1; ssq_sh[wave][2] = 0.f; ssq_sh[wave][3] = 0.f; }
+    } else {
     const unsigned kk = lane * 4;
     const unsigned st_off = ((kk >> 5) * 4 + ((kk & 31) >> 3)) * GSB + (kk & 7) * 2;
     float ssq[MR] = {0.f, 0.f, 0.f, 0.f};
@@ -144,12 +168,28 @@
         const float s = (r < T) ? vv_wave_sum(ssq[r]) : 0.f;
         if (lane == 0) ssq_sh[wave][r] = s;
     }
+    }
     __syncthreads();
     if (wave < NT) {
         const int nt = wave;
-        f32x4 e = reinterpret_cast<const f32x4*>(stg_all)[nt * 64 + lane];
+        f32x4 e, esh = f32x4{0.f, 0.f, 0.f, 0.f};
+        if constexpr (FOLD) {
+            const int fi = (frow & 1) * 16 + nt * 4 + fq;
+            e = f32x4{0.f, 0.f, 0.f, 0.f};
+            if (frow < 2) {
+                e = reinterpret_cast<const f32x4*>(stg_all)[fi];
+                esh = reinterpret_cast<const f32x4*>(stg_all)[32 + fi];
+#pragma unroll
+                for (int w = 1; w < WPB; ++w) {
+                    e += reinterpret_cast<const f32x4*>(stg_all + (size_t)w * (KMAX * 4 * GSB))[fi];
+                    esh += reinterpret_cast<const f32x4*>(stg_all + (size_t)w * (KMAX * 4 * GSB))[32 + fi];
+                }
+            }
+        } else {
+        e = reinterpret_cast<const f32x4*>(stg_all)[nt * 64 + lane];
 #pragma unroll
         for (int w = 1; w < WPB; ++w) e += reinterpret_cast<const f32x4*>(stg_all + (size_t)w * (KMAX * 4 * GSB))[nt * 64 + lane];
+        }
         float s = 0.f;
 #pragma unroll
         for (int w = 0; w < WPB; ++w) s += ssq_sh[w][frow & 3];
@@ -160,8 +200,10 @@
 #pragma unroll
         for (int r = 0; r < 4; ++r) {
             const float av = e[r];
-            const int sv = __builtin_amdgcn_update_dpp(0, __builtin_bit_cast(int, av), 0x100 + MR, 0xF, 0xF, true);
-            const float o = av * rs + __builtin_bit_cast(float, sv);
+            float shv;
+            if constexpr (FOLD) shv = esh[r];
+            else shv = __builtin_bit_cast(float, __builtin_amdgcn_update_dpp(0, __builtin_bit_cast(int, av), 0x100 + MR, 0xF, 0xF, true));
+            const float o = av * rs + shv;
             const int oi = __builtin_bit_cast(int, o);
             const int ui = (nc == 1) ? __builtin_amdgcn_update_dpp(0, oi, 0x101, 0xF, 0xF, true) : __builtin_amdgcn_update_dpp(0, oi, 0x102, 0xF, 0xF, true);
             const float vu = __builtin_bit_cast(float, ui);
@@ -212,6 +254,7 @@
     if (a->bin && (((uintptr_t)a->bin) & 15)) return 0;
     if (a->n_xa != 0 && (a->n_xa != 2 || !a->xa || (((uintptr_t)a->xa) & 15) || (a->part_stride & 3))) return 0;
     if ((int64_t)a->T * a->ld_mod >= (1LL << 30) || (int64_t)a->T * a->H >= (1LL << 30)) return 0;
+    if (a->fold && (a->n_xa != 0 || (((uintptr_t)a->fold) & 15))) return 0;
     return 1;
 }
 
@@ -219,7 +262,7 @@
 constexpr size_t HT_SMEM = 8 * KMAX * 4 * 128 + 2 * 1024 + 8 * 4 * sizeof(float);
 
 extern "C" int vv_head_tail_init() {
-    if (vv_raise_lds_limit((int)HT_SMEM, &vv_head_tail_kernel<HT_TPW, 1, 2>, &vv_head_tail_kernel<HT_TPW, 0, 2>) != hipSuccess) { (void)hipGetLastError(); return -1; }
+    if (vv_raise_lds_limit((int)HT_SMEM, &vv_head_tail_kernel<HT_TPW, 1, 2>, &vv_head_tail_kernel<HT_TPW, 0, 2>, &vv_head_tail_kernel<HT_TPW, 0, 2, 1>) != hipSuccess) { (void)hipGetLastError(); return -1; }
     return 0;
 }
 
@@ -227,7 +270,8 @@
     if (!vv_head_tail_ok(ap)) return -3;
     const VVTail& a = *ap;
     const dim3 grid((a.H / 16 + HT_TPW - 1) / HT_TPW);
-    if (a.n_xa) hipLaunchKernelGGL((vv_head_tail_kernel<HT_TPW, 1, 2>), grid, dim3(512), HT_SMEM, s, a);
+    if (a.fold) hipLaunchKernelGGL((vv_head_tail_kernel<HT_TPW, 0, 2, 1>), grid, dim3(512), HT_SMEM, s, a);
+    else if (a.n_xa) hipLaunchKernelGGL((vv_head_tail_kernel<HT_TPW, 1, 2>), grid, dim3(512), HT_SMEM, s, a);
     else hipLaunchKernelGGL((vv_head_tail_kernel<HT_TPW, 0, 2>), grid, dim3(512), HT_SMEM, s, a);
     return vv_launch_rc(0);
 }
diff --git a/vibevoice_amd/csrc/pass_plan.h b/vibevoice_amd/csrc/pass_plan.h
--- a/vibevoice_amd/csrc/pass_plan.h
+++ b/vibevoice_amd/csrc/pass_plan.h
@@ -1,5 +1,6 @@
 #pragma once
 #include "vv_common.h"
+#include "gemv_plan.h"
 
 constexpr int VV_P16_MIN_ROWS = 5, VV_P16_MAX_ROWS = 16;
 inline bool vv_p16_rows(int rows) { return rows >= VV_P16_MIN_ROWS && rows <= VV_P16_MAX_ROWS; }
@@ -72,7 +73,7 @@
        VV_FINAL_GEMM_CFG,
        VV_FINAL_GEMM };
 
-struct VVHeadCaps { bool p16_ok, p16_shift, ada_p, mod_all, head_tail; };
+struct VVHeadCaps { bool p16_ok, p16_shift, ada_p, mod_all, head_tail, fold = false; };
 
 struct VVHeadPlan {
     int rows, n_steps;
@@ -82,9 +83,11 @@
     bool seam;
     int final_stage;
     bool solver_step;
+    bool fold;
 };
 
-inline VVHeadPlan vv_head_plan(int rows, int n_steps, int HF, int HL, int MODW, const VVHeadCaps& c, bool has_coef, bool solver_step = false) {
+inline VVHeadPlan vv_head_plan(int rows, int n_steps, int HF, int HL, int MODW, const VVHeadCaps& c, bool has_coef, bool solver_step = false,
+                               int H = 0) {
     VVHeadPlan p;
     p.rows = rows; p.n_steps = n_steps;
     const bool batch_ada = has_coef && c.mod_all;
@@ -94,7 +97,9 @@
     p.seam = has_coef && rows == 2 && c.head_tail;
     p.final_stage = p.layers == VV_HEAD_P16 && p.sh_tiles && has_coef && HL > 0 ? VV_FINAL_P16_CFG : has_coef ? VV_FINAL_GEMM_CFG : VV_FINAL_GEMM;
     p.solver_step = solver_step;
+    p.fold = p.seam && c.fold && !solver_step && HL > 0 && H > 0 && (H % 32) == 0 && p.layers == VV_HEAD_GEMV && !vv_ksplit_shape(rows, H, HF);
     if (solver_step) { p.sh_tiles = false; p.seam = false; p.final_stage = VV_FINAL_GEMM; }
     return p;
 }
 inline int vv_head_final(const VVHeadPlan& p, int step) { return p.seam && step + 1 < p.n_steps ? VV_FINAL_SEAM : p.final_stage; }
+inline bool vv_head_fold(const VVHeadPlan& p, int step) { return p.fold && vv_head_final(p, step) == VV_FINAL_SEAM; }
diff --git a/vibevoice_amd/csrc/vv_common.h b/vibevoice_amd/csrc/vv_common.h
--- a/vibevoice_amd/csrc/vv_common.h
+++ b/vibevoice_amd/csrc/vv_common.h
@@ -32,7 +32,8 @@
        VV_PRO_NORMDW = 4 };
 enum { VV_EPI_STORE = 0, VV_EPI_BIAS = 1, VV_EPI_BIAS_GELU = 2, VV_EPI_SWIGLU = 3,
        VV_EPI_RESID = 4, VV_EPI_GATED_RESID = 5, VV_EPI_CFG_DPM = 6,
-       VV_EPI_QKV_ROPE = 7 };
+       VV_EPI_QKV_ROPE = 7,
+       VV_EPI_GATED_RESID_FOLD = 8 };
 
 struct VVGemm {
     const u32x4* W;
@@ -77,7 +78,17 @@
     const float* dw_nw;
     float* dw_xout;
     float* dw_hnew;
+    const u32x4* fold_w;
+    const float* fold_sc;
+    const float* fold_sh;
+    int fold_ld;
+    float* fold_out;
+    float* z_copy;
 };
+
+constexpr int VV_FOLD_TILE = 2 * 2 * 64;
+static inline __host__ __device__ size_t vv_fold_ssq_off(int tiles) { return (size_t)tiles * VV_FOLD_TILE; }
+static inline __host__ __device__ size_t vv_fold_floats(int tiles) { return (size_t)tiles * (VV_FOLD_TILE + 2); }
 
 struct VVGemv16p {
     const u32x4* W;
@@ -98,6 +109,7 @@
     float* ssq_out;
     float* z; float* x0p; const float* coef; float cfg; int n_cfg; const float* sde_noise;
     const float* cfg_rows;
+    float* z_copy;
 };
 
 struct VVTail {
@@ -113,6 +125,7 @@
     const float* coef; float cfg; int n_cfg; const float* sde_noise;
     const float* cfg_rows;
     int T, H, L; float eps;
+    const float* fold;
 };
 
 struct VVSlotIds { int n; int id[8]; };
```

Result: no change. 16.47, median of 6 (+0.1%).
